# wenbowen123/BundleTrack

Measured on AMD Instinct MI355X. Metric: Gauss-Newton iters/sec (K=15, 2k corr/frame-pair) + achieved HBM GB/s, higher is better.
Workload: dtype f32

## Files before the change

bundletrack_amd/_lib.py:

```python
from __future__ import annotations

import ctypes as C
import os
import subprocess

import numpy as np

_PKG = os.path.dirname(os.path.abspath(__file__))
_ROOT = os.path.dirname(_PKG)
LIB_PATH = os.path.join(_PKG, "libbtba.so")
SRC_DIR = os.path.join(_PKG, "csrc")
HEADER = os.path.join(_ROOT, "include", "btba.h")

BTBA_OK, BTBA_EINVAL, BTBA_EHIP, BTBA_ENUMERIC, BTBA_ENOMEM, BTBA_ESCHED = 0, 1, 2, 3, 4, 5
PAIRS_TARGET_LOWER, PAIRS_TARGET_MORE_VALID, PAIRS_EXPLICIT, PAIRS_TARGET_HIGHER = 0, 1, 2, 3
REDUCE_DETERMINISTIC, REDUCE_ATOMIC = 0, 1
RANSAC_REFERENCE_SVD, RANSAC_HORN = 0, 1
RANSAC_DRAW_HASH = 0x100
FLAG_TRACE, FLAG_TIME_KERNELS = 1, 2
FLAG_OVERLAP, FLAG_NO_FUSE, FLAG_KEYED_CORR, FLAG_FLOAT4_CACHE, FLAG_NO_COMPACTION, FLAG_COMPACTION, FLAG_TIME_SAMPLED = 32, 64, 4096, 256, 512, 1024, 2048
OPT_DENSE_ORDER, OPT_TILE_MAJOR, OPT_BLOCK_WALK, OPT_BLOCK_SKIP, OPT_BIG_ASSEMBLY, OPT_OVERLAP_GROUPS, OPT_OVERLAP_EQUAL_PRIO, OPT_KEYED_CORR_MIN_BYTES, OPT_SPARSE_TAIL = 1, 2, 3, 4, 5, 6, 7, 8, 9
OPT_CHAIN, OPT_CHAIN_SPARSE_PERIOD, OPT_CHAIN_TIMEOUT_MS, OPT_COUNT_LIVE, OPT_RELAYOUT, OPT_CORR_NONTEMPORAL, OPT_SOLVE_SMALL = 10, 11, 12, 13, 14, 15, 16

ENTRYJ_DTYPE = np.dtype(
    [("imgIdx_i", "<u4"), ("imgIdx_j", "<u4"), ("pos_i", "<f4", (3,)), ("pos_j", "<f4", (3,))]
)

EXPORTED_SYMBOLS = [
    "btba_params_default", "btba_strerror", "btba_last_hip_error", "btba_version",
    "btba_workspace_create", "btba_workspace_create_on_stream", "btba_workspace_destroy", "btba_workspace_sync",
    "btba_workspace_wait_stream", "btba_workspace_signal_stream", "btba_workspace_set_option", "btba_workspace_live_blocks",
    "btba_optimize_frames", "btba_optimize_frames_keyed", "btba_frame_cache_clear", "btba_frame_cache_evict", "btba_ransac_pairs", "btba_ransac_pairs_ex", "btba_ransac_reference_uniforms", "btba_build_cache", "btba_solve_batch", "btba_solve_cached", "btba_collect_stats",
    "btba_trace_layout_get", "btba_bucket_correspondences",
    "btba_matrices_to_poses", "btba_poses_to_matrices",
    "btba_process_depth", "btba_depth_to_normals",
    "btba_build_cache_zn", "btba_pack_zn", "btba_solve_batch_zn", "btba_zn_block_ranges", "btba_zn_valid_lists", "btba_solve_batch_zn_aux", "btba_pack_correspondences24",
    "btba_match_params_default", "btba_match_capacity", "btba_match_pairs",
    "btba_mask_params_default", "btba_apply_masks",
    "btba_detector_params_default", "btba_detector_transform", "btba_detector_inputs", "btba_detector_keypoints_to_image",
    "btba_pose_errors",
    "btba_mappoints_create", "btba_mappoints_destroy", "btba_mappoints_register_frame", "btba_mappoints_forget_frame", "btba_mappoints_export",
    "btba_corres_params_default", "btba_corres_chain_capacity", "btba_corres_chain",
    "btba_window_layout", "btba_marshal_windows", "btba_procrustes_pairs",
]

MATCH_DTYPE = np.dtype(
    [("idx_a", "<i4"), ("idx_b", "<i4"), ("dist", "<f4"), ("dir", "<i4"), ("ptA_cam", "<f4", (3,)), ("ptB_cam", "<f4", (3,))]
)


class Params(C.Structure):
    _fields_ = [
        ("n_gn_iters", C.c_int32), ("n_pcg_iters", C.c_int32),
        ("robust_delta", C.c_float), ("dense_dist_thresh", C.c_float), ("dense_normal_thresh", C.c_float),
        ("depth_min", C.c_float), ("depth_max", C.c_float),
        ("weight_sparse", C.c_float), ("weight_dense_depth", C.c_float), ("image_downscale", C.c_float),
        ("pair_policy", C.c_int32), ("dense_tiles", C.c_int32), ("sparse_chunks", C.c_int32), ("flags", C.c_int32), ("reduction_mode", C.c_int32),
        ("weights_sparse_per_iter", C.c_void_p), ("weights_dense_per_iter", C.c_void_p),
        ("n_weights_per_iter", C.c_int32),
    ]


class MatchParams(C.Structure):
    _fields_ = [("k", C.c_int32), ("mutual", C.c_int32), ("max_dist_neighbor", C.c_float), ("cos_max_normal_neighbor", C.c_float),
                ("max_dist_no_neighbor", C.c_float), ("cos_max_normal_no_neighbor", C.c_float), ("min_z", C.c_float)]


class MaskParams(C.Structure):
    _fields_ = [("largest_component_hull", C.c_int32), ("dilate", C.c_int32)]


class DetectorParams(C.Structure):
    _fields_ = [("out_size", C.c_int32)]


class Stats(C.Structure):
    _fields_ = [
        ("n_instances", C.c_int32), ("n_frames", C.c_int32), ("n_pairs", C.c_int32), ("n_dense_pairs", C.c_int32),
        ("n_corr", C.c_int64),
        ("dense_tiles", C.c_int32), ("sparse_chunks", C.c_int32),
        ("ms_total", C.c_float), ("ms_upload", C.c_float), ("ms_cache", C.c_float), ("ms_solve", C.c_float),
        ("ms_dense_sweep", C.c_float), ("ms_sparse_sweep", C.c_float), ("ms_system_solve", C.c_float),
        ("n_dense_launches", C.c_int32), ("n_sparse_launches", C.c_int32), ("n_solve_launches", C.c_int32),
        ("bytes_dense_alg", C.c_int64), ("bytes_sparse_alg", C.c_int64),
        ("fused_sweeps", C.c_int32), ("cache_frames_built", C.c_int32), ("corr_pairs_uploaded", C.c_int32),
        ("chain_iterations", C.c_int32),
    ]

    def as_dict(self):
        return {f[0]: getattr(self, f[0]) for f in self._fields_}


class ZnAux(C.Structure):
    _fields_ = [("block_ranges", C.c_void_p), ("valid_lists", C.c_void_p), ("valid_counts", C.c_void_p), ("corr24", C.c_void_p)]


class TraceLayout(C.Structure):
    _fields_ = [(n, C.c_int64) for n in
                ("record_floats", "off_x", "off_T", "off_rhs", "off_precond", "off_pcg", "off_delta", "off_dense_pair", "off_A", "off_clk")]


class CorresParams(C.Structure):
    _fields_ = [("n_trials", C.c_int32), ("dist_thres", C.c_float), ("hypothesis", C.c_int32), ("pad", C.c_int32), ("seed", C.c_uint64)]


class BtbaError(RuntimeError):
    def __init__(self, status: int, where: str):
        self.status = status
        msg = lib().btba_strerror(status).decode() if _lib is not None else str(status)
        extra = f" (hipError {lib().btba_last_hip_error()})" if status == BTBA_EHIP else ""
        super().__init__(f"{where}: {msg}{extra}")


HIPCC_FLAGS = ["--offload-arch=gfx950", "-O3", "-std=c++17", "-fno-slp-vectorize", "-Wno-pass-failed", "-fPIC", "-shared", "-fvisibility=hidden"]


def build(force: bool = False, verbose: bool = False) -> str:
    srcs = [os.path.join(SRC_DIR, f) for f in os.listdir(SRC_DIR)] + [HEADER]
    newest = max(os.path.getmtime(s) for s in srcs)
    if not force and os.path.exists(LIB_PATH) and os.path.getmtime(LIB_PATH) >= newest:
        return LIB_PATH
    cmd = ["hipcc"] + HIPCC_FLAGS + ["-o", LIB_PATH, os.path.join(SRC_DIR, "btba_api.hip")]
    if verbose:
        print(" ".join(cmd))
    subprocess.check_call(cmd)
    return LIB_PATH


HOST_DRIVER = os.path.join(os.path.dirname(_PKG), "tests", "cpp", "host_driver")


def build_host_cpp(force: bool = False, verbose: bool = False) -> str:
    root = os.path.dirname(_PKG)
    srcs = [os.path.join(root, "tests", "cpp", "host_driver.cpp"), os.path.join(_PKG, "cpp", "btba_host.cpp")]
    deps = srcs + [os.path.join(_PKG, "cpp", "btba_host.hpp"), HEADER, LIB_PATH]
    if not force and os.path.exists(HOST_DRIVER) and os.path.getmtime(HOST_DRIVER) >= max(os.path.getmtime(d) for d in deps):
        return HOST_DRIVER
    rocm = os.environ.get("ROCM_PATH", "/opt/rocm")
    cmd = ["g++", "-O2", "-std=c++17", "-Wall", "-D__HIP_PLATFORM_AMD__", "-I" + os.path.join(rocm, "include"), "-o", HOST_DRIVER] + srcs + [
        "-L" + _PKG, "-lbtba", "-L" + os.path.join(rocm, "lib"), "-lamdhip64",
        "-Wl,-rpath," + _PKG, "-Wl,-rpath,$ORIGIN/../../bundletrack_amd", "-Wl,-rpath," + os.path.join(rocm, "lib")]
    if verbose:
        print(" ".join(cmd))
    subprocess.check_call(cmd)
    return HOST_DRIVER


_lib = None


def lib() -> C.CDLL:
    global _lib
    if _lib is None:
        path = os.environ.get("BTBA_LIB_PATH", LIB_PATH)
        if not os.path.exists(path):
            raise ImportError(
                f"{path} is missing: the HIP extension has not been built. "
                "Run `python -c 'import __graft_entry__ as g; g.build()'` (needs hipcc). There is no CPU fallback.")
        try:
            import torch
        except ImportError:
            pass
        L = C.CDLL(path)
        import re
        header_version = int(re.search(r"#define BTBA_VERSION (\d+)", open(HEADER).read()).group(1))
        if "BTBA_LIB_PATH" not in os.environ and L.btba_version() != header_version:
            raise ImportError(f"{path} is version {L.btba_version()}, include/btba.h is {header_version}: rebuild (python -c 'import __graft_entry__ as g; g.build()')")
        L.btba_strerror.restype = C.c_char_p
        L.btba_strerror.argtypes = [C.c_int]
        for name in EXPORTED_SYMBOLS:
            if "BTBA_LIB_PATH" in os.environ and name in ("btba_workspace_set_option", "btba_pack_correspondences24", "btba_workspace_live_blocks") and not hasattr(L, name):
                continue
            getattr(L, name)
        L.btba_workspace_create.argtypes = [C.POINTER(C.c_void_p), C.c_void_p]
        L.btba_workspace_create_on_stream.argtypes = [C.POINTER(C.c_void_p), C.c_void_p]
        L.btba_workspace_destroy.argtypes = [C.c_void_p]
        L.btba_workspace_destroy.restype = None
        L.btba_workspace_sync.argtypes = [C.c_void_p]
        if hasattr(L, "btba_workspace_set_option"):
            L.btba_workspace_set_option.argtypes = [C.c_void_p, C.c_int, C.c_int64]
        if hasattr(L, "btba_workspace_live_blocks"):
            L.btba_workspace_live_blocks.argtypes = [C.c_void_p, C.POINTER(C.c_uint64)]
        L.btba_workspace_wait_stream.argtypes = [C.c_void_p, C.c_void_p]
        L.btba_workspace_signal_stream.argtypes = [C.c_void_p, C.c_void_p]
        L.btba_collect_stats.argtypes = [C.c_void_p, C.POINTER(Stats)]
        L.btba_optimize_frames.argtypes = [
            C.c_void_p, C.POINTER(Params), C.c_int, C.c_int, C.c_int, C.c_void_p,
            C.c_void_p, C.c_uint32, C.c_void_p, C.c_void_p, C.c_void_p, C.c_void_p, C.c_int, C.c_void_p, C.POINTER(Stats)]
        L.btba_optimize_frames_keyed.argtypes = [
            C.c_void_p, C.POINTER(Params), C.c_int, C.c_int, C.c_int, C.c_void_p,
            C.c_void_p, C.c_uint32, C.c_void_p, C.c_void_p, C.c_void_p, C.c_void_p, C.c_void_p, C.c_int, C.c_void_p, C.POINTER(Stats)]
        L.btba_frame_cache_clear.argtypes = [C.c_void_p]
        L.btba_frame_cache_evict.argtypes = [C.c_void_p, C.c_uint64]
        L.btba_solve_cached.argtypes = [
            C.c_void_p, C.POINTER(Params), C.c_int, C.c_int, C.c_int, C.c_void_p,
            C.c_void_p, C.c_void_p, C.c_void_p, C.c_uint32, C.c_void_p, C.c_uint32, C.c_void_p, C.c_int, C.c_void_p, C.c_void_p]
        L.btba_build_cache.argtypes = [C.c_void_p, C.c_int, C.c_int, C.c_int, C.c_void_p, C.c_float,
                                       C.c_void_p, C.c_void_p, C.c_void_p, C.c_void_p, C.c_void_p, C.c_void_p]
        L.btba_solve_batch.argtypes = [
            C.c_void_p, C.POINTER(Params), C.c_int, C.c_int, C.c_int, C.c_int, C.c_void_p,
            C.c_void_p, C.c_void_p, C.c_void_p, C.c_int64, C.c_void_p, C.c_uint32, C.c_void_p, C.c_int, C.c_void_p, C.c_void_p]
        L.btba_trace_layout_get.argtypes = [C.c_int, C.c_int, C.c_int, C.POINTER(TraceLayout)]
        L.btba_trace_layout_get.restype = None
        L.btba_bucket_correspondences.argtypes = [C.c_void_p, C.c_uint32, C.c_int, C.c_void_p, C.c_void_p]
        L.btba_matrices_to_poses.argtypes = [C.c_void_p, C.c_int, C.c_void_p, C.c_void_p]
        L.btba_poses_to_matrices.argtypes = [C.c_void_p, C.c_int, C.c_void_p, C.c_void_p, C.c_void_p]
        L.btba_build_cache_zn.argtypes = [C.c_void_p, C.c_int, C.c_int, C.c_int, C.c_void_p, C.c_float, C.c_void_p, C.c_void_p, C.c_void_p, C.c_void_p, C.c_void_p]
        L.btba_pack_zn.argtypes = [C.c_void_p, C.c_int64, C.c_void_p, C.c_void_p, C.c_void_p]
        L.btba_solve_batch_zn.argtypes = [C.c_void_p, C.POINTER(Params), C.c_int, C.c_int, C.c_int, C.c_int, C.c_void_p, C.c_void_p,
                                          C.c_void_p, C.c_int64, C.c_void_p, C.c_uint32, C.c_void_p, C.c_int, C.c_void_p, C.c_void_p]
        L.btba_zn_block_ranges.argtypes = [C.c_void_p, C.c_int, C.c_int, C.c_int, C.c_void_p, C.c_void_p]
        if hasattr(L, "btba_pack_correspondences24"):
            L.btba_pack_correspondences24.argtypes = [C.c_void_p, C.c_int, C.c_int, C.c_void_p, C.c_int64, C.c_void_p, C.c_uint32, C.c_void_p, C.c_void_p]
        L.btba_zn_valid_lists.argtypes = [C.c_void_p, C.c_int, C.c_int, C.c_int, C.c_void_p, C.c_void_p, C.c_void_p]
        L.btba_solve_batch_zn_aux.argtypes = [C.c_void_p, C.POINTER(Params), C.c_int, C.c_int, C.c_int, C.c_int, C.c_void_p, C.c_void_p, C.POINTER(ZnAux),
                                              C.c_void_p, C.c_int64, C.c_void_p, C.c_uint32, C.c_void_p, C.c_int, C.c_void_p, C.c_void_p]
        L.btba_process_depth.argtypes = [C.c_void_p, C.c_int, C.c_int, C.c_void_p, C.c_void_p, C.c_int, C.c_float, C.c_float, C.c_int, C.c_float, C.c_float]
        L.btba_depth_to_normals.argtypes = [C.c_void_p, C.c_int, C.c_int, C.c_void_p, C.c_void_p, C.c_void_p, C.c_void_p]
        L.btba_match_params_default.argtypes = [C.POINTER(MatchParams)]
        L.btba_match_params_default.restype = None
        L.btba_match_capacity.argtypes = [C.POINTER(MatchParams), C.c_int, C.c_int, C.c_int, C.c_int, C.c_void_p, C.c_int, C.c_void_p, C.POINTER(C.c_int64)]
        L.btba_match_pairs.argtypes = [C.c_void_p, C.POINTER(MatchParams), C.c_int, C.c_int, C.c_int, C.c_int, C.c_void_p, C.c_void_p, C.c_int, C.c_void_p,
                                       C.c_void_p, C.c_void_p, C.c_void_p, C.c_void_p, C.c_void_p, C.c_int, C.c_void_p,
                                       C.c_void_p, C.c_void_p, C.c_void_p, C.c_void_p]
        L.btba_mask_params_default.argtypes = [C.POINTER(MaskParams)]
        L.btba_mask_params_default.restype = None
        L.btba_apply_masks.argtypes = [C.c_void_p, C.POINTER(MaskParams), C.c_int, C.c_int, C.c_int, C.c_void_p, C.c_void_p, C.c_void_p,
                                       C.c_void_p, C.c_void_p, C.c_void_p]
        L.btba_detector_params_default.argtypes = [C.POINTER(DetectorParams)]
        L.btba_detector_params_default.restype = None
        L.btba_detector_transform.argtypes = [C.POINTER(DetectorParams), C.c_void_p, C.c_void_p, C.c_void_p]
        L.btba_detector_inputs.argtypes = [C.c_void_p, C.POINTER(DetectorParams), C.c_int, C.c_int, C.c_int, C.c_void_p, C.c_void_p,
                                           C.c_void_p, C.c_void_p]
        L.btba_detector_keypoints_to_image.argtypes = [C.c_void_p, C.POINTER(DetectorParams), C.c_int, C.c_void_p, C.c_void_p, C.c_void_p,
                                                       C.c_void_p]
        L.btba_pose_errors.argtypes = [C.c_void_p, C.c_int, C.c_int, C.c_void_p, C.c_void_p, C.c_int, C.c_void_p, C.c_void_p, C.c_void_p,
                                       C.c_void_p, C.c_void_p]
        L.btba_mappoints_create.argtypes = [C.c_void_p, C.POINTER(C.c_void_p)]
        L.btba_mappoints_destroy.argtypes = [C.c_void_p]
        L.btba_mappoints_destroy.restype = None
        L.btba_mappoints_register_frame.argtypes = [C.c_void_p, C.c_int, C.c_void_p, C.POINTER(C.c_int32)]
        L.btba_mappoints_forget_frame.argtypes = [C.c_void_p, C.c_int32]
        L.btba_mappoints_export.argtypes = [C.c_void_p, C.c_void_p, C.c_void_p, C.c_void_p, C.c_void_p, C.c_void_p]
        L.btba_corres_params_default.argtypes = [C.POINTER(CorresParams)]
        L.btba_corres_params_default.restype = None
        L.btba_corres_chain_capacity.argtypes = L.btba_match_capacity.argtypes
        L.btba_corres_chain.argtypes = [C.c_void_p, C.c_void_p, C.POINTER(MatchParams), C.POINTER(CorresParams), C.c_int, C.c_int, C.c_int, C.c_int,
                                        C.c_void_p, C.c_void_p, C.c_int, C.c_void_p, C.c_void_p, C.c_void_p, C.c_void_p, C.c_void_p, C.c_void_p,
                                        C.c_void_p, C.c_void_p, C.c_int, C.c_void_p, C.c_void_p, C.c_void_p, C.c_void_p]
        L.btba_window_layout.argtypes = [C.c_int, C.c_int, C.c_void_p, C.c_void_p, C.c_int32, C.POINTER(C.c_int64), C.POINTER(C.c_uint32),
                                         C.c_void_p, C.c_void_p, C.c_void_p]
        L.btba_marshal_windows.argtypes = [C.c_void_p, C.c_int, C.c_int, C.c_void_p, C.c_int64, C.c_void_p, C.c_uint32, C.c_int64,
                                           C.c_void_p, C.c_void_p, C.c_void_p]
        L.btba_procrustes_pairs.argtypes = [C.c_void_p, C.c_int, C.c_int, C.c_void_p, C.c_int64, C.c_void_p, C.c_void_p, C.c_void_p,
                                            C.c_void_p, C.c_void_p, C.c_void_p]
        _lib = L
    return _lib


def check(status: int, where: str) -> None:
    if status != BTBA_OK:
        raise BtbaError(status, where)


def default_params(**kw) -> Params:
    p = Params()
    lib().btba_params_default(C.byref(p))
    for k, v in kw.items():
        if not hasattr(p, k):
            raise AttributeError(k)
        setattr(p, k, v)
    return p


def match_params(**kw) -> MatchParams:
    p = MatchParams()
    lib().btba_match_params_default(C.byref(p))
    for k, v in kw.items():
        if not hasattr(p, k):
            raise AttributeError(k)
        setattr(p, k, v)
    return p


def corres_params(**kw) -> CorresParams:
    p = CorresParams()
    lib().btba_corres_params_default(C.byref(p))
    for k, v in kw.items():
        if not hasattr(p, k):
            raise AttributeError(k)
        setattr(p, k, v)
    return p


def mask_params(**kw) -> MaskParams:
    p = MaskParams()
    lib().btba_mask_params_default(C.byref(p))
    for k, v in kw.items():
        if not hasattr(p, k):
            raise AttributeError(k)
        setattr(p, k, v)
    return p


def detector_params(**kw) -> DetectorParams:
    p = DetectorParams()
    lib().btba_detector_params_default(C.byref(p))
    for k, v in kw.items():
        if not hasattr(p, k):
            raise AttributeError(k)
        setattr(p, k, v)
    return p


def declared_symbols() -> list[str]:
    import re
    txt = open(HEADER).read()
    return sorted(set(re.findall(r"^BTBA_API[^;]*?\b(btba_[a-z_0-9]+)\s*\(", txt, flags=re.M)))


def bucket_correspondences(corr: np.ndarray, n_frames: int):
    corr = np.ascontiguousarray(corr, ENTRYJ_DTYPE)
    P = n_frames * (n_frames - 1) // 2
    out = np.zeros(max(corr.shape[0], 1), ENTRYJ_DTYPE)
    off = np.zeros(P + 1, np.uint32)
    check(lib().btba_bucket_correspondences(corr.ctypes.data, corr.shape[0], n_frames, out.ctypes.data, off.ctypes.data),
          "btba_bucket_correspondences")
    return out[: int(off[P])], off
```

bundletrack_amd/csrc/btba_api.hip:

```cpp
#include <hip/hip_runtime.h>
#include <chrono>
#include <cmath>
#include <cstdio>
#include <cstring>
#include <cstdlib>
#include <new>
#include <string>
#include <map>
#include <memory>
#include <vector>

#include "../../include/btba.h"
#include "btba_kernels.hpp"
#include "btba_solve_small.hpp"
#include "btba_solve_mid.hpp"
#include "btba_image.hpp"
#include "btba_ransac.hpp"
#include "btba_xorwow.hpp"
#include "btba_match.hpp"
#include "btba_mask.hpp"
#include "btba_detect.hpp"
#include "btba_eval.hpp"
#include "btba_mappoints.hpp"
#include "btba_window.hpp"

using namespace btba;

static thread_local int g_last_hip_error = 0;

#define HIP_TRY(expr)                                   \
    do {                                                \
        hipError_t e_ = (expr);                         \
        if (e_ != hipSuccess) {                         \
            g_last_hip_error = (int)e_;                 \
            return BTBA_EHIP;                           \
        }                                               \
    } while (0)

namespace {

struct DevBuf {
    void *p = nullptr;
    size_t cap = 0;
    int ensure(size_t bytes)
    {
        if (bytes <= cap) return BTBA_OK;
        if (p) { hipError_t e = hipFree(p); p = nullptr; cap = 0; if (e != hipSuccess) { g_last_hip_error = (int)e; return BTBA_EHIP; } }
        size_t want = bytes + bytes / 4 + 256;
        hipError_t e = hipMalloc(&p, want);
        if (e != hipSuccess) { g_last_hip_error = (int)e; p = nullptr; return e == hipErrorOutOfMemory ? BTBA_ENOMEM : BTBA_EHIP; }
        cap = want;
        return BTBA_OK;
    }
    void release() { if (p) (void)hipFree(p); p = nullptr; cap = 0; }
    template <class T> T *as() const { return reinterpret_cast<T *>(p); }
};

struct EventPair { hipEvent_t a, b; int kind; };

}

struct btba_workspace {
    hipStream_t stream = nullptr;
    bool owns_stream = false;
    int device = 0;
    DevBuf x, T, Tinv, sparse_part, dense_part, pairsum, dense_pairs, ptrs, big_A, solve_tab;
    DevBuf corr, offsets, poses, campos, normals, nvalid;
    DevBuf valid_lists, valid_counts;
    DevBuf block_ranges;
    DevBuf chain_sync;
    DevBuf chain_trace;
    DevBuf corr24_tmp;
    DevBuf live_blocks;
    bool count_live = false;
    int *chain_error = nullptr;
    bool chain_failed = false;
    bool chain_reported = false;
    uint64_t chain_launches = 0;
    struct Tuning {
        bool dense_order = true;
        bool tile_major = true;
        bool block_walk = true;
        bool block_skip = true;
        int sparse_tail_256 = -1;
        bool big_assembly = true;
        int overlap_groups = 2;
        bool overlap_equal_prio = false;
        size_t keyed_corr_min_bytes = (size_t)1 << 20;
        int chain = 0;
        int corr_nt = -1;
        int corr_nt_partial = 1;
        long long last_level_cache = 224ll << 20;
        bool relayout = false;
        int chain_group = 1;
        int chain_sparse_period = 0;
        int chain_timeout_ms = 500;
        int chain_solve_prio = 0;
        int chain_debug_skip = 0;
        bool solve_small = true;
        int prepare_keep_T = 0;
        int debug_lds_pad = 0;
        std::string chain_trace_file;
    } tune;
    std::vector<int32_t> dense_pairs_host;
    int dense_pairs_frames = -1;
    size_t dense_work_offset = 0;
    int work_formula = 0;
    int solve_tab_frames = -1;
    std::vector<EventPair> events;
    std::vector<hipEvent_t> event_pool;
    btba_stats stats{};
    bool lds_attr_set = false, small_attr_set = false, mid_attr_set = false;
    int n_cus = 0;
    bool always_time_region = false;
    static constexpr int kMaxGroups = 8;
    uint64_t solves_enqueued = 0;
    hipStream_t aux_streams[kMaxGroups - 1] = {};
    hipEvent_t ev_fork = nullptr, ev_join[kMaxGroups - 1] = {}, ev_order = nullptr;
    hipStream_t copy_stream = nullptr;
    hipEvent_t ev_copy = nullptr, ev_cache = nullptr;
    void *pin = nullptr; size_t pin_cap = 0;
    void *pin_io = nullptr; size_t pin_io_cap = 0;
    int pin_io_ensure(size_t bytes)
    {
        if (bytes <= pin_io_cap) return BTBA_OK;
        if (pin_io) { (void)hipHostFree(pin_io); pin_io = nullptr; pin_io_cap = 0; }
        const size_t want = bytes + bytes / 2 + 4096;
        hipError_t e = hipHostMalloc(&pin_io, want, hipHostMallocDefault);
        if (e != hipSuccess) { g_last_hip_error = (int)e; pin_io = nullptr; return e == hipErrorOutOfMemory ? BTBA_ENOMEM : BTBA_EHIP; }
        pin_io_cap = want;
        return BTBA_OK;
    }
    int pin_ensure(size_t bytes)
    {
        if (bytes <= pin_cap) return BTBA_OK;
        if (pin) { (void)hipHostFree(pin); pin = nullptr; pin_cap = 0; }
        const size_t want = bytes + bytes / 2 + 4096;
        hipError_t e = hipHostMalloc(&pin, want, hipHostMallocDefault);
        if (e != hipSuccess) { g_last_hip_error = (int)e; pin = nullptr; return e == hipErrorOutOfMemory ? BTBA_ENOMEM : BTBA_EHIP; }
        pin_cap = want;
        return BTBA_OK;
    }
    struct PendingSlot { int slot; uint64_t key; const float *depth, *normal; };
    std::vector<PendingSlot> pool_pending;

    struct FrameSlot { uint64_t key = 0; const float *depth = nullptr, *normal = nullptr; uint64_t stamp = 0; bool live = false; int32_t n_valid = 0; };
    DevBuf pool_zn, pool_lists, pool_counts, pool_nvalid, pool_map, pool_ranges;
    size_t pool_map_offset = 0;
    struct CorrSeg { uint32_t off = 0, count = 0; };
    DevBuf corr_pool, corr_desc, corr_stage_dev, corr_lens;
    std::map<std::pair<uint64_t, uint64_t>, CorrSeg> corr_index;
    size_t corr_pool_used = 0;
    void *corr_stage = nullptr; size_t corr_stage_cap = 0;
    DevBuf ransac;
    DevBuf ransac_u;
    std::vector<float> ransac_u_host;
    DevBuf match;
    DevBuf mask;
    DevBuf eval;
    DevBuf corres;
    DevBuf window;
    uint64_t ransac_u_seed = 0;
    std::vector<FrameSlot> pool_slots;
    int pool_H = 0, pool_W = 0, pool_npix = 0;
    float pool_downscale = 0.0f, pool_K[9] = {0};
    uint64_t pool_stamp = 0;
    uint64_t pool_hits = 0, pool_misses = 0;

    hipEvent_t get_event()
    {
        if (!event_pool.empty()) { hipEvent_t e = event_pool.back(); event_pool.pop_back(); return e; }
        hipEvent_t e = nullptr;
        if (hipEventCreate(&e) != hipSuccess) return nullptr;
        return e;
    }
};

struct DeviceGuard {
    int prev = -1;
    explicit DeviceGuard(const btba_workspace *ws)
    {
        int cur = -1;
        if (ws && hipGetDevice(&cur) == hipSuccess && cur != ws->device && hipSetDevice(ws->device) == hipSuccess) prev = cur;
    }
    ~DeviceGuard() { if (prev >= 0) (void)hipSetDevice(prev); }
    DeviceGuard(const DeviceGuard &) = delete;
    DeviceGuard &operator=(const DeviceGuard &) = delete;
};

extern "C" {

void btba_params_default(btba_params *p)
{
    if (!p) return;
    p->n_gn_iters = 7;
    p->n_pcg_iters = 5;
    p->robust_delta = 0.005f;
    p->dense_dist_thresh = 0.02f;
    p->dense_normal_thresh = (float)std::cos(45.0 / 180.0 * M_PI);
    p->depth_min = 0.1f;
    p->depth_max = 9999.0f;
    p->weight_sparse = 1.0f;
    p->weight_dense_depth = 1.0f;
    p->image_downscale = 4.0f;
    p->pair_policy = BTBA_PAIRS_TARGET_LOWER;
    p->dense_tiles = 0;
    p->sparse_chunks = 0;
    p->flags = 0;
    p->reduction_mode = BTBA_REDUCE_DETERMINISTIC;
    p->weights_sparse_per_iter = nullptr;
    p->weights_dense_per_iter = nullptr;
    p->n_weights_per_iter = 0;
}

const char *btba_strerror(int status)
{
    switch (status) {
    case BTBA_OK: return "ok";
    case BTBA_EINVAL: return "invalid argument";
    case BTBA_EHIP: return "HIP runtime error (see btba_last_hip_error)";
    case BTBA_ENUMERIC: return "non-finite value in the output poses";
    case BTBA_ENOMEM: return "out of device memory";
    case BTBA_ESCHED: return "a wait inside the chained launch timed out (workgroups did not start in grid order): the solve's poses are invalid; the workspace now solves unchained";
    default: return "unknown status";
    }
}

int btba_last_hip_error(void) { return g_last_hip_error; }
int btba_version(void) { return BTBA_VERSION; }

static int workspace_create(btba_workspace **out, void *stream, bool use_given);

int btba_workspace_create(btba_workspace **out, void *stream) { return workspace_create(out, stream, stream != nullptr); }
int btba_workspace_create_on_stream(btba_workspace **out, void *stream) { return workspace_create(out, stream, true); }

static int workspace_create(btba_workspace **out, void *stream, bool use_given)
{
    if (!out) return BTBA_EINVAL;
    *out = nullptr;
    int ndev = 0;
    HIP_TRY(hipGetDeviceCount(&ndev));
    if (ndev <= 0) { g_last_hip_error = (int)hipErrorNoDevice; return BTBA_EHIP; }
    btba_workspace *ws = new (std::nothrow) btba_workspace();
    if (!ws) return BTBA_ENOMEM;
    if (hipGetDevice(&ws->device) != hipSuccess) { delete ws; return BTBA_EHIP; }
    if (hipDeviceGetAttribute(&ws->n_cus, hipDeviceAttributeMultiprocessorCount, ws->device) != hipSuccess) ws->n_cus = 0;
    {
        auto on = [](const char *name) { const char *e = std::getenv(name); return e && e[0] && e[0] != '0'; };
        btba_workspace::Tuning &t = ws->tune;
        t.dense_order = !on("BTBA_NO_DENSE_ORDER");
        t.tile_major = !on("BTBA_PAIR_MAJOR");
        t.block_walk = !on("BTBA_NO_BLOCK_WALK");
        t.block_skip = !on("BTBA_NO_BLOCK_SKIP");
        t.big_assembly = !on("BTBA_NO_BIG_ASSEMBLY");
        if (const char *e = std::getenv("BTBA_SPARSE_TAIL")) t.sparse_tail_256 = std::max(0, std::min(256, std::atoi(e)));
        if (const char *e = std::getenv("BTBA_GROUPS")) t.overlap_groups = std::atoi(e);
        if (const char *e = std::getenv("BTBA_GROUP_PRIO")) t.overlap_equal_prio = e[0] == 'e';
        if (const char *e = std::getenv("BTBA_KEYED_CORR_MIN_BYTES")) t.keyed_corr_min_bytes = (size_t)std::strtoull(e, nullptr, 10);
        if (const char *e = std::getenv("BTBA_CHAIN")) t.chain = std::max(-1, std::min(1, std::atoi(e)));
        if (const char *e = std::getenv("BTBA_CHAIN_PERIOD")) t.chain_sparse_period = std::max(0, std::atoi(e));
        t.relayout = on("BTBA_RELAYOUT");
        t.solve_small = !on("BTBA_SOLVE_LEGACY");
        if (const char *e = std::getenv("BTBA_CORR_NT")) t.corr_nt = std::atoi(e);
        if (const char *e = std::getenv("BTBA_LLC_MB")) t.last_level_cache = (long long)std::atoll(e) << 20;
        if (const char *e = std::getenv("BTBA_CORR_NT_PARTIAL")) t.corr_nt_partial = std::atoi(e);
        if (const char *e = std::getenv("BTBA_CHAIN_TIMEOUT_MS")) t.chain_timeout_ms = std::max(1, std::atoi(e));
#if defined(BTBA_DEV_EXPERIMENTS) || defined(BTBA_REFERENCE_ORDER)
        t.prepare_keep_T = on("BTBA_PREPARE_KEEP_T") ? 1 : 0;
#endif
#ifdef BTBA_DEV_EXPERIMENTS
        if (const char *e = std::getenv("BTBA_CHAIN_GROUP")) t.chain_group = std::max(1, std::atoi(e));
        if (const char *e = std::getenv("BTBA_CHAIN_TRACE_FILE")) t.chain_trace_file = e;
        if (const char *e = std::getenv("BTBA_CHAIN_SOLVE_PRIO")) t.chain_solve_prio = std::max(0, std::min(3, std::atoi(e)));
        if (const char *e = std::getenv("BTBA_CHAIN_DEBUG_SKIP")) t.chain_debug_skip = std::atoi(e);
        if (const char *e = std::getenv("BTBA_DEBUG_LDS_PAD")) t.debug_lds_pad = std::max(0, std::min(60000, std::atoi(e)));
#endif
    }
    if (use_given) {
        ws->stream = reinterpret_cast<hipStream_t>(stream);
    } else {
        hipError_t e = hipStreamCreateWithFlags(&ws->stream, hipStreamNonBlocking);
        if (e != hipSuccess) { g_last_hip_error = (int)e; delete ws; return BTBA_EHIP; }
        ws->owns_stream = true;
    }
    *out = ws;
    return BTBA_OK;
}

void btba_workspace_destroy(btba_workspace *ws)
{
    DeviceGuard device_guard(ws);
    if (!ws) return;
    (void)hipStreamSynchronize(ws->stream);
    for (auto &ep : ws->events) { (void)hipEventDestroy(ep.a); (void)hipEventDestroy(ep.b); }
    for (auto e : ws->event_pool) (void)hipEventDestroy(e);
    DevBuf *bufs[] = { &ws->x, &ws->T, &ws->Tinv, &ws->sparse_part, &ws->dense_part, &ws->pairsum, &ws->dense_pairs, &ws->ptrs, &ws->big_A, &ws->solve_tab,
                       &ws->corr, &ws->offsets, &ws->poses, &ws->campos, &ws->normals, &ws->nvalid, &ws->valid_lists, &ws->valid_counts, &ws->block_ranges,
                       &ws->chain_sync, &ws->chain_trace, &ws->live_blocks, &ws->corr24_tmp, &ws->pool_zn, &ws->pool_lists, &ws->pool_counts, &ws->pool_nvalid, &ws->pool_map, &ws->pool_ranges, &ws->ransac, &ws->ransac_u, &ws->match, &ws->mask, &ws->eval, &ws->corr_pool, &ws->corr_desc, &ws->corr_stage_dev, &ws->corr_lens, &ws->window };
    for (auto b : bufs) b->release();
    if (ws->corr_stage) (void)hipHostFree(ws->corr_stage);
    if (ws->chain_error) (void)hipHostFree(ws->chain_error);
    for (auto st : ws->aux_streams) if (st) (void)hipStreamDestroy(st);
    if (ws->copy_stream) (void)hipStreamDestroy(ws->copy_stream);
    if (ws->ev_copy) (void)hipEventDestroy(ws->ev_copy);
    if (ws->ev_cache) (void)hipEventDestroy(ws->ev_cache);
    if (ws->pin) (void)hipHostFree(ws->pin);
    if (ws->pin_io) (void)hipHostFree(ws->pin_io);
    if (ws->ev_fork) (void)hipEventDestroy(ws->ev_fork);
    for (auto e : ws->ev_join) if (e) (void)hipEventDestroy(e);
    if (ws->ev_order) (void)hipEventDestroy(ws->ev_order);
    if (ws->owns_stream) (void)hipStreamDestroy(ws->stream);
    delete ws;
}

int btba_workspace_set_option(btba_workspace *ws, int option, int64_t value)
{
    DeviceGuard device_guard(ws);
    if (!ws) return BTBA_EINVAL;
    btba_workspace::Tuning &t = ws->tune;
    switch (option) {
    case BTBA_OPT_DENSE_ORDER: t.dense_order = value != 0; ws->dense_pairs_frames = -1; break;
    case BTBA_OPT_TILE_MAJOR: t.tile_major = value != 0; break;
    case BTBA_OPT_BLOCK_WALK: t.block_walk = value != 0; break;
    case BTBA_OPT_BLOCK_SKIP: t.block_skip = value != 0; break;
    case BTBA_OPT_BIG_ASSEMBLY: t.big_assembly = value != 0; break;
    case BTBA_OPT_SPARSE_TAIL: if (value < -1 || value > 256) return BTBA_EINVAL; t.sparse_tail_256 = (int)value; break;
    case BTBA_OPT_OVERLAP_GROUPS: if (value < 1 || value > btba_workspace::kMaxGroups) return BTBA_EINVAL; t.overlap_groups = (int)value; break;
    case BTBA_OPT_OVERLAP_EQUAL_PRIO:
        if (t.overlap_equal_prio != (value != 0)) {
            for (auto &st : ws->aux_streams) if (st) { HIP_TRY(hipStreamSynchronize(st)); HIP_TRY(hipStreamDestroy(st)); st = nullptr; }
        }
        t.overlap_equal_prio = value != 0;
        break;
    case BTBA_OPT_KEYED_CORR_MIN_BYTES: if (value < 0) return BTBA_EINVAL; t.keyed_corr_min_bytes = (size_t)value; break;
    case BTBA_OPT_CHAIN: if (value < -1 || value > 1) return BTBA_EINVAL; t.chain = (int)value; break;
    case BTBA_OPT_CHAIN_SPARSE_PERIOD: if (value < 0 || value == 1 || value > 64) return BTBA_EINVAL; t.chain_sparse_period = (int)value; break;
    case BTBA_OPT_CHAIN_TIMEOUT_MS: if (value < 1 || value > 60000) return BTBA_EINVAL; t.chain_timeout_ms = (int)value; break;
    case BTBA_OPT_RELAYOUT: t.relayout = value != 0; break;
    case BTBA_OPT_SOLVE_SMALL: t.solve_small = value != 0; break;
    case BTBA_OPT_CORR_NONTEMPORAL: if (value < -1 || value > 1) return BTBA_EINVAL; t.corr_nt = (int)value; break;
    case BTBA_OPT_COUNT_LIVE:
        ws->count_live = value != 0;
        if (ws->count_live) {
            int rc = ws->live_blocks.ensure(sizeof(unsigned long long));
            if (rc) return rc;
            HIP_TRY(hipMemsetAsync(ws->live_blocks.p, 0, sizeof(unsigned long long), ws->stream));
        }
        break;
    case 1000:
#ifdef BTBA_DEV_EXPERIMENTS
        t.chain_debug_skip = (int)value; break;
#else
        if (value != 0 && value != 64) return BTBA_EINVAL;
        t.chain_debug_skip = (int)value; break;
#endif
    default: return BTBA_EINVAL;
    }
    return BTBA_OK;
}

static int chain_check(btba_workspace *ws)
{
    if (!ws->chain_error || !*ws->chain_error) return BTBA_OK;
    *ws->chain_error = 0;
    ws->chain_failed = true;
    const bool already = ws->chain_reported;
    ws->chain_reported = false;
    return already ? BTBA_OK : BTBA_ESCHED;
}

int btba_workspace_live_blocks(btba_workspace *ws, uint64_t *blocks)
{
    DeviceGuard device_guard(ws);
    if (!ws || !blocks) return BTBA_EINVAL;
    *blocks = 0;
    if (!ws->live_blocks.p) return BTBA_OK;
    HIP_TRY(hipStreamSynchronize(ws->stream));
    unsigned long long v = 0;
    HIP_TRY(hipMemcpy(&v, ws->live_blocks.p, sizeof v, hipMemcpyDeviceToHost));
    *blocks = v;
    return BTBA_OK;
}

int btba_workspace_sync(btba_workspace *ws)
{
    DeviceGuard device_guard(ws);
    if (!ws) return BTBA_EINVAL;
    HIP_TRY(hipStreamSynchronize(ws->stream));
    return chain_check(ws);
}

static int order_streams(btba_workspace *ws, hipStream_t from, hipStream_t to)
{
    if (from == to) return BTBA_OK;
    if (!ws->ev_order) HIP_TRY(hipEventCreateWithFlags(&ws->ev_order, hipEventDisableTiming));
    HIP_TRY(hipEventRecord(ws->ev_order, from));
    HIP_TRY(hipStreamWaitEvent(to, ws->ev_order, 0));
    return BTBA_OK;
}

int btba_workspace_wait_stream(btba_workspace *ws, void *stream)
{
    DeviceGuard device_guard(ws);
    if (!ws) return BTBA_EINVAL;
    return order_streams(ws, static_cast<hipStream_t>(stream), ws->stream);
}

int btba_workspace_signal_stream(btba_workspace *ws, void *stream)
{
    DeviceGuard device_guard(ws);
    if (!ws) return BTBA_EINVAL;
    return order_streams(ws, ws->stream, static_cast<hipStream_t>(stream));
}

void btba_trace_layout_get(int n_frames, int n_dense_pairs, int n_pcg_iters, btba_trace_layout *L)
{
    if (!L) return;
    const int64_t N = n_frames, n = 6 * N;
    int64_t o = 0;
    L->off_x = o; o += N * 6;
    L->off_T = o; o += N * 16;
    L->off_rhs = o; o += N * 6;
    L->off_precond = o; o += N * 6;
    L->off_pcg = o; o += (int64_t)n_pcg_iters * 4;
    L->off_delta = o; o += N * 6;
    L->off_dense_pair = o; o += (int64_t)n_dense_pairs * kDenseVals;
    L->off_A = o; o += n * n;
    L->off_clk = o; o += 8;
    L->record_floats = o;
}

static inline int pair_index(int n_frames, uint32_t i, uint32_t j) { return (int)(i * n_frames - i * (i + 1) / 2 + (j - i - 1)); }

static int count_correspondences(const btba_entryj *in, uint32_t n, int n_frames, uint32_t *out_offsets, bool *already_bucketed)
{
    const int P = n_frames * (n_frames - 1) / 2;
    std::vector<uint32_t> cnt(P + 1, 0);
    bool ordered = true;
    int prev = 0;
    for (uint32_t e = 0; e < n; e++) {
        const btba_entryj &c = in[e];
        if (c.imgIdx_i == 0xFFFFFFFFu) { ordered = false; continue; }
        if (c.imgIdx_i >= (uint32_t)n_frames || c.imgIdx_j >= (uint32_t)n_frames || c.imgIdx_i >= c.imgIdx_j) return BTBA_EINVAL;
        const int p = pair_index(n_frames, c.imgIdx_i, c.imgIdx_j);
        ordered = ordered && (p >= prev);
        prev = p;
        cnt[p + 1]++;
    }
    out_offsets[0] = 0;
    for (int p = 0; p < P; p++) out_offsets[p + 1] = out_offsets[p] + cnt[p + 1];
    if (already_bucketed) *already_bucketed = ordered;
    return BTBA_OK;
}

static void scatter_correspondences(const btba_entryj *in, uint32_t n, int n_frames, const uint32_t *offsets, btba_entryj *out_sorted)
{
    const int P = n_frames * (n_frames - 1) / 2;
    std::vector<uint32_t> cur(offsets, offsets + P);
    for (uint32_t e = 0; e < n; e++) {
        const btba_entryj &c = in[e];
        if (c.imgIdx_i == 0xFFFFFFFFu) continue;
        out_sorted[cur[pair_index(n_frames, c.imgIdx_i, c.imgIdx_j)]++] = c;
    }
}

int btba_bucket_correspondences(const btba_entryj *in, uint32_t n, int n_frames, btba_entryj *out_sorted, uint32_t *out_offsets)
{
    if ((!in && n) || n_frames < 2 || !out_sorted || !out_offsets) return BTBA_EINVAL;
    if (int rc = count_correspondences(in, n, n_frames, out_offsets, nullptr)) return rc;
    scatter_correspondences(in, n, n_frames, out_offsets, out_sorted);
    return BTBA_OK;
}

}

static int time_begin(btba_workspace *ws, bool on, int kind, size_t *slot, hipStream_t st = nullptr)
{
    if (!st) st = ws->stream;
    *slot = (size_t)-1;
    if (!on) return BTBA_OK;
    EventPair ep{ ws->get_event(), ws->get_event(), kind };
    if (!ep.a || !ep.b) return BTBA_EHIP;
    HIP_TRY(hipEventRecord(ep.a, st));
    ws->events.push_back(ep);
    *slot = ws->events.size() - 1;
    return BTBA_OK;
}
static int time_end(btba_workspace *ws, size_t slot, hipStream_t st = nullptr)
{
    if (!st) st = ws->stream;
    if (slot == (size_t)-1) return BTBA_OK;
    HIP_TRY(hipEventRecord(ws->events[slot].b, st));
    return BTBA_OK;
}

static int pick_chunks(const btba_params *prm, int B, int P, uint32_t max_corr_per_pair, bool with_dense)
{
    if (prm->sparse_chunks > 0) return prm->sparse_chunks;
    if (max_corr_per_pair == 0) return 1;
    const long blocks = (long)B * P;
    if (with_dense) {
        const int cap = std::min(16, (int)((max_corr_per_pair + 2 * kBlock - 1) / (2 * kBlock)));
        const int want = (int)((64 + blocks - 1) / blocks);
        if (want <= cap) return std::max(1, want);
    }
    int want = (int)((512 + blocks - 1) / blocks);
    const int cap = (int)((max_corr_per_pair + 2 * kBlock - 1) / (2 * kBlock));
    if (want > cap) want = cap;
    if (want < 1) want = 1;
    if (want > 16) want = 16;
    return want;
}
static int pick_tiles(const btba_params *prm, int B, int Pd, int npix, bool lists, int Wd, int Hd)
{
    if (prm->dense_tiles > 0) return prm->dense_tiles;
    if (Pd == 0) return 1;
    const long blocks = (long)B * Pd;
    if (lists) return blocks >= 64 ? 1 : 3;
    int want = blocks >= 1536 ? 1 : blocks >= 768 ? 2 : blocks >= 192 ? 4 : 8;
    const int cap = (npix + kBlock - 1) / kBlock;
    if (want > cap) want = cap;
    if (want < 1) want = 1;
    if (Wd % 8 == 0 && Hd % 8 == 0) {
        const int bw = Wd / 8, bh = Hd / 8;
        const int min_tiles = (bw * bh + 1023) / 1024;
        if (want < min_tiles && bw <= 1024) want = std::min(min_tiles, bh);
        const int rows_per = (bh + want - 1) / want;
        want = (bh + rows_per - 1) / rows_per;
        while (want < bh && (long)((bh + want - 1) / want) * bw > 1024 && bw <= 1024) want++;
    }
    return want;
}

static void scaled_intrinsics(int H, int W, int Hd, int Wd, const float *K, float intr[4], Mat4 *Kinv);

struct ZnSpec {
    const float *zn = nullptr; int H = 0, W = 0; const float *K = nullptr;
    const int *frame_slot = nullptr;
    const uint32_t *lists = nullptr; const int *counts = nullptr;
    const float *block_ranges = nullptr;
};

static int solve_enqueue(btba_workspace *ws, const btba_params *prm, int B, int N, int Hd, int Wd, const float *intr,
                         const float *campos, const float *normals, const ZnSpec &Z, const btba_entryj *corr, int64_t corr_stride,
                         const uint32_t *pair_offsets, uint32_t max_corr_per_pair,
                         const int32_t *dense_pairs, int Pd_in, float *poses, float *trace, int *order_flag = nullptr,
                         bool corr24 = false, const uint32_t *pair_lens = nullptr)
{
    if (!ws || !prm || B < 1 || N < 2 || Hd < 2 || Wd < 2 || !intr || !poses) return BTBA_EINVAL;
    if (prm->n_gn_iters < 1 || prm->n_pcg_iters < 0) return BTBA_EINVAL;
    if (ws->chain_error && *ws->chain_error && !ws->chain_reported) { ws->chain_reported = true; ws->chain_failed = true; return BTBA_ESCHED; }
    if (prm->reduction_mode != BTBA_REDUCE_DETERMINISTIC && prm->reduction_mode != BTBA_REDUCE_ATOMIC) return BTBA_EINVAL;
    const bool atomic_sums = prm->reduction_mode == BTBA_REDUCE_ATOMIC;
    if (atomic_sums && trace) return BTBA_EINVAL;
    if (N > BTBA_MAX_FRAMES) return BTBA_EINVAL;
    const int P = N * (N - 1) / 2;
    const float *wsi = prm->weights_sparse_per_iter, *wdi = prm->weights_dense_per_iter;
    if ((wsi || wdi) && prm->n_weights_per_iter != prm->n_gn_iters) return BTBA_EINVAL;
    auto ws_at = [&](int it) { return wsi ? wsi[it] : prm->weight_sparse; };
    auto wd_at = [&](int it) { return wdi ? wdi[it] : prm->weight_dense_depth; };
    bool any_dense_weight = false, any_sparse_weight = false;
    for (int it = 0; it < prm->n_gn_iters; it++) {
        if (!(ws_at(it) >= 0.0f) || !(wd_at(it) >= 0.0f)) return BTBA_EINVAL;
        any_dense_weight |= wd_at(it) > 0.0f; any_sparse_weight |= ws_at(it) > 0.0f;
    }
    const bool use_sparse = any_sparse_weight && corr && pair_offsets && max_corr_per_pair > 0;
    std::vector<int32_t> pairs;
    if (any_dense_weight) {
        if (dense_pairs && Pd_in >= 0) pairs.assign(dense_pairs, dense_pairs + 2 * (size_t)Pd_in);
        else for (int i = 0; i < N; i++) for (int j = i + 1; j < N; j++) { pairs.push_back(i); pairs.push_back(j); }
        for (size_t k = 0; k < pairs.size(); k += 2)
            if (pairs[k] < 0 || pairs[k] >= N || pairs[k + 1] < 0 || pairs[k + 1] >= N || pairs[k] == pairs[k + 1]) return BTBA_EINVAL;
        if (dense_pairs && Pd_in >= 0) {
            std::vector<char> seen((size_t)N * N, 0);
            for (size_t k = 0; k < pairs.size(); k += 2) {
                char &c = seen[(size_t)pairs[k] * N + pairs[k + 1]];
                if (c) return BTBA_EINVAL;
                c = 1;
            }
        }
    }
    const int Pd = (int)(pairs.size() / 2);
    const bool use_zn = Z.zn != nullptr;
    const bool use_dense = Pd > 0 && ((campos && normals) || use_zn);
    if (!use_sparse && !use_dense) {
    }
    const int npix = Hd * Wd;
    int B_launch = B;
    if (B >= 8 && (prm->flags & BTBA_FLAG_OVERLAP)) {
        const int groups = std::max(1, std::min({ ws->tune.overlap_groups, (int)btba_workspace::kMaxGroups, B / 2 }));
        B_launch = B / groups;
    }
    const int chunks = use_sparse ? pick_chunks(prm, B_launch, P, max_corr_per_pair, use_dense && !(prm->flags & BTBA_FLAG_NO_FUSE)) : 1;
    const int tiles = use_dense ? pick_tiles(prm, B_launch, Pd, npix, use_zn && (prm->flags & BTBA_FLAG_COMPACTION), Wd, Hd) : 1;
    const bool timing = (prm->flags & BTBA_FLAG_TIME_KERNELS) != 0;
    const int timed_iteration = (prm->flags & BTBA_FLAG_TIME_SAMPLED) ? (int)(ws->solves_enqueued++ % (uint64_t)std::max(1, prm->n_gn_iters)) : -1;

    int rc;
    if ((rc = ws->x.ensure(sizeof(float) * 6 * (size_t)B * N))) return rc;
    if ((rc = ws->T.ensure(sizeof(float) * 16 * (size_t)B * N))) return rc;
    if ((rc = ws->Tinv.ensure(sizeof(float) * 16 * (size_t)B * N))) return rc;
    if ((rc = ws->sparse_part.ensure(sizeof(float) * (size_t)B * P * chunks * kSparseVals))) return rc;
    if ((rc = ws->dense_part.ensure(sizeof(float) * (size_t)B * (Pd > 0 ? Pd : 1) * tiles * kDenseVals))) return rc;
    if (Pd > 0 && (pairs != ws->dense_pairs_host || ws->dense_pairs_frames != N)) {
        std::vector<int32_t> tab(pairs);
        std::vector<int32_t> off(N + 1, 0);
        for (int q = 0; q < Pd; q++) { off[pairs[2 * q] + 1]++; off[pairs[2 * q + 1] + 1]++; }
        for (int k = 0; k < N; k++) off[k + 1] += off[k];
        std::vector<int32_t> adj(2 * (size_t)Pd), cur(off.begin(), off.end() - 1);
        for (int q = 0; q < Pd; q++) { adj[cur[pairs[2 * q]]++] = (q << 1); adj[cur[pairs[2 * q + 1]]++] = (q << 1) | 1; }
        tab.insert(tab.end(), off.begin(), off.end());
        tab.insert(tab.end(), adj.begin(), adj.end());
        std::vector<int32_t> first_listed((size_t)N * N, -1);
        for (int q = Pd - 1; q >= 0; q--) first_listed[(size_t)pairs[2 * q] * N + pairs[2 * q + 1]] = q;
        for (int i = 0; i < N; i++) for (int j = i + 1; j < N; j++) tab.push_back(first_listed[(size_t)i * N + j]);
        std::vector<int32_t> order(Pd);
        for (int q = 0; q < Pd; q++) order[q] = q;
        if (ws->tune.dense_order) std::stable_sort(order.begin(), order.end(), [&](int32_t a, int32_t b2) { return std::abs(pairs[2 * a] - pairs[2 * a + 1]) < std::abs(pairs[2 * b2] - pairs[2 * b2 + 1]); });
        ws->work_formula = 0;
        if (Pd == N * (N - 1) / 2) {
            for (int form = 1; form <= 2 && !ws->work_formula; form++) {
                bool same = true;
                int q = 0;
                for (int d = 1; d < N && same; d++)
                    for (int i = 0; i + d < N && same; i++, q++) {
                        const int pc = pair_index(N, (uint32_t)i, (uint32_t)(i + d));
                        same = order[q] == pc && pairs[2 * pc] == (form == 1 ? i : i + d) && pairs[2 * pc + 1] == (form == 1 ? i + d : i);
                    }
                if (same) ws->work_formula = form;
            }
        }
        while (tab.size() % 4) tab.push_back(0);
        ws->dense_work_offset = tab.size();
        for (int q = 0; q < Pd; q++) { tab.push_back(pairs[2 * order[q]]); tab.push_back(pairs[2 * order[q] + 1]); tab.push_back(order[q]); tab.push_back(0); }
        if ((rc = ws->dense_pairs.ensure(sizeof(int32_t) * tab.size()))) return rc;
        HIP_TRY(hipMemcpyAsync(ws->dense_pairs.p, tab.data(), sizeof(int32_t) * tab.size(), hipMemcpyHostToDevice, ws->stream));
        HIP_TRY(hipStreamSynchronize(ws->stream));
        ws->dense_pairs_host = pairs;
        ws->dense_pairs_frames = N;
    }
    if (ws->solve_tab_frames != N) {
        const size_t lut16 = ((size_t)P + 288 + 3) & ~(size_t)3;
        std::vector<int32_t> tab(lut16 + 288);
        int q = 0;
        for (int i = 0; i < N; i++) for (int j = i + 1; j < N; j++) tab[q++] = (i << 8) | j;
        for (int t = 0; t < 72; t++) { sparse_entry_descriptor(t >= 36, (t % 36) / 6, t % 6, &tab[(size_t)P + 4 * t]); sparse_entry_descriptor(t >= 36, (t % 36) / 6, t % 6, &tab[lut16 + 4 * t]); }
        if ((rc = ws->solve_tab.ensure(sizeof(int32_t) * tab.size()))) return rc;
        HIP_TRY(hipMemcpyAsync(ws->solve_tab.p, tab.data(), sizeof(int32_t) * tab.size(), hipMemcpyHostToDevice, ws->stream));
        HIP_TRY(hipStreamSynchronize(ws->stream));
        ws->solve_tab_frames = N;
    }
    const int32_t *d_adj_off = ws->dense_pairs.as<int32_t>() + 2 * (size_t)Pd;
    const int32_t *d_adj = d_adj_off + (N + 1);

    SolveDims D{};
    D.n_frames = N; D.n_pairs = P; D.n_dense_pairs = use_dense ? Pd : 0;
    D.npix = npix; D.width = Wd; D.height = Hd;
    D.sparse_chunks = chunks; D.dense_tiles = tiles; D.n_pcg = prm->n_pcg_iters;
    D.use_sparse = use_sparse; D.use_dense = use_dense;
    D.fx = intr[0]; D.fy = intr[1]; D.cx = intr[2]; D.cy = intr[3];
    D.robust_delta = prm->robust_delta; D.dist_thresh = prm->dense_dist_thresh; D.normal_thresh = prm->dense_normal_thresh;
    D.dist2_thresh = prm->dense_dist_thresh * prm->dense_dist_thresh;
    D.wm1 = (float)(Wd - 1); D.hm1 = (float)(Hd - 1); D.wm2 = (float)(Wd - 2); D.hm2 = (float)(Hd - 2);
    D.depth_min = prm->depth_min; D.depth_max = prm->depth_max;
    D.w_sparse = prm->weight_sparse; D.w_dense = prm->weight_dense_depth;
    D.corr_stride = corr_stride;
    D.corr_nt_from = B;
    D.order_flag = order_flag;
    D.live_blocks = (ws->count_live && ws->live_blocks.p) ? ws->live_blocks.as<unsigned long long>() : nullptr;
    D.pose_stride = 16 * N; D.x_stride = 6 * N;
    D.sp_stride = (unsigned)((size_t)P * (atomic_sums ? 1 : chunks) * kSparseVals);
    D.dp_stride = (unsigned)((size_t)(Pd > 0 ? Pd : 1) * (atomic_sums ? 1 : tiles) * kDenseVals);
    if ((size_t)B * std::max(D.sp_stride, D.dp_stride) >= ((size_t)1 << 32) || (size_t)B * 16 * N >= ((size_t)1 << 31)) return BTBA_EINVAL;
    D.atomic_sums = atomic_sums ? 1 : 0;
    D.corr24 = corr24 ? 1 : 0;
    D.pair_lens = pair_lens;
    if (Pd > 0) { D.dense_work = reinterpret_cast<const int4 *>(ws->dense_pairs.as<int32_t>() + ws->dense_work_offset); D.work_formula = ws->work_formula; }
    D.tile_major = ws->tune.tile_major ? 1 : 0;
    D.sparse_tail_256 = 0;
    D.walk_blocks = (Wd % 8 == 0 && Hd % 8 == 0 && Wd + Hd <= 1024 && ws->tune.block_walk) ? 1 : 0;
    D.n_gn = prm->n_gn_iters;
    int zn_layout = 0;
    if (use_zn) {
        if (!Z.K || Z.H < 2 || Z.W < 2) return BTBA_EINVAL;
        float intr_chk[4];
        Mat4 Kinv;
        scaled_intrinsics(Z.H, Z.W, Hd, Wd, Z.K, intr_chk, &Kinv);
        for (int k = 0; k < 16; k++) D.zn_ki[k] = Kinv.m[k];
        D.zn_scale_w = (float)(Z.W - 1) / (float)(Wd - 1);
        D.zn_scale_h = (float)(Z.H - 1) / (float)(Hd - 1);
        const float *ki = D.zn_ki;
        D.zn_simple = (ki[1] == 0.f && ki[3] == 0.f && ki[4] == 0.f && ki[7] == 0.f && ki[12] == 0.f && ki[13] == 0.f && ki[14] == 0.f && ki[15] == 1.0f) ? 1 : 0;
        zn_layout = D.zn_simple ? 1 : 2;
    }
    D.trace_on = (trace != nullptr) && (prm->flags & BTBA_FLAG_TRACE);
    btba_trace_layout L;
    btba_trace_layout_get(N, D.n_dense_pairs, prm->n_pcg_iters, &L);
    D.trace_record = L.record_floats; D.tr_x = L.off_x; D.tr_T = L.off_T; D.tr_rhs = L.off_rhs; D.tr_prec = L.off_precond;
    D.tr_pcg = L.off_pcg; D.tr_delta = L.off_delta; D.tr_dpair = L.off_dense_pair; D.tr_A = L.off_A; D.tr_clk = L.off_clk;

    const size_t n = 6 * (size_t)N, ld = 4 * (((n + 3) / 4) | 1);
    const size_t lds_rest = (6 * ld + 16 + 16 * (size_t)N + 4 * (size_t)D.n_dense_pairs + (size_t)N + 1 + (size_t)P + 288 + (((size_t)P + 3) & ~(size_t)3) + ((6 * (size_t)N + 3) & ~(size_t)3)) * sizeof(float);
    const size_t lds_limit = 160 * 1024;
    const bool a_global = n * ld * sizeof(float) + lds_rest > lds_limit;
    const size_t lds_core = (a_global ? 0 : n * ld * sizeof(float)) + lds_rest;
    const size_t lds_pairs = ((size_t)P * kSparseVals + (size_t)D.n_dense_pairs * kDenseVals) * sizeof(float);
    D.pairsum_in_lds = (lds_core + lds_pairs <= 64 * 1024) ? 1 : 0;
    if (!D.pairsum_in_lds && lds_core + lds_pairs <= lds_limit && B <= 256) D.pairsum_in_lds = 1;
    const size_t lds_bytes = lds_core + (D.pairsum_in_lds ? lds_pairs : 0);
    if (lds_bytes > lds_limit) return BTBA_EINVAL;
    if (!D.pairsum_in_lds) { if ((rc = ws->pairsum.ensure((size_t)B * lds_pairs + 16))) return rc; }
    const size_t mid_lds = sizeof(float) * mid_solve_lds_floats(N, D.n_dense_pairs);
    const bool mid_solve = ws->tune.solve_small && N > kSmallMaxFrames && N <= kMidMaxFrames && !atomic_sums && !a_global && D.n_dense_pairs <= P && mid_lds <= lds_limit;
    D.pre_assembled = ((a_global || N >= 24) && !trace && ws->tune.big_assembly && !mid_solve) ? 1 : 0;
    if (a_global || D.pre_assembled) { if ((rc = ws->big_A.ensure((size_t)B * (n + 2) * ld * sizeof(float)))) return rc; }
    if (D.pre_assembled && D.pairsum_in_lds) { D.pairsum_in_lds = 0; if ((rc = ws->pairsum.ensure((size_t)B * lds_pairs + 16))) return rc; }
    if (lds_bytes > 64 * 1024 || !ws->lds_attr_set) {
        HIP_TRY(hipFuncSetAttribute(reinterpret_cast<const void *>(&k_system_solve<true, false>), hipFuncAttributeMaxDynamicSharedMemorySize, (int)lds_limit));
        HIP_TRY(hipFuncSetAttribute(reinterpret_cast<const void *>(&k_system_solve<false, false>), hipFuncAttributeMaxDynamicSharedMemorySize, (int)lds_limit));
        HIP_TRY(hipFuncSetAttribute(reinterpret_cast<const void *>(&k_system_solve<true, true>), hipFuncAttributeMaxDynamicSharedMemorySize, (int)lds_limit));
        HIP_TRY(hipFuncSetAttribute(reinterpret_cast<const void *>(&k_system_solve<false, true>), hipFuncAttributeMaxDynamicSharedMemorySize, (int)lds_limit));
        ws->lds_attr_set = true;
    }

    const int small_cpl_v = small_cpl(N);
    const size_t small_lds = sizeof(float) * small_solve_lds_floats(N, D.n_dense_pairs, small_cpl_v);
    const bool small_solve = ws->tune.solve_small && N <= kSmallMaxFrames && !atomic_sums && !a_global && !D.pre_assembled && 2 * D.n_dense_pairs <= kSmallBlock && small_lds <= lds_limit;
    if (small_solve && !ws->small_attr_set) {
        HIP_TRY(hipFuncSetAttribute(reinterpret_cast<const void *>(&k_solve_small<4>), hipFuncAttributeMaxDynamicSharedMemorySize, (int)lds_limit));
        HIP_TRY(hipFuncSetAttribute(reinterpret_cast<const void *>(&k_solve_small<8>), hipFuncAttributeMaxDynamicSharedMemorySize, (int)lds_limit));
        HIP_TRY(hipFuncSetAttribute(reinterpret_cast<const void *>(&k_solve_small<12>), hipFuncAttributeMaxDynamicSharedMemorySize, (int)lds_limit));
        HIP_TRY(hipFuncSetAttribute(reinterpret_cast<const void *>(&k_solve_small<16>), hipFuncAttributeMaxDynamicSharedMemorySize, (int)lds_limit));
        ws->small_attr_set = true;
    }
    if (mid_solve && !ws->mid_attr_set) {
        HIP_TRY(hipFuncSetAttribute(reinterpret_cast<const void *>(&k_solve_mid), hipFuncAttributeMaxDynamicSharedMemorySize, (int)lds_limit));
        ws->mid_attr_set = true;
    }

    btba_stats &S = ws->stats;
    if (ws->events.empty() || !timing) std::memset(&S, 0, sizeof S);
    S.n_instances = B; S.n_frames = N; S.n_pairs = P; S.n_dense_pairs = D.n_dense_pairs;
    S.dense_tiles = tiles; S.sparse_chunks = chunks;
    S.bytes_dense_alg = use_dense ? (int64_t)64 * D.n_dense_pairs * npix * B : 0;
    S.bytes_sparse_alg = 0;

    {
        const int nb0 = (B >= 8 && (prm->flags & BTBA_FLAG_OVERLAP)) ? B / 2 : B;
        S.fused_sweeps = (use_sparse && use_dense && (unsigned)chunks * P * nb0 >= 64u && (unsigned)tiles * D.n_dense_pairs * nb0 >= 64u && !(prm->flags & BTBA_FLAG_NO_FUSE)) ? 1 : 0;
    }
    size_t reg;
    if ((rc = time_begin(ws, timing || ws->always_time_region, 3, &reg))) return rc;
    if (atomic_sums) {
        HIP_TRY(hipMemsetAsync(ws->sparse_part.p, 0, sizeof(float) * (size_t)B * P * kSparseVals, ws->stream));
        HIP_TRY(hipMemsetAsync(ws->dense_part.p, 0, sizeof(float) * (size_t)B * (Pd > 0 ? Pd : 1) * kDenseVals, ws->stream));
    }
    const bool compaction = use_zn && use_dense && (prm->flags & BTBA_FLAG_COMPACTION);
    const int chain_lay = zn_layout == 1 ? (compaction ? 3 : 1) : 0;
    const bool chain = chain_lay != 0 && !ws->chain_failed && ws->n_cus == 256 && ws->tune.chain > 0 && use_sparse && use_dense && !wsi && !wdi
                       && !trace && !atomic_sums && !a_global && !D.pre_assembled && N <= kChainMaxFrames && chunks <= kChainMaxParts && tiles <= kChainMaxParts
                       && !(prm->flags & (BTBA_FLAG_NO_FUSE | BTBA_FLAG_OVERLAP)) && !Z.frame_slot
                       && lds_rest + 16 + sizeof(float) * chain_region_floats(N) <= kChainLdsBytes;
    const bool relayout = ws->tune.relayout && use_sparse && !corr24 && !pair_lens && !chain && prm->n_gn_iters >= 3 && !atomic_sums && !compaction
                          && (size_t)B * (size_t)corr_stride * sizeof(btba_entryj) >= ((size_t)4 << 20);
    if (relayout) { if ((rc = ws->corr24_tmp.ensure(sizeof(float2) * 192 * (((size_t)B * (size_t)corr_stride + 63) / 64)))) return rc; }
    const long long frames_bytes = use_dense ? (long long)B * N * npix * (use_zn ? 16 : 32) : 0;
    const long long corr_bytes = use_sparse ? (long long)B * (long long)corr_stride * (corr24 ? 24 : 32) : 0;
    const long long corr_per_instance = corr_bytes / B;
    int corr_nt_auto = B;
    if (use_dense && use_sparse && !compaction && frames_bytes + corr_bytes > ws->tune.last_level_cache)
        corr_nt_auto = (frames_bytes >= ws->tune.last_level_cache || corr_per_instance <= 0) ? 0 : (int)std::min<long long>(B, (ws->tune.last_level_cache - frames_bytes) / corr_per_instance);
    if (ws->tune.corr_nt_partial == 0 && corr_nt_auto < B) corr_nt_auto = 0;
    const int corr_nt_from = ws->tune.corr_nt >= 0 ? (ws->tune.corr_nt ? 0 : B) : corr_nt_auto;
    ChainDims Cn{};
    int plain_pairsum_in_lds = 0;
    auto pad32 = [](size_t floats) { return (floats + 31) & ~(size_t)31; };
    if (chain) {
        const int n_it = prm->n_gn_iters;
        D.pose_stride = (int)pad32(16 * (size_t)N); D.x_stride = (int)pad32(6 * (size_t)N);
        D.sp_stride = (unsigned)pad32((size_t)P * chunks * kSparseVals); D.dp_stride = (unsigned)pad32((size_t)Pd * tiles * kDenseVals);
        D.publish = 1;
        D.corr_nt_from = corr_nt_from;
        plain_pairsum_in_lds = D.pairsum_in_lds;
        D.pairsum_in_lds = 0;
        Cn.last_solve_external = 1;
        Cn.n_iter = n_it; Cn.n_inst = B; Cn.inst_per_xcd = (unsigned)((B + 7) / 8);
        Cn.items_d = (unsigned)tiles * (unsigned)D.n_dense_pairs; Cn.items_s = (unsigned)chunks * (unsigned)P;
        Cn.sparse_period = (unsigned)ws->tune.chain_sparse_period;
        if (Cn.sparse_period >= 2u && Cn.sparse_period * Cn.items_s > Cn.items_d + Cn.items_s) Cn.sparse_period = (Cn.items_d + Cn.items_s) / Cn.items_s;
        if (Cn.sparse_period < 2u) Cn.sparse_period = 0u;
        Cn.group = (Cn.sparse_period == 0u && ws->tune.chain_group > 1 && Cn.inst_per_xcd % (unsigned)ws->tune.chain_group == 0u && B % 8 == 0) ? (unsigned)ws->tune.chain_group : 1u;
        Cn.timeout_ticks = (long long)ws->tune.chain_timeout_ms * 100000ll;
        Cn.solve_prio = ws->tune.chain_solve_prio;
        Cn.debug_skip = ws->tune.chain_debug_skip;
        if (Cn.debug_skip & 16) D.publish = 0;
        Cn.pose_ring = (size_t)B * D.pose_stride; Cn.x_ring = (size_t)B * D.x_stride;
        Cn.sp_ring = (size_t)B * (size_t)D.sp_stride; Cn.dp_ring = (size_t)B * (size_t)D.dp_stride;
        Cn.ps_size = pad32((size_t)D.n_dense_pairs * kDenseVals); Cn.A_size = pad32((n + 2) * ld);
        if ((rc = ws->x.ensure(sizeof(float) * (n_it + 1) * Cn.x_ring))) return rc;
        if ((rc = ws->T.ensure(sizeof(float) * (n_it + 1) * Cn.pose_ring))) return rc;
        if ((rc = ws->Tinv.ensure(sizeof(float) * (n_it + 1) * Cn.pose_ring))) return rc;
        if ((rc = ws->sparse_part.ensure(sizeof(float) * n_it * Cn.sp_ring))) return rc;
        if ((rc = ws->dense_part.ensure(sizeof(float) * n_it * Cn.dp_ring))) return rc;
        if ((rc = ws->pairsum.ensure(sizeof(float) * (size_t)n_it * B * Cn.ps_size))) return rc;
        if ((rc = ws->big_A.ensure(sizeof(float) * (size_t)n_it * B * Cn.A_size))) return rc;
        const size_t sync_head = ((size_t)B * (n_it + 1) + 15) & ~(size_t)15;
        const size_t sync_ints = sync_head + (size_t)16 * B * (n_it + 1);
        if ((rc = ws->chain_sync.ensure(sizeof(int) * sync_ints))) return rc;
        if (!ws->chain_error) {
            HIP_TRY(hipHostMalloc(reinterpret_cast<void **>(&ws->chain_error), 64, hipHostMallocDefault));
            *ws->chain_error = 0;
        }
        HIP_TRY(hipMemsetAsync(ws->chain_sync.p, 0, sizeof(int) * sync_ints, ws->stream));
        Cn.flags = ws->chain_sync.as<int>(); Cn.arrivals = Cn.flags + B; Cn.published = Cn.flags + sync_head; Cn.error = ws->chain_error;
    }
    {
        const int total = B * N;
        if (chain) k_prepare_strided<<<(total + 63) / 64, 64, 0, ws->stream>>>(total, N, D.pose_stride, D.x_stride, poses, ws->x.as<float>(), ws->T.as<float>(), ws->Tinv.as<float>());
        else k_prepare<<<(total + 63) / 64, 64, 0, ws->stream>>>(total, poses, ws->x.as<float>(), ws->T.as<float>(), ws->Tinv.as<float>(), ws->tune.prepare_keep_T);
    }
    const uint32_t *lists_base = Z.lists;
    const int *counts_base = Z.counts;
    if (compaction && !lists_base) {
        if ((rc = ws->valid_lists.ensure(sizeof(uint32_t) * (size_t)B * N * npix))) return rc;
        if ((rc = ws->valid_counts.ensure(sizeof(int) * (size_t)B * N))) return rc;
        k_valid_lists<<<B * N, 1024, 0, ws->stream>>>(npix, reinterpret_cast<const float4 *>(Z.zn), ws->valid_lists.as<uint32_t>(), ws->valid_counts.as<int>(), nullptr);
        lists_base = ws->valid_lists.as<uint32_t>();
        counts_base = ws->valid_counts.as<int>();
    }
    if (Z.frame_slot && B != 1) return BTBA_EINVAL;
    D.frame_slot = Z.frame_slot;
    size_t blist_bytes = 0;
    if (!(zn_layout == 1 && use_dense && !compaction)) D.walk_blocks = 0;
    D.sparse_tail_256 = ws->tune.sparse_tail_256 >= 0 ? ws->tune.sparse_tail_256 : ((use_dense && !compaction) ? 256 : 0);
    if (D.walk_blocks) {
        const int bw = Wd / 8, bh = Hd / 8;
        const size_t band_blocks = (size_t)((bh + tiles - 1) / tiles) * bw;
        if (band_blocks > 1024) D.walk_blocks = 0;
        else {
            blist_bytes = 32 + sizeof(uint32_t) * band_blocks;
            if (ws->tune.block_skip) {
                if (Z.block_ranges) D.block_ranges = reinterpret_cast<const float2 *>(Z.block_ranges);
                else if (!Z.frame_slot) {
                    if ((rc = ws->block_ranges.ensure(sizeof(float2) * (size_t)B * N * bw * bh))) return rc;
                    k_block_ranges<<<dim3((unsigned)((bw * bh + kBlock / 64 - 1) / (kBlock / 64)), (unsigned)(B * N)), kBlock, 0, ws->stream>>>(Wd, Hd, reinterpret_cast<const float4 *>(Z.zn), nullptr, ws->block_ranges.as<float2>());
                    D.block_ranges = ws->block_ranges.as<float2>();
                }
            }
        }
    }
    int n_halves = (B >= 8 && (prm->flags & BTBA_FLAG_OVERLAP)) ? 2 : 1;
    if (n_halves == 2) n_halves = std::max(1, std::min({ ws->tune.overlap_groups, (int)btba_workspace::kMaxGroups, B / 2 }));
    for (int g = 1; g < n_halves; g++) {
        if (ws->aux_streams[g - 1]) continue;
        int prio_least = 0, prio_greatest = 0;
        HIP_TRY(hipDeviceGetStreamPriorityRange(&prio_least, &prio_greatest));
        HIP_TRY(hipStreamCreateWithPriority(&ws->aux_streams[g - 1], hipStreamNonBlocking, ws->tune.overlap_equal_prio ? 0 : prio_least));
        HIP_TRY(hipEventCreateWithFlags(&ws->ev_join[g - 1], hipEventDisableTiming));
        if (!ws->ev_fork) HIP_TRY(hipEventCreateWithFlags(&ws->ev_fork, hipEventDisableTiming));
    }
    struct Half { int b0, nb; hipStream_t st; } halves[btba_workspace::kMaxGroups];
    for (int g = 0; g < n_halves; g++) {
        const int lo = (int)((long long)B * g / n_halves), hi = (int)((long long)B * (g + 1) / n_halves);
        halves[g] = { lo, hi - lo, g == 0 ? ws->stream : ws->aux_streams[g - 1] };
    }
    if (n_halves > 1) {
        HIP_TRY(hipEventRecord(ws->ev_fork, ws->stream));
        for (int g = 1; g < n_halves; g++) HIP_TRY(hipStreamWaitEvent(ws->aux_streams[g - 1], ws->ev_fork, 0));
    }
    const size_t pairsum_floats = lds_pairs / sizeof(float);
    S.chain_iterations = 0;
    const size_t lut_bytes = sizeof(float) * (size_t)((Wd + Hd + 3) & ~3) + (zn_layout == 1 ? sizeof(float4) * (size_t)(Wd + Hd) : 0) + blist_bytes + (size_t)ws->tune.debug_lds_pad;
    if (chain) {
        const size_t chain_lds = std::max(lut_bytes, lds_rest + 16 + sizeof(float) * chain_region_floats(N));
        const unsigned per_inst = Cn.items_d + Cn.items_s + 1u;
        const unsigned grid = 8u * (unsigned)prm->n_gn_iters * Cn.inst_per_xcd * per_inst;
        if (!ws->tune.chain_trace_file.empty()) {
            const size_t trace_bytes = 32 * (size_t)grid + 64 * (size_t)prm->n_gn_iters * B;
            if ((rc = ws->chain_trace.ensure(trace_bytes))) return rc;
            HIP_TRY(hipMemsetAsync(ws->chain_trace.p, 0, trace_bytes, ws->stream));
            Cn.trace = ws->chain_trace.as<unsigned long long>();
            Cn.stamps = Cn.trace + 4 * (size_t)grid;
        }
        const float4 *corr_c = reinterpret_cast<const float4 *>(corr);
        size_t slot;
        if (Cn.debug_skip & 32) {
            ChainDims C1 = Cn;
            C1.n_iter = 1; C1.debug_skip |= 8; C1.trace = nullptr; C1.stamps = nullptr;
            const unsigned grid1 = 8u * Cn.inst_per_xcd * per_inst;
            if ((rc = ws->pairsum.ensure(sizeof(float) * (size_t)B * ((size_t)P * kSparseVals + (size_t)D.n_dense_pairs * kDenseVals + 64)))) return rc;
            for (int it = 0; it < prm->n_gn_iters; it++) {
                if ((rc = time_begin(ws, timing, 0, &slot))) return rc;
#define BTBA_CHAIN_ARGS1 D, C1, reinterpret_cast<const float4 *>(Z.zn), ws->T.as<float>(), ws->Tinv.as<float>(), ws->x.as<float>(), ws->dense_part.as<float>(), corr_c, pair_offsets, \
                        ws->sparse_part.as<float>(), compaction ? lists_base : nullptr, compaction ? counts_base : nullptr, ws->dense_pairs.as<int2>(), d_adj_off, d_adj, ws->solve_tab.as<int>(), \
                        ws->pairsum.as<float>(), ws->big_A.as<float>(), poses
                if (chain_lay == 1) k_chain<1><<<dim3(grid1), kBlock, chain_lds, ws->stream>>>(BTBA_CHAIN_ARGS1);
                else k_chain<3><<<dim3(grid1), kBlock, chain_lds, ws->stream>>>(BTBA_CHAIN_ARGS1);
#undef BTBA_CHAIN_ARGS1
                if ((rc = time_end(ws, slot))) return rc;
                if ((rc = time_begin(ws, timing, 2, &slot))) return rc;
                k_system_solve<false, false><<<B, kSolveBlock, lds_core, ws->stream>>>(D, it, ws->sparse_part.as<float>(), ws->dense_part.as<float>(), ws->dense_pairs.as<int2>(), d_adj_off, d_adj,
                    ws->x.as<float>(), ws->T.as<float>(), ws->Tinv.as<float>(), ws->pairsum.as<float>(), nullptr, nullptr, it == prm->n_gn_iters - 1 ? poses : nullptr, ws->solve_tab.as<int>());
                if ((rc = time_end(ws, slot))) return rc;
            }
            S.fused_sweeps = 1;
        } else {
        if ((rc = time_begin(ws, timing, 0, &slot))) return rc;
#define BTBA_CHAIN_ARGS D, Cn, reinterpret_cast<const float4 *>(Z.zn), ws->T.as<float>(), ws->Tinv.as<float>(), ws->x.as<float>(), ws->dense_part.as<float>(), corr_c, pair_offsets, \
                        ws->sparse_part.as<float>(), compaction ? lists_base : nullptr, compaction ? counts_base : nullptr, ws->dense_pairs.as<int2>(), d_adj_off, d_adj, ws->solve_tab.as<int>(), \
                        ws->pairsum.as<float>(), ws->big_A.as<float>(), poses
        if (chain_lay == 1) k_chain<1><<<dim3(grid), kBlock, chain_lds, ws->stream>>>(BTBA_CHAIN_ARGS);
        else k_chain<3><<<dim3(grid), kBlock, chain_lds, ws->stream>>>(BTBA_CHAIN_ARGS);
#undef BTBA_CHAIN_ARGS
        if ((rc = time_end(ws, slot))) return rc;
        if (Cn.last_solve_external) {
            const int il = prm->n_gn_iters - 1;
            SolveDims Dl = D;
            Dl.pairsum_in_lds = plain_pairsum_in_lds; Dl.publish = 0;
            if (!Dl.pairsum_in_lds) { if ((rc = ws->pairsum.ensure(std::max(sizeof(float) * (size_t)prm->n_gn_iters * B * Cn.ps_size, (size_t)B * lds_pairs + 16)))) return rc; }
            if ((rc = time_begin(ws, timing, 2, &slot))) return rc;
#define BTBA_LAST_SOLVE(LP) k_system_solve<LP, false><<<B, kSolveBlock, lds_bytes, ws->stream>>>(Dl, il, ws->sparse_part.as<float>() + il * Cn.sp_ring, ws->dense_part.as<float>() + il * Cn.dp_ring, \
                ws->dense_pairs.as<int2>(), d_adj_off, d_adj, ws->x.as<float>() + il * Cn.x_ring, ws->T.as<float>() + il * Cn.pose_ring, ws->Tinv.as<float>() + il * Cn.pose_ring, \
                ws->pairsum.as<float>(), nullptr, nullptr, poses, ws->solve_tab.as<int>())
            if (Dl.pairsum_in_lds) BTBA_LAST_SOLVE(true); else BTBA_LAST_SOLVE(false);
#undef BTBA_LAST_SOLVE
            if ((rc = time_end(ws, slot))) return rc;
        }
        k_chain_poison<<<(16 * B * N + 255) / 256, 256, 0, ws->stream>>>(Cn.error, poses, 16 * B * N);
        S.chain_iterations = prm->n_gn_iters;
        S.fused_sweeps = 1;
        ws->chain_launches++;
        if (Cn.trace) {
            HIP_TRY(hipStreamSynchronize(ws->stream));
            std::vector<unsigned long long> host(4 * (size_t)grid + 8 * (size_t)prm->n_gn_iters * B);
            HIP_TRY(hipMemcpy(host.data(), ws->chain_trace.p, 8 * host.size(), hipMemcpyDeviceToHost));
            if (FILE *f = std::fopen(ws->tune.chain_trace_file.c_str(), "wb")) {
                const unsigned long long nrec = grid;
                std::fwrite(&nrec, 8, 1, f); std::fwrite(host.data(), 8, host.size(), f); std::fclose(f);
            }
        }
        }
    } else
    for (int it = 0; it < prm->n_gn_iters; it++) {
        const bool timing_it = timing && (timed_iteration < 0 || timed_iteration == it);
        SolveDims Di = D;
        Di.w_sparse = ws_at(it); Di.w_dense = wd_at(it);
        const bool use_dense_it = use_dense && Di.w_dense > 0.0f;
        Di.use_dense = use_dense_it ? 1 : 0;
        for (int h = 0; h < n_halves; h++) {
            const Half &H = halves[h];
            const size_t b0 = (size_t)H.b0;
            const float *campos_h = campos ? campos + 4 * b0 * N * npix : nullptr, *normals_h = normals ? normals + 4 * b0 * N * npix : nullptr;
            const float4 *zn_h = use_zn ? reinterpret_cast<const float4 *>(Z.zn) + b0 * N * npix : nullptr;
            const uint32_t *vl_h = compaction ? lists_base + b0 * N * npix : nullptr;
            const int *vc_h = compaction ? counts_base + b0 * N : nullptr;
            const bool c24_it = corr24 || (relayout && it > 0);
            const float4 *corr_h = corr ? (corr24 ? reinterpret_cast<const float4 *>(corr) : (relayout && it > 0) ? ws->corr24_tmp.as<float4>()
                                                  : reinterpret_cast<const float4 *>(corr) + 2 * b0 * (size_t)corr_stride) : nullptr;
            const uint32_t *off_h = pair_offsets ? pair_offsets + b0 * (P + 1) : nullptr;
            float *x_h = ws->x.as<float>() + 6 * b0 * N, *T_h = ws->T.as<float>() + 16 * b0 * N, *Ti_h = ws->Tinv.as<float>() + 16 * b0 * N;
            float *sp_h = ws->sparse_part.as<float>() + b0 * P * (atomic_sums ? 1 : chunks) * kSparseVals;
            float *dp_h = ws->dense_part.as<float>() + b0 * (size_t)(Pd > 0 ? Pd : 1) * (atomic_sums ? 1 : tiles) * kDenseVals;
            float *ps_h = ws->pairsum.p ? ws->pairsum.as<float>() + b0 * pairsum_floats : nullptr;
            float *tr_h = trace ? trace + b0 * (size_t)D.n_gn * D.trace_record : nullptr;
            size_t slot;
            SolveDims Dh = Di;
            if (Dh.pair_lens) Dh.pair_lens += b0 * P;
            Dh.corr24 = c24_it ? 1 : 0;
            Dh.corr_entry0 = (c24_it || relayout) ? (int64_t)b0 * corr_stride : 0;
            Dh.corr24_out = (relayout && it == 0) ? ws->corr24_tmp.as<float2>() : nullptr;
            if (Dh.block_ranges) Dh.block_ranges += b0 * N * (size_t)((Wd / 8) * (Hd / 8));
            const unsigned n_d = (unsigned)tiles * D.n_dense_pairs * H.nb, n_s = (unsigned)chunks * P * H.nb;
            const bool fuse = use_sparse && use_dense_it && n_s >= 64 && n_d >= 64 && !(prm->flags & BTBA_FLAG_NO_FUSE);
            Dh.corr_nt_from = ((fuse && use_dense_it) || ws->tune.corr_nt >= 0) ? corr_nt_from - (int)b0 : B;
            if (fuse) {
                if ((rc = time_begin(ws, timing_it, 0, &slot, H.st))) return rc;
#define BTBA_FUSED_ARGS(CACHE) Dh, n_d, n_s, CACHE, reinterpret_cast<const float4 *>(normals_h), ws->dense_pairs.as<int2>(), T_h, Ti_h, dp_h, corr_h, off_h, sp_h, vl_h, vc_h
                const int lay = zn_layout ? zn_layout + (compaction ? 2 : 0) : 0;
                if (lay == 0) k_fused_sweeps<0><<<dim3(n_d + n_s), kBlock, 0, H.st>>>(BTBA_FUSED_ARGS(reinterpret_cast<const float4 *>(campos_h)));
                else if (lay == 1) k_fused_sweeps<1><<<dim3(n_d + n_s), kBlock, lut_bytes, H.st>>>(BTBA_FUSED_ARGS(zn_h));
                else if (lay == 2) k_fused_sweeps<2><<<dim3(n_d + n_s), kBlock, lut_bytes, H.st>>>(BTBA_FUSED_ARGS(zn_h));
                else if (lay == 3) k_fused_sweeps<3><<<dim3(n_d + n_s), kBlock, lut_bytes, H.st>>>(BTBA_FUSED_ARGS(zn_h));
                else k_fused_sweeps<4><<<dim3(n_d + n_s), kBlock, lut_bytes, H.st>>>(BTBA_FUSED_ARGS(zn_h));
#undef BTBA_FUSED_ARGS
                if ((rc = time_end(ws, slot, H.st))) return rc;
            } else {
                if (use_sparse) {
                    if ((rc = time_begin(ws, timing_it, 1, &slot, H.st))) return rc;
                    k_sparse_sweep<<<dim3(chunks, P, H.nb), kBlock, 0, H.st>>>(Dh, corr_h, off_h, T_h, sp_h);
                    if ((rc = time_end(ws, slot, H.st))) return rc;
                }
                if (use_dense_it) {
                    if ((rc = time_begin(ws, timing_it, 0, &slot, H.st))) return rc;
                    const dim3 dgrid(n_d);
#define BTBA_DENSE_ARGS Di, reinterpret_cast<const float4 *>(campos_h), reinterpret_cast<const float4 *>(normals_h), ws->dense_pairs.as<int2>(), T_h, Ti_h, dp_h
                    if (zn_layout == 1 && !compaction) k_dense_sweep_zn<true, false><<<dgrid, kBlock, lut_bytes, H.st>>>(Dh, zn_h, ws->dense_pairs.as<int2>(), T_h, Ti_h, dp_h, vl_h, vc_h);
                    else if (zn_layout == 2 && !compaction) k_dense_sweep_zn<false, false><<<dgrid, kBlock, lut_bytes, H.st>>>(Dh, zn_h, ws->dense_pairs.as<int2>(), T_h, Ti_h, dp_h, vl_h, vc_h);
                    else if (zn_layout == 1) k_dense_sweep_zn<true, true><<<dgrid, kBlock, lut_bytes, H.st>>>(Dh, zn_h, ws->dense_pairs.as<int2>(), T_h, Ti_h, dp_h, vl_h, vc_h);
                    else if (zn_layout == 2) k_dense_sweep_zn<false, true><<<dgrid, kBlock, lut_bytes, H.st>>>(Dh, zn_h, ws->dense_pairs.as<int2>(), T_h, Ti_h, dp_h, vl_h, vc_h);
                    else k_dense_sweep<<<dgrid, kBlock, 0, H.st>>>(BTBA_DENSE_ARGS);
#undef BTBA_DENSE_ARGS
                    if ((rc = time_end(ws, slot, H.st))) return rc;
                }
            }
            if ((rc = time_begin(ws, timing_it, 2, &slot, H.st))) return rc;
            float *A_h = (a_global || D.pre_assembled) ? ws->big_A.as<float>() + b0 * (n + 2) * ld : nullptr;
            float *out_h = (it == prm->n_gn_iters - 1) ? poses + 16 * b0 * N : nullptr;
            SolveDims Ds = Di;
            if (atomic_sums) { Ds.sparse_chunks = 1; Ds.dense_tiles = 1; }
            if (D.pre_assembled) {
                const size_t n_sums = (size_t)P * kSparseVals + (size_t)D.n_dense_pairs * kDenseVals;
                k_big_reduce<<<dim3((unsigned)((n_sums + 255) / 256), (unsigned)H.nb), 256, 0, H.st>>>(Ds, sp_h, dp_h, ps_h);
                const BigTasks bt = big_tasks(N, P, (int)ld);
                k_big_assemble<<<dim3((bt.total + 255u) / 256u, (unsigned)H.nb), 256, 0, H.st>>>(Di, ps_h, ws->dense_pairs.as<int2>(), d_adj_off, d_adj, ws->solve_tab.as<int>(), A_h);
            }
#define BTBA_SOLVE(LP, AG) k_system_solve<LP, AG><<<H.nb, kSolveBlock, lds_bytes, H.st>>>(Ds, it, sp_h, dp_h, ws->dense_pairs.as<int2>(), d_adj_off, d_adj, x_h, T_h, Ti_h, ps_h, tr_h, A_h, out_h, ws->solve_tab.as<int>())
            if (small_solve || mid_solve) {
                SmallSolveArgs Sa{};
                Sa.n_frames = N; Sa.n_pairs = P; Sa.n_dense_pairs = use_dense_it ? D.n_dense_pairs : 0;
                Sa.sparse_chunks = Ds.sparse_chunks; Sa.dense_tiles = Ds.dense_tiles; Sa.n_pcg = D.n_pcg; Sa.use_sparse = use_sparse ? 1 : 0;
                Sa.w_sparse = Di.w_sparse;
                Sa.sp_stride = D.sp_stride; Sa.dp_stride = D.dp_stride; Sa.pose_stride = D.pose_stride; Sa.x_stride = D.x_stride;
                Sa.iter = it;
                Sa.trace_record = D.trace_record; Sa.tr_x = D.tr_x; Sa.tr_T = D.tr_T; Sa.tr_rhs = D.tr_rhs; Sa.tr_prec = D.tr_prec; Sa.tr_pcg = D.tr_pcg;
                Sa.tr_delta = D.tr_delta; Sa.tr_dpair = D.tr_dpair; Sa.tr_A = D.tr_A; Sa.tr_clk = D.tr_clk; Sa.trace_instance = (int64_t)D.n_gn * D.trace_record;
                Sa.sparse_partials = sp_h; Sa.dense_partials = dp_h;
                Sa.adj_off = d_adj_off; Sa.adj = d_adj; Sa.cross = d_adj + 2 * (size_t)Pd; Sa.pair_ij = ws->solve_tab.as<int>(); Sa.entry_lut = ws->solve_tab.as<int>() + (((size_t)P + 288 + 3) & ~(size_t)3);
                Sa.x = x_h; Sa.T = T_h; Sa.Tinv = Ti_h; Sa.poses_out = out_h; Sa.trace = D.trace_on ? tr_h : nullptr;
                if (mid_solve) k_solve_mid<<<H.nb, kSmallBlock, mid_lds, H.st>>>(Sa);
                else if (small_cpl_v == 4) k_solve_small<4><<<H.nb, kSmallBlock, small_lds, H.st>>>(Sa);
                else if (small_cpl_v == 8) k_solve_small<8><<<H.nb, kSmallBlock, small_lds, H.st>>>(Sa);
                else if (small_cpl_v == 12) k_solve_small<12><<<H.nb, kSmallBlock, small_lds, H.st>>>(Sa);
                else k_solve_small<16><<<H.nb, kSmallBlock, small_lds, H.st>>>(Sa);
            } else
            if (a_global) { if (D.pairsum_in_lds) BTBA_SOLVE(true, true); else BTBA_SOLVE(false, true); }
            else { if (D.pairsum_in_lds) BTBA_SOLVE(true, false); else BTBA_SOLVE(false, false); }
#undef BTBA_SOLVE
            if ((rc = time_end(ws, slot, H.st))) return rc;
        }
    }
    for (int g = 1; g < n_halves; g++) {
        HIP_TRY(hipEventRecord(ws->ev_join[g - 1], ws->aux_streams[g - 1]));
        HIP_TRY(hipStreamWaitEvent(ws->stream, ws->ev_join[g - 1], 0));
    }
    if ((rc = time_end(ws, reg))) return rc;
    HIP_TRY(hipGetLastError());
    return BTBA_OK;
}

extern "C" {

int btba_collect_stats(btba_workspace *ws, btba_stats *stats)
{
    DeviceGuard device_guard(ws);
    if (!ws) return BTBA_EINVAL;
    HIP_TRY(hipStreamSynchronize(ws->stream));
    btba_stats &S = ws->stats;
    for (auto &ep : ws->events) {
        float ms = 0.0f;
        hipError_t e = hipEventElapsedTime(&ms, ep.a, ep.b);
        if (e == hipSuccess) {
            switch (ep.kind) {
            case 0: S.ms_dense_sweep += ms; S.n_dense_launches++; break;
            case 1: S.ms_sparse_sweep += ms; S.n_sparse_launches++; break;
            case 2: S.ms_system_solve += ms; S.n_solve_launches++; break;
            case 3: S.ms_solve += ms; break;
            case 4: S.ms_cache += ms; break;
            default: break;
            }
        }
        ws->event_pool.push_back(ep.a);
        ws->event_pool.push_back(ep.b);
    }
    ws->events.clear();
    if (stats) *stats = S;
    S.ms_dense_sweep = S.ms_sparse_sweep = S.ms_system_solve = S.ms_solve = S.ms_cache = 0.0f;
    S.n_dense_launches = S.n_sparse_launches = S.n_solve_launches = 0;
    return chain_check(ws);
}

int btba_solve_batch(btba_workspace *ws, const btba_params *params, int n_instances, int n_frames, int Hd, int Wd, const float *intr,
                     const float *campos_dev, const float *normals_dev, const btba_entryj *corr_dev, int64_t corr_stride,
                     const uint32_t *pair_offsets_dev, uint32_t max_corr_per_pair, const int32_t *dense_pairs, int n_dense_pairs,
                     float *poses_dev, float *trace_dev)
{
    DeviceGuard device_guard(ws);
    if (!ws) return BTBA_EINVAL;
    if (ws->events.size() > 65536) {
        for (auto &ep : ws->events) { ws->event_pool.push_back(ep.a); ws->event_pool.push_back(ep.b); }
        ws->events.clear();
    }
    return solve_enqueue(ws, params, n_instances, n_frames, Hd, Wd, intr, campos_dev, normals_dev, ZnSpec{}, corr_dev, corr_stride,
                         pair_offsets_dev, max_corr_per_pair, dense_pairs, dense_pairs ? n_dense_pairs : -1, poses_dev, trace_dev);
}

int btba_solve_cached(btba_workspace *ws, const btba_params *params, int n_frames, int Hd, int Wd, const float *intr,
                      const float *campos_dev, const float *normals_dev, const btba_entryj *corr_dev, uint32_t n_corr,
                      const uint32_t *pair_offsets_dev, uint32_t max_corr_per_pair, const int32_t *dense_pairs, int n_dense_pairs,
                      float *poses_dev, float *trace_dev)
{
    DeviceGuard device_guard(ws);
    return btba_solve_batch(ws, params, 1, n_frames, Hd, Wd, intr, campos_dev, normals_dev, corr_dev, (int64_t)(n_corr ? n_corr : 1), pair_offsets_dev,
                            max_corr_per_pair, dense_pairs, n_dense_pairs, poses_dev, trace_dev);
}

static void scaled_intrinsics(int H, int W, int Hd, int Wd, const float *K, float intr[4], Mat4 *Kinv)
{
    intr[0] = K[0] * ((float)Wd / (float)W);
    intr[1] = K[4] * ((float)Hd / (float)H);
    intr[2] = K[2] * ((float)(Wd - 1) / (float)(W - 1));
    intr[3] = K[5] * ((float)(Hd - 1) / (float)(H - 1));
    const float m[16] = { K[0], K[1], K[2], 0, K[3], K[4], K[5], 0, K[6], K[7], K[8], 0, 0, 0, 0, 1 };
    auto minor = [&](int r0, int r1, int r2, int c0, int c1, int c2) {
        return m[4 * r0 + c0] * (m[4 * r1 + c1] * m[4 * r2 + c2] - m[4 * r1 + c2] * m[4 * r2 + c1])
             - m[4 * r0 + c1] * (m[4 * r1 + c0] * m[4 * r2 + c2] - m[4 * r1 + c2] * m[4 * r2 + c0])
             + m[4 * r0 + c2] * (m[4 * r1 + c0] * m[4 * r2 + c1] - m[4 * r1 + c1] * m[4 * r2 + c0]);
    };
    float adj[16];
    for (int r = 0; r < 4; r++)
        for (int c = 0; c < 4; c++) {
            int rr[3], cc[3], a = 0, b = 0;
            for (int k = 0; k < 4; k++) { if (k != r) rr[a++] = k; if (k != c) cc[b++] = k; }
            float mn = minor(rr[0], rr[1], rr[2], cc[0], cc[1], cc[2]);
// ... 1666 lines not shown
```

bundletrack_amd/csrc/btba_kernels.hpp:

```cpp
#pragma once
#ifndef BTBA_FUSED_WAVES
#define BTBA_FUSED_WAVES 6
#endif
#if defined(BTBA_REFERENCE_ORDER) && !defined(BTBA_EXACT_DIV)
#define BTBA_EXACT_DIV 1
#endif
#include <type_traits>
#include <hip/hip_runtime.h>
#include <stdint.h>
#include "btba_device.hpp"

namespace btba {

constexpr int kBlock = 256;
constexpr int kSolveBlock = 1024;
constexpr int kSparseVals = 44;
constexpr int kDenseVals = 28;
constexpr float kEps = 0.000001f;
constexpr int kRedFloats = 4 * kSparseVals + 8;


struct SolveDims {
    int n_frames;
    int n_pairs;
    int n_dense_pairs;
    int npix, width, height;
    int sparse_chunks;
    int dense_tiles;
    int n_pcg;
    int use_sparse, use_dense;
    float fx, fy, cx, cy;
    float robust_delta, dist_thresh, normal_thresh, depth_min, depth_max;
    float dist2_thresh;
    float wm1, hm1, wm2, hm2;
    float w_sparse, w_dense;
    int64_t corr_stride;
    int trace_on;
    int64_t trace_record;
    int64_t tr_x, tr_T, tr_rhs, tr_prec, tr_pcg, tr_delta, tr_dpair, tr_A, tr_clk;
    int n_gn;
    int pairsum_in_lds;
    int pre_assembled;
    int walk_blocks;
    const int4 *dense_work;
    int work_formula;
    const float2 *block_ranges;
    int sparse_tail_256;
    int tile_major;
    int *order_flag;
    int atomic_sums;
    int corr24;
    int64_t corr_entry0;
    const uint32_t *pair_lens;
    float zn_ki[16];
    float zn_scale_w, zn_scale_h;
    int zn_simple;
    const int *frame_slot;
    int pose_stride, x_stride;
    unsigned sp_stride, dp_stride;
    float2 *corr24_out;
    unsigned long long *live_blocks;
    int publish;
    int corr_nt_from;
};

__device__ __forceinline__ size_t frame_slot_of(const SolveDims &D, size_t f) { return D.frame_slot ? (size_t)D.frame_slot[f] : f; }

__device__ __forceinline__ void pair_from_index(int p, int n, int &i, int &j)
{
    int ii = 0, rem = p;
    while (rem >= n - 1 - ii) { rem -= n - 1 - ii; ii++; }
    i = ii; j = ii + 1 + rem;
}
__device__ __forceinline__ int pair_index(int i, int j, int n) { return i * n - i * (i + 1) / 2 + (j - i - 1); }

__device__ __forceinline__ Mat4 load_mat4(const float *p)
{
    Mat4 m;
    const float4 *q = reinterpret_cast<const float4 *>(p);
    float4 a = q[0], b = q[1], c = q[2], d = q[3];
    m.m[0] = a.x; m.m[1] = a.y; m.m[2] = a.z; m.m[3] = a.w;
    m.m[4] = b.x; m.m[5] = b.y; m.m[6] = b.z; m.m[7] = b.w;
    m.m[8] = c.x; m.m[9] = c.y; m.m[10] = c.z; m.m[11] = c.w;
    m.m[12] = d.x; m.m[13] = d.y; m.m[14] = d.z; m.m[15] = d.w;
    return m;
}
__device__ __forceinline__ Mat4 load_mat4_uniform(const float *p)
{
    Mat4 m;
    const float4 a = ld_const_f4(p), b = ld_const_f4(p + 4), c = ld_const_f4(p + 8), d = ld_const_f4(p + 12);
    m.m[0] = a.x; m.m[1] = a.y; m.m[2] = a.z; m.m[3] = a.w;
    m.m[4] = b.x; m.m[5] = b.y; m.m[6] = b.z; m.m[7] = b.w;
    m.m[8] = c.x; m.m[9] = c.y; m.m[10] = c.z; m.m[11] = c.w;
    m.m[12] = d.x; m.m[13] = d.y; m.m[14] = d.z; m.m[15] = d.w;
    return m;
}
__device__ __forceinline__ void store_mat4(float *p, const Mat4 &m)
{
    float4 *q = reinterpret_cast<float4 *>(p);
    q[0] = make_float4(m.m[0], m.m[1], m.m[2], m.m[3]);
    q[1] = make_float4(m.m[4], m.m[5], m.m[6], m.m[7]);
    q[2] = make_float4(m.m[8], m.m[9], m.m[10], m.m[11]);
    q[3] = make_float4(m.m[12], m.m[13], m.m[14], m.m[15]);
}

__global__ void __launch_bounds__(64) k_prepare(int total, const float *__restrict__ poses, float *__restrict__ x, float *__restrict__ T, float *__restrict__ Tinv, int keep_T = 0)
{
    const int idx = blockIdx.x * blockDim.x + threadIdx.x;
    if (idx >= total) return;
    const Mat4 M = load_mat4(poses + 16 * (size_t)idx);
    float rot[3], trans[3];
    matrix_to_pose(M, rot, trans);
    if (x) { float *o = x + 6 * (size_t)idx; o[0] = rot[0]; o[1] = rot[1]; o[2] = rot[2]; o[3] = trans[0]; o[4] = trans[1]; o[5] = trans[2]; }
    if (T || Tinv) {
        Mat4 E = pose_to_matrix(rot, trans);
#if defined(BTBA_DEV_EXPERIMENTS) || defined(BTBA_REFERENCE_ORDER)
        if (keep_T) E = M;
#endif
        if (T) store_mat4(T + 16 * (size_t)idx, E);
        if (Tinv) store_mat4(Tinv + 16 * (size_t)idx, mat_inverse(E));
    }
}

__global__ void __launch_bounds__(64) k_poses_to_matrices(int total, const float *__restrict__ x, float *__restrict__ T, float *__restrict__ Tinv)
{
    const int idx = blockIdx.x * blockDim.x + threadIdx.x;
    if (idx >= total) return;
    const float *o = x + 6 * (size_t)idx;
    const float rot[3] = { o[0], o[1], o[2] }, trans[3] = { o[3], o[4], o[5] };
    const Mat4 E = pose_to_matrix(rot, trans);
    if (T) store_mat4(T + 16 * (size_t)idx, E);
    if (Tinv) store_mat4(Tinv + 16 * (size_t)idx, mat_inverse(E));
}

__global__ void __launch_bounds__(kBlock) k_build_cache(int W, int H, int Wd, int Hd, Mat4 Kinv,
                                                       const float *const *__restrict__ depth, const float *const *__restrict__ normals,
                                                       float4 *__restrict__ campos_out, float4 *__restrict__ normals_out, int *__restrict__ n_valid)
{
#pragma clang fp contract(off)
    const int f = blockIdx.y;
    const int o = blockIdx.x * blockDim.x + threadIdx.x;
    const int npix = Wd * Hd;
    int valid = 0;
    if (o < npix) {
        const int x = o % Wd, y = o / Wd;
        const float scaleW = (float)(W - 1) / (float)(Wd - 1);
        const float scaleH = (float)(H - 1) / (float)(Hd - 1);
        const unsigned xi = (unsigned)(x * scaleW + 0.5f);
        const unsigned yi = (unsigned)(y * scaleH + 0.5f);
        if (xi < (unsigned)W && yi < (unsigned)H) {
            const size_t s = (size_t)yi * W + xi;
            const float d = depth[f][s];
            float4 cp = make_float4(0.f, 0.f, 0.f, 0.f);
            if ((double)d >= 0.1) {
                const float vx = (float)xi * d, vy = (float)yi * d;
                cp.x = Kinv.m[0] * vx + Kinv.m[1] * vy + Kinv.m[2] * d + Kinv.m[3] * d;
                cp.y = Kinv.m[4] * vx + Kinv.m[5] * vy + Kinv.m[6] * d + Kinv.m[7] * d;
                cp.z = Kinv.m[12] * vx + Kinv.m[13] * vy + Kinv.m[14] * d + Kinv.m[15] * d;
                cp.w = 1.0f;
                valid = 1;
            }
            campos_out[(size_t)f * npix + o] = cp;
            normals_out[(size_t)f * npix + o] = reinterpret_cast<const float4 *>(normals[f])[s];
        }
    }
    if (n_valid) {
        const unsigned long long b = __ballot(valid);
        if ((threadIdx.x & 63) == 0 && b) atomicAdd(&n_valid[f], __popcll(b));
    }
}

template <bool SIMPLE>
__device__ __forceinline__ float3 zn_backproject(const float *ki, float cx, float cy, float d)
{
#pragma clang fp contract(off)
    d = (d >= 0.1f) ? d : 0.0f;
    if (SIMPLE) return make_float3(cx * d, cy * d, ki[15] * d);
    const float vx = cx * d, vy = cy * d;
    return make_float3(ki[0] * vx + ki[1] * vy + ki[2] * d + ki[3] * d, ki[4] * vx + ki[5] * vy + ki[6] * d + ki[7] * d,
                       ki[12] * vx + ki[13] * vy + ki[14] * d + ki[15] * d);
}
__device__ __forceinline__ unsigned zn_src_coord(int c, float scale)
{
#pragma clang fp contract(off)
    return (unsigned)(c * scale + 0.5f);
}

__global__ void __launch_bounds__(kBlock) k_build_cache_zn(int W, int H, int Wd, int Hd, const float *const *__restrict__ depth, const float *const *__restrict__ normals,
                                                          float4 *__restrict__ zn_out, int *__restrict__ n_valid, const int *__restrict__ out_slot)
{
#pragma clang fp contract(off)
    const int f = blockIdx.y;
    const int fo = out_slot ? out_slot[f] : f;
    const int o = blockIdx.x * blockDim.x + threadIdx.x;
    const int npix = Wd * Hd;
    int valid = 0;
    if (o < npix) {
        const int x = o % Wd, y = o / Wd;
        const float scaleW = (float)(W - 1) / (float)(Wd - 1);
        const float scaleH = (float)(H - 1) / (float)(Hd - 1);
        const unsigned xi = (unsigned)(x * scaleW + 0.5f);
        const unsigned yi = (unsigned)(y * scaleH + 0.5f);
        if (xi < (unsigned)W && yi < (unsigned)H) {
            const size_t s = (size_t)yi * W + xi;
            const float d = depth[f][s];
            const float4 nr = reinterpret_cast<const float4 *>(normals[f])[s];
            valid = ((double)d >= 0.1) ? 1 : 0;
            zn_out[(size_t)fo * npix + o] = make_float4(valid ? d : 0.0f, nr.x, nr.y, nr.z);
        }
    }
    if (n_valid) {
        const unsigned long long b = __ballot(valid);
        if ((threadIdx.x & 63) == 0 && b) atomicAdd(&n_valid[fo], __popcll(b));
    }
}

__global__ void __launch_bounds__(kBlock) k_pack_zn(size_t total, const float4 *__restrict__ campos, const float4 *__restrict__ normals, float4 *__restrict__ zn)
{
    const size_t o = (size_t)blockIdx.x * blockDim.x + threadIdx.x;
    if (o >= total) return;
    const float4 c = campos[o], nr = normals[o];
    zn[o] = make_float4(c.z, nr.x, nr.y, nr.z);
}

__device__ __forceinline__ size_t corr24_index(size_t E) { return (E >> 6) * 192 + (E & 63); }
template <bool C24, bool NT>
__device__ __forceinline__ void sparse_block_impl(const SolveDims &D, const float4 *__restrict__ corr, const uint32_t *__restrict__ pair_offsets,
                                                  const float *__restrict__ T, float *__restrict__ partials, int chunk, int p, int b, float *red)
{
    const unsigned tid = item_tid();
    int fi, fj;
    pair_from_index(p, D.n_frames, fi, fj);
    const auto off = as_const(pair_offsets + (size_t)b * (D.n_pairs + 1));
    const uint32_t seg0 = off[p];
    const uint32_t len = D.pair_lens ? as_const(D.pair_lens)[(size_t)b * D.n_pairs + p] : off[p + 1] - seg0;
    const uint32_t per = (len + D.sparse_chunks - 1) / D.sparse_chunks;
    const uint32_t lo = seg0 + min(len, per * chunk), hi = seg0 + min(len, per * (chunk + 1));
    const float *Tb = T + (unsigned)b * (unsigned)D.pose_stride;
    const Mat4 Ti = load_mat4_uniform(Tb + 16 * fi);
    const Mat4 Tj = load_mat4_uniform(Tb + 16 * fj);
    float acc[kSparseVals];
#pragma unroll
    for (int k = 0; k < kSparseVals; k++) acc[k] = 0.0f;

    const float delta2 = D.robust_delta * D.robust_delta;
    auto accumulate = [&](bool valid, float pix, float piy, float piz, float pjx, float pjy, float pjz) {
        const float m = valid ? 1.0f : 0.0f;
        float wix, wiy, wiz, wjx, wjy, wjz;
        xform_point(Ti, pix, piy, piz, wix, wiy, wiz);
        xform_point(Tj, pjx, pjy, pjz, wjx, wjy, wjz);
        wix = m != 0.0f ? wix : 0.0f; wiy = m != 0.0f ? wiy : 0.0f; wiz = m != 0.0f ? wiz : 0.0f;
        wjx = m != 0.0f ? wjx : 0.0f; wjy = m != 0.0f ? wjy : 0.0f; wjz = m != 0.0f ? wjz : 0.0f;
        const float rx = wix - wjx, ry = wiy - wjy, rz = wiz - wjz;
        const float e2 = rx * rx + ry * ry + rz * rz;
#ifdef BTBA_EXACT_DIV
        const float rho = m * ((e2 <= delta2) ? 1.0f : D.robust_delta / sqrtf(e2));
#else
        const float rho = m * ((e2 <= delta2) ? 1.0f : D.robust_delta * __builtin_amdgcn_rsqf(e2));
#endif
        acc[0] += m;
        acc[1] += wix; acc[2] += wiy; acc[3] += wiz;
        acc[4] += wjx; acc[5] += wjy; acc[6] += wjz;
        acc[7] += wix * wix; acc[8] += wix * wiy; acc[9] += wix * wiz; acc[10] += wiy * wiy; acc[11] += wiy * wiz; acc[12] += wiz * wiz;
        acc[13] += wjx * wjx; acc[14] += wjx * wjy; acc[15] += wjx * wjz; acc[16] += wjy * wjy; acc[17] += wjy * wjz; acc[18] += wjz * wjz;
        acc[19] += wix * wjx; acc[20] += wix * wjy; acc[21] += wix * wjz;
        acc[22] += wiy * wjx; acc[23] += wiy * wjy; acc[24] += wiy * wjz;
        acc[25] += wiz * wjx; acc[26] += wiz * wjy; acc[27] += wiz * wjz;
        acc[28] += rho * rx; acc[29] += rho * ry; acc[30] += rho * rz;
        acc[31] += rho * (wiy * rz - wiz * ry); acc[32] += rho * (wiz * rx - wix * rz); acc[33] += rho * (wix * ry - wiy * rx);
        acc[34] += rho * (wjy * rz - wjz * ry); acc[35] += rho * (wjz * rx - wjx * rz); acc[36] += rho * (wjx * ry - wjy * rx);
        acc[37] += rho;
        acc[38] += rho * (wiy * wiy + wiz * wiz); acc[39] += rho * (wix * wix + wiz * wiz); acc[40] += rho * (wix * wix + wiy * wiy);
        acc[41] += rho * (wjy * wjy + wjz * wjz); acc[42] += rho * (wjx * wjx + wjz * wjz); acc[43] += rho * (wjx * wjx + wjy * wjy);
    };
    if (C24) {
        const float2 *cb = reinterpret_cast<const float2 *>(corr);
        const size_t e_base = (size_t)D.corr_entry0 + (size_t)b * (size_t)D.corr_stride;
        for (uint32_t e = lo + tid; e < hi; e += 2 * kBlock) {
            const uint32_t e2 = e + kBlock;
            const bool live2 = e2 < hi;
            const float2 *qa = cb + corr24_index(e_base + e), *qb = cb + corr24_index(e_base + (live2 ? e2 : e));
            const float2 a0 = ld_stream_f2<NT>(qa), a1 = ld_stream_f2<NT>(qa + 64), a2 = ld_stream_f2<NT>(qa + 128), b0 = ld_stream_f2<NT>(qb), b1 = ld_stream_f2<NT>(qb + 64), b2 = ld_stream_f2<NT>(qb + 128);
            accumulate(__float_as_uint(a0.x) != 0xFFFFFFFFu, a0.x, a0.y, a1.x, a1.y, a2.x, a2.y);
            accumulate(live2 && __float_as_uint(b0.x) != 0xFFFFFFFFu, b0.x, b0.y, b1.x, b1.y, b2.x, b2.y);
        }
    } else {
        const float4 *cb = corr + 2 * (size_t)b * D.corr_stride;
        bool misplaced = false;
        float2 *const c24 = D.corr24_out;
        const size_t e_out = (size_t)D.corr_entry0 + (size_t)b * (size_t)D.corr_stride;
        auto entry = [&](const float4 &q0, const float4 &q1, bool live, uint32_t e) {
            const bool valid = live && __float_as_uint(q0.x) != 0xFFFFFFFFu;
            misplaced |= valid & ((__float_as_uint(q0.x) != (uint32_t)fi) | (__float_as_uint(q0.y) != (uint32_t)fj));
            if (c24 && live) {
                float2 *o = c24 + corr24_index(e_out + e);
                o[0] = make_float2(valid ? q0.z : __uint_as_float(0xFFFFFFFFu), q0.w);
                o[64] = make_float2(q1.x, q1.y);
                o[128] = make_float2(q1.z, q1.w);
            }
            accumulate(valid, q0.z, q0.w, q1.x, q1.y, q1.z, q1.w);
        };
        for (uint32_t e = lo + tid; e < hi; e += 2 * kBlock) {
            const uint32_t e2 = e + kBlock;
            const bool live2 = e2 < hi;
            const uint32_t e2c = live2 ? e2 : e;
            const float4 a0 = ld_stream_f4<NT>(cb + 2 * (size_t)e), a1 = ld_stream_f4<NT>(cb + 2 * (size_t)e + 1), b0 = ld_stream_f4<NT>(cb + 2 * (size_t)e2c), b1 = ld_stream_f4<NT>(cb + 2 * (size_t)e2c + 1);
            entry(a0, a1, true, e);
            entry(b0, b1, live2, e2c);
        }
        if (D.order_flag && misplaced) atomicOr(D.order_flag, 1);
    }
    float *out = partials + ((unsigned)b * D.sp_stride + (unsigned)(D.atomic_sums ? p : p * D.sparse_chunks + chunk) * (unsigned)kSparseVals);
    block_reduce_store<kSparseVals, 4>(acc, red, out, D.atomic_sums ? 1 : D.publish ? 2 : 0);
}
__device__ __forceinline__ void sparse_block(const SolveDims &D, const float4 *__restrict__ corr, const uint32_t *__restrict__ pair_offsets,
                                             const float *__restrict__ T, float *__restrict__ partials, int chunk, int p, int b, float *red)
{
    if (D.corr24) { if (b >= D.corr_nt_from) sparse_block_impl<true, true>(D, corr, pair_offsets, T, partials, chunk, p, b, red); else sparse_block_impl<true, false>(D, corr, pair_offsets, T, partials, chunk, p, b, red); }
    else { if (b >= D.corr_nt_from) sparse_block_impl<false, true>(D, corr, pair_offsets, T, partials, chunk, p, b, red); else sparse_block_impl<false, false>(D, corr, pair_offsets, T, partials, chunk, p, b, red); }
}

__global__ void __launch_bounds__(256) k_pack_corr24(const uint4 *__restrict__ seg, const uint4 *__restrict__ src, float2 *__restrict__ dst, int *__restrict__ order_flag)
{
    const uint4 d = seg[blockIdx.y];
    const uint32_t e = blockIdx.x * 256u + threadIdx.x;
    if (e >= d.z) return;
    const uint4 a = src[2 * (size_t)(d.x + e)], b = src[2 * (size_t)(d.x + e) + 1];
    const bool valid = a.x != 0xFFFFFFFFu;
    if (valid && ((a.x != (d.w >> 16)) | (a.y != (d.w & 0xFFFFu)))) atomicOr(order_flag, 1);
    float2 *o = dst + corr24_index((size_t)(d.y + e));
    o[0] = make_float2(valid ? __uint_as_float(a.z) : __uint_as_float(0xFFFFFFFFu), __uint_as_float(a.w));
    o[64] = make_float2(__uint_as_float(b.x), __uint_as_float(b.y));
    o[128] = make_float2(__uint_as_float(b.z), __uint_as_float(b.w));
}
__global__ void __launch_bounds__(256) k_pack_corr24_batch(int n_frames, int n_pairs, int64_t corr_stride, const uint32_t *__restrict__ pair_offsets,
                                                          const uint4 *__restrict__ src, float2 *__restrict__ dst, int *__restrict__ order_flag)
{
    const int p = blockIdx.y, b = blockIdx.z;
    const uint32_t *off = pair_offsets + (size_t)b * (n_pairs + 1);
    const uint32_t seg0 = off[p], len = off[p + 1] - seg0, e = blockIdx.x * 256u + threadIdx.x;
    if (e >= len) return;
    int fi, fj;
    pair_from_index(p, n_frames, fi, fj);
    const size_t at = (size_t)b * (size_t)corr_stride + seg0 + e;
    const uint4 a = src[2 * at], q = src[2 * at + 1];
    const bool valid = a.x != 0xFFFFFFFFu;
    if (order_flag && valid && ((a.x != (uint32_t)fi) | (a.y != (uint32_t)fj))) atomicOr(order_flag, 1);
    float2 *o = dst + corr24_index(at);
    o[0] = make_float2(valid ? __uint_as_float(a.z) : __uint_as_float(0xFFFFFFFFu), __uint_as_float(a.w));
    o[64] = make_float2(__uint_as_float(q.x), __uint_as_float(q.y));
    o[128] = make_float2(__uint_as_float(q.z), __uint_as_float(q.w));
}

__global__ void __launch_bounds__(kBlock) k_sparse_sweep(SolveDims D, const float4 *__restrict__ corr, const uint32_t *__restrict__ pair_offsets,
                                                        const float *__restrict__ T, float *__restrict__ partials)
{
    __shared__ float red[kRedFloats];
    sparse_block(D, corr, pair_offsets, T, partials, blockIdx.x, blockIdx.y, blockIdx.z, red);
}

#ifdef BTBA_EXACT_DIV
__device__ __forceinline__ float fast_rcp(float x) { return 1.0f / x; }
__device__ __forceinline__ float fast_rsq(float x) { return 1.0f / sqrtf(x); }
#else
__device__ __forceinline__ float fast_rcp(float x) { return __builtin_amdgcn_rcpf(x); }
__device__ __forceinline__ float fast_rsq(float x) { return __builtin_amdgcn_rsqf(x); }
#endif

__device__ __forceinline__ unsigned xcd_remap(unsigned L, unsigned n)
{
    const unsigned q = n >> 3, r = n & 7u, xcd = L & 7u, slot = L >> 3;
    return xcd < r ? xcd * (q + 1) + slot : r * (q + 1) + (xcd - r) * q + slot;
}

struct DenseCtx {
    Mat4 Tij;
    const float4 *cam_t, *nrm_t;
    float fx, fy, cx, cy, depth_min, depth_max, normal_thresh, dist2_thresh, delta, delta2, w_dense;
    int W, H;
};

struct PixelGeom {
    float qx, qy, qz, nqx, nqy, nqz;
    float c00, c10, c01, c11;
    int i00, i10, i01, i11;
    int xa, xb, ya, yb;
    bool valid;
};

__device__ __forceinline__ PixelGeom pixel_geom(const DenseCtx &C, const float4 &cs, const float4 &ns)
{
    PixelGeom g;
    g.valid = (cs.z > C.depth_min && cs.z < C.depth_max);
    const Mat4 &M = C.Tij;
    g.nqx = M.m[0] * ns.x + M.m[1] * ns.y + M.m[2] * ns.z;
    g.nqy = M.m[4] * ns.x + M.m[5] * ns.y + M.m[6] * ns.z;
    g.nqz = M.m[8] * ns.x + M.m[9] * ns.y + M.m[10] * ns.z;
    xform_point(M, cs.x, cs.y, cs.z, g.qx, g.qy, g.qz);
    const float rqz = fast_rcp(g.qz);
    float u = g.qx * C.fx * rqz + C.cx, v = g.qy * C.fy * rqz + C.cy;
    g.valid = g.valid && (u > -0.5f) && (u < (float)C.W - 0.5f) && (v > -0.5f) && (v < (float)C.H - 0.5f);
    u = g.valid ? u : 0.0f; v = g.valid ? v : 0.0f;
    const float fx0 = floorf(u), fy0 = floorf(v);
    const int x0 = (int)fx0, y0 = (int)fy0;
    const float alpha = u - fx0, beta = v - fy0;
    const bool okx0 = (unsigned)x0 < (unsigned)C.W, okx1 = (unsigned)(x0 + 1) < (unsigned)C.W;
    const bool oky0 = (unsigned)y0 < (unsigned)C.H, oky1 = (unsigned)(y0 + 1) < (unsigned)C.H;
    const int xa = min(max(x0, 0), C.W - 1), xb = min(max(x0 + 1, 0), C.W - 1);
    const int ya = min(max(y0, 0), C.H - 1), yb = min(max(y0 + 1, 0), C.H - 1);
    g.i00 = ya * C.W + xa; g.i10 = ya * C.W + xb; g.i01 = yb * C.W + xa; g.i11 = yb * C.W + xb;
    g.xa = xa; g.xb = xb; g.ya = ya; g.yb = yb;
    const float a0 = okx0 ? 1.0f - alpha : 0.0f, a1 = okx1 ? alpha : 0.0f;
    const float wr = a0 + a1;
    const float b0 = (oky0 && wr > 0.0f) ? 1.0f - beta : 0.0f, b1 = (oky1 && wr > 0.0f) ? beta : 0.0f;
    const float ww = b0 + b1;
    const float k = (ww > 0.0f) ? fast_rcp(wr) * fast_rcp(ww) : 0.0f;
    const float k0 = k * b0, k1 = k * b1;
    g.c00 = k0 * a0; g.c10 = k0 * a1; g.c01 = k1 * a0; g.c11 = k1 * a1;
    return g;
}

__device__ __forceinline__ void pixel_accumulate(const DenseCtx &C, const PixelGeom &g,
                                                 const float4 &c00, const float4 &c10, const float4 &c01, const float4 &c11,
                                                 const float4 &n00, const float4 &n10, const float4 &n01, const float4 &n11,
                                                 float (&acc)[kDenseVals])
{
    const float cix = g.c00 * c00.x + g.c10 * c10.x + g.c01 * c01.x + g.c11 * c11.x;
    const float ciy = g.c00 * c00.y + g.c10 * c10.y + g.c01 * c01.y + g.c11 * c11.y;
    const float ciz = g.c00 * c00.z + g.c10 * c10.z + g.c01 * c01.z + g.c11 * c11.z;
    const float nix = g.c00 * n00.x + g.c10 * n10.x + g.c01 * n01.x + g.c11 * n11.x;
    const float niy = g.c00 * n00.y + g.c10 * n10.y + g.c01 * n01.y + g.c11 * n11.y;
    const float niz = g.c00 * n00.z + g.c10 * n10.z + g.c01 * n01.z + g.c11 * n11.z;
    const float dx = g.qx - cix, dy = g.qy - ciy, dz = g.qz - ciz;
    const float dist2 = dx * dx + dy * dy + dz * dz;
    const float dn = g.nqx * nix + g.nqy * niy + g.nqz * niz;
    const bool ok = g.valid & (ciz > C.depth_min) & (ciz < C.depth_max) & (dn >= C.normal_thresh) & (dist2 <= C.dist2_thresh);
    const unsigned keep = ok ? 0xFFFFFFFFu : 0u;
    auto masked = [keep](float x) { return __uint_as_float(__float_as_uint(x) & keep); };
    const float res = masked(-(dx * nix + dy * niy + dz * niz));
    const float e = res * res;
    const float wgt = masked(C.w_dense * ((e <= C.delta2) ? 1.0f : C.delta * fast_rsq(e)));
    const float mx = masked(nix), my = masked(niy), mz = masked(niz);
    const float a[6] = { -mx, -my, -mz, my * g.qz - mz * g.qy, mz * g.qx - mx * g.qz, mx * g.qy - my * g.qx };
    int k = 0;
#pragma unroll
    for (int r = 0; r < 6; r++) {
        const float wa = wgt * a[r];
#pragma unroll
        for (int c = r; c < 6; c++) acc[k++] += wa * a[c];
        acc[21 + r] += wa * res;
    }
    acc[27] += masked(1.0f);
}

#ifdef BTBA_REFERENCE_ORDER
__device__ __attribute__((noinline)) bool bilinear4_reference(float x, float y, const float4 *__restrict__ img, int W, int H, float out[4])
{
#pragma clang fp contract(off)
    const int p00x = (int)floorf(x), p00y = (int)floorf(y);
    const int p01x = p00x, p01y = p00y + 1, p10x = p00x + 1, p10y = p00y, p11x = p00x + 1, p11y = p00y + 1;
    const float alpha = x - (float)p00x, beta = y - (float)p00y;
    const float MINF = -INFINITY;
    float s0[4] = { 0.f, 0.f, 0.f, 0.f }, w0 = 0.0f;
    if ((unsigned)p00x < (unsigned)W && (unsigned)p00y < (unsigned)H) { const float4 q = img[(size_t)p00y * W + p00x]; const float v[4] = { q.x, q.y, q.z, q.w }; if (v[0] != MINF) { for (int k = 0; k < 4; k++) s0[k] += (1.0f - alpha) * v[k]; w0 += (1.0f - alpha); } }
    if ((unsigned)p10x < (unsigned)W && (unsigned)p10y < (unsigned)H) { const float4 q = img[(size_t)p10y * W + p10x]; const float v[4] = { q.x, q.y, q.z, q.w }; if (v[0] != MINF) { for (int k = 0; k < 4; k++) s0[k] += alpha * v[k]; w0 += alpha; } }
    float s1[4] = { 0.f, 0.f, 0.f, 0.f }, w1 = 0.0f;
    if ((unsigned)p01x < (unsigned)W && (unsigned)p01y < (unsigned)H) { const float4 q = img[(size_t)p01y * W + p01x]; const float v[4] = { q.x, q.y, q.z, q.w }; if (v[0] != MINF) { for (int k = 0; k < 4; k++) s1[k] += (1.0f - alpha) * v[k]; w1 += (1.0f - alpha); } }
    if ((unsigned)p11x < (unsigned)W && (unsigned)p11y < (unsigned)H) { const float4 q = img[(size_t)p11y * W + p11x]; const float v[4] = { q.x, q.y, q.z, q.w }; if (v[0] != MINF) { for (int k = 0; k < 4; k++) s1[k] += alpha * v[k]; w1 += alpha; } }
    float ss[4] = { 0.f, 0.f, 0.f, 0.f }, ww = 0.0f;
    if (w0 > 0.0f) { for (int k = 0; k < 4; k++) ss[k] += (1.0f - beta) * (s0[k] / w0); ww += (1.0f - beta); }
    if (w1 > 0.0f) { for (int k = 0; k < 4; k++) ss[k] += beta * (s1[k] / w1); ww += beta; }
    if (ww > 0.0f) { for (int k = 0; k < 4; k++) out[k] = ss[k] / ww; return true; }
    out[0] = out[1] = out[2] = out[3] = MINF;
    return false;
}

__device__ __attribute__((noinline)) void pixel_reference_order(const DenseCtx &C, float dist_thresh, const float4 &cs, const float4 &ns, float (&acc)[kDenseVals])
{
#pragma clang fp contract(off)
    const float *T = C.Tij.m;
    bool ok = (cs.z > C.depth_min && cs.z < C.depth_max) && (ns.x != -INFINITY);
    float q[3] = { 0.f, 0.f, 0.f }, ci[4] = { 0.f, 0.f, 0.f, 0.f }, ni[4] = { 0.f, 0.f, 0.f, 0.f };
    if (ok) {
        const float nt[4] = { T[0] * ns.x + T[1] * ns.y + T[2] * ns.z + T[3] * ns.w, T[4] * ns.x + T[5] * ns.y + T[6] * ns.z + T[7] * ns.w,
                              T[8] * ns.x + T[9] * ns.y + T[10] * ns.z + T[11] * ns.w, T[12] * ns.x + T[13] * ns.y + T[14] * ns.z + T[15] * ns.w };
        q[0] = T[0] * cs.x + T[1] * cs.y + T[2] * cs.z + T[3] * 1.0f;
        q[1] = T[4] * cs.x + T[5] * cs.y + T[6] * cs.z + T[7] * 1.0f;
        q[2] = T[8] * cs.x + T[9] * cs.y + T[10] * cs.z + T[11] * 1.0f;
        const float u = q[0] * C.fx / q[2] + C.cx, v = q[1] * C.fy / q[2] + C.cy;
        const int sx = (int)roundf(u), sy = (int)roundf(v);
        ok = sx >= 0 && sy >= 0 && sx < C.W && sy < C.H;
        if (ok) {
            bilinear4_reference(u, v, C.cam_t, C.W, C.H, ci);
            ok = ci[2] > C.depth_min && ci[2] < C.depth_max;
        }
        if (ok) {
            bilinear4_reference(u, v, C.nrm_t, C.W, C.H, ni);
            ok = ni[0] != -INFINITY;
        }
        if (ok) {
            const float d[3] = { q[0] - ci[0], q[1] - ci[1], q[2] - ci[2] };
            const float dist = sqrtf(d[0] * d[0] + d[1] * d[1] + d[2] * d[2]);
            const float dNormal = nt[0] * ni[0] + nt[1] * ni[1] + nt[2] * ni[2] + nt[3] * ni[3];
            ok = dNormal >= C.normal_thresh && dist <= dist_thresh;
        }
    }
    if (!ok) return;
    const float dx = q[0] - ci[0], dy = q[1] - ci[1], dz = q[2] - ci[2];
    const float res = -(dx * ni[0] + dy * ni[1] + dz * ni[2]);
    const float e = res * res;
    const float wgt = C.w_dense * ((e <= C.delta2) ? 1.0f : C.delta / sqrtf(e));
// ... 499 lines not shown
        const float nix = fma_nd(c11, z11.y, fma_nd(c01, z01.y, fma_nd(c00, z00.y, c10 * z10.y)));
        const float niy = fma_nd(c11, z11.z, fma_nd(c01, z01.z, fma_nd(c00, z00.z, c10 * z10.z)));
        const float niz = fma_nd(c11, z11.w, fma_nd(c01, z01.w, fma_nd(c00, z00.w, c10 * z10.w)));
        const float dx = qx - cix, dy = qy - ciy, dz = qz - ciz;
        const float dist2 = fma_nd(dz, dz, fma_nd(dx, dx, dy * dy));
        const float dn = fma_nd(nqz, niz, fma_nd(nqx, nix, nqy * niy));
        const bool ok = valid & ((__float_as_uint(ciz) - C.zmin_bits) < C.zrange_bits) & (dn >= C.normal_thresh) & (dist2 <= C.dist2_thresh);
        const unsigned keep = opaque_vgpr(ok ? 0xFFFFFFFFu : 0u);
        auto masked = [keep](float x) { return __uint_as_float(__float_as_uint(x) & keep); };
        const float res = masked(fma_nd(dz, niz, fma_nd(dx, nix, dy * niy)));
        const float wgt = min_raw_s(C.wdelta * fast_rsq(res * res), C.w_dense);
        const float mx = masked(nix), my = masked(niy), mz = masked(niz);
        const float a[6] = { mx, my, mz, my * qz - mz * qy, mz * qx - mx * qz, mx * qy - my * qx };
        int k = 0;
        typedef float f2v __attribute__((ext_vector_type(2)));
        f2v pr[6];
#pragma unroll
        for (int r = 0; r < 6; r++) { pr[r] = (f2v){ wgt * a[r], a[r] }; asm volatile("" : "+v"(pr[r])); }
        f2v rr = (f2v){ wgt, res };
        asm volatile("" : "+v"(rr));
#pragma unroll
        for (int r = 0; r < 6; r++) {
#pragma unroll
            for (int c = r; c < 6; c++) acc[k++] += pr[r].x * pr[c].y;
            acc[21 + r] += pr[r].x * rr.y;
        }
        acc[27] += masked(1.0f);
    };

    if (WALK == 2) {
        const int lane = (int)tid & 63, wave = __builtin_amdgcn_readfirstlane((int)tid >> 6);
        n_live = __builtin_amdgcn_readfirstlane(n_live);
        if (D.live_blocks && tid == 0) atomicAdd(D.live_blocks, (unsigned long long)n_live);
        const unsigned lx = (unsigned)lane & 7u, ly = (unsigned)lane >> 3;
        const unsigned lane_px = ly * (unsigned)D.width + lx;
        const unsigned ox_l = 16u * lx, oy_l = 16u * ly + 16u * (unsigned)D.width;
        unsigned lane_off16 = 16u * lane_px;
        constexpr unsigned kBlockStep = 128u;
        const int nt = (n_live > wave) ? (n_live - wave + kBlock / 64 - 1) / (kBlock / 64) : 0;
        int list_chunk = 0;
        unsigned list_reg = nt > 0 ? blist[wave + (kBlock / 64) * min(lane, nt - 1)] : 0u;
        auto fetch = [&](int i, unsigned &code, float4 &zs) {
            const int idx = min(i, nt - 1);
            if ((idx >> 6) != list_chunk) { list_chunk = idx >> 6; list_reg = blist[wave + (kBlock / 64) * min(64 * list_chunk + lane, nt - 1)]; }
            code = (unsigned)__builtin_amdgcn_readlane((int)list_reg, idx & 63);
            asm volatile("" : "+v"(lane_off16));
            zs = gather16_imm<0>(reinterpret_cast<const char *>(zn_s) + (size_t)(16u * ((code >> 16) * 8u * (unsigned)D.width + (code & 0xFFFFu) * 8u)), lane_off16);
        };
        auto work = [&](const float4 &zs, unsigned code) { pixel(zs, ox_l + kBlockStep * (code & 0xFFFFu), oy_l + kBlockStep * (code >> 16)); };
        if (nt > 0) {
            unsigned code_a, code_b = 0u;
            float4 zs_a, zs_b = make_float4(0.f, 0.f, 0.f, 0.f);
            fetch(0, code_a, zs_a);
            for (int i = 0;;) {
                fetch(i + 1, code_b, zs_b);
                work(zs_a, code_a);
                if (++i >= nt) break;
                fetch(i + 1, code_a, zs_a);
                work(zs_b, code_b);
                if (++i >= nt) break;
            }
        }
    } else {
        const int n_src = LISTS ? valid_counts[slot_s] : D.npix;
        const uint32_t *list = LISTS ? valid_lists + slot_s * (size_t)D.npix : nullptr;
        const int per = (n_src + D.dense_tiles - 1) / D.dense_tiles;
        const int lo = min(n_src, per * tile), hi = min(n_src, per * (tile + 1));
        const float inv_w = 1.0f / (float)D.width;
        int t = lo + (int)tid;
        int s_n = (t < hi) ? (LISTS ? (int)list[t] : t) : 0;
        const unsigned w4 = 4u * (unsigned)D.width;
        unsigned px4 = 4u * (unsigned)(s_n % D.width), py4 = 4u * (unsigned)(s_n / D.width) + w4;
        const unsigned step_x4 = 4u * (unsigned)(kBlock % D.width), step_y4 = 4u * (unsigned)(kBlock / D.width);
        float4 zs_n = make_float4(0.f, 0.f, 0.f, 0.f);
        if (t < hi) zs_n = zn_s[s_n];
        for (; t < hi; t += kBlock) {
            const float4 zs = zs_n;
            const int s = s_n;
            const int tn = min(t + (int)kBlock, hi - 1);
            s_n = LISTS ? (int)list[tn] : tn; zs_n = zn_s[s_n];
            unsigned ox, oy;
            if (!LISTS) {
                ox = px4; oy = py4;
                px4 += step_x4; py4 += step_y4;
                if (px4 >= w4) { px4 -= w4; py4 += 4u; }
            } else {
                const float sf = (float)s;
                const float pyf = floorf((sf + 0.5f) * inv_w);
                ox = (unsigned)(4.0f * (sf - pyf * (float)D.width)); oy = (unsigned)(4.0f * pyf + C.ybase4);
            }
            pixel(zs, 4u * ox, 4u * oy);
        }
    }
    float *out = partials + ((unsigned)b * D.dp_stride + (unsigned)(D.atomic_sums ? p : p * D.dense_tiles + tile) * (unsigned)kDenseVals);
    dense_epilogue<true>(acc, red, out, D.atomic_sums ? 1 : D.publish ? 2 : 0);
}

template <bool SIMPLE, bool LISTS>
__global__ void __launch_bounds__(kBlock, 5) k_dense_sweep_zn(SolveDims D, const float4 *__restrict__ zn, const int2 *__restrict__ dense_pairs,
                                                             const float *__restrict__ T, const float *__restrict__ Tinv, float *__restrict__ partials,
                                                             const uint32_t *__restrict__ valid_lists, const int *__restrict__ valid_counts)
{
    __shared__ float red[kRedFloats];
    extern __shared__ __attribute__((aligned(16))) float zn_lut[];
    const unsigned L = xcd_remap(blockIdx.x, gridDim.x);
    const int tile = (int)(L % (unsigned)D.dense_tiles);
    const int p = (int)((L / (unsigned)D.dense_tiles) % (unsigned)D.n_dense_pairs);
    const int b = (int)(L / ((unsigned)D.dense_tiles * (unsigned)D.n_dense_pairs));
    if (SIMPLE && LISTS) dense_block_pinhole<1>(D, zn, p, T, Tinv, partials, tile, b, red, valid_lists, valid_counts, zn_lut);
    else if (SIMPLE && D.walk_blocks) dense_block_pinhole<2>(D, zn, p, T, Tinv, partials, tile, b, red, valid_lists, valid_counts, zn_lut);
    else if (SIMPLE) dense_block_pinhole<0>(D, zn, p, T, Tinv, partials, tile, b, red, valid_lists, valid_counts, zn_lut);
    else dense_block_zn<false, LISTS>(D, zn, dense_pairs[p], T, Tinv, partials, tile, p, b, red, valid_lists, valid_counts, zn_lut);
}

__global__ void __launch_bounds__(kBlock, 3) k_dense_sweep(SolveDims D, const float4 *__restrict__ campos, const float4 *__restrict__ normals,
                                                              const int2 *__restrict__ dense_pairs, const float *__restrict__ T, const float *__restrict__ Tinv,
                                                              float *__restrict__ partials)
{
    __shared__ float red[kRedFloats];
    const unsigned L = xcd_remap(blockIdx.x, gridDim.x);
    const int tile = (int)(L % (unsigned)D.dense_tiles);
    const int p = (int)((L / (unsigned)D.dense_tiles) % (unsigned)D.n_dense_pairs);
    const int b = (int)(L / ((unsigned)D.dense_tiles * (unsigned)D.n_dense_pairs));
    dense_block(D, campos, normals, dense_pairs[p], T, Tinv, partials, tile, p, b, red);
}

#ifndef BTBA_FUSED_WAVES
#define BTBA_FUSED_WAVES 3
#endif
template <int LAYOUT>
__device__ __forceinline__ void fused_item(const SolveDims &D, unsigned n_d, unsigned n_s, unsigned g,
                                           const float4 *__restrict__ campos, const float4 *__restrict__ normals,
                                           const int2 *__restrict__ dense_pairs, const float *__restrict__ T, const float *__restrict__ Tinv,
                                           float *__restrict__ dense_partials,
                                           const float4 *__restrict__ corr, const uint32_t *__restrict__ pair_offsets, float *__restrict__ sparse_partials,
                                           const uint32_t *__restrict__ valid_lists, const int *__restrict__ valid_counts, float *red, float *zn_lut)
{
    const unsigned G = n_d + n_s, xcd = g & 7u, slot = g >> 3;
    const unsigned qd = n_d >> 3, rd = n_d & 7u;
    const unsigned Gx = (G - xcd + 7u) >> 3, ndx = qd + (xcd < rd ? 1u : 0u), nsx = Gx - ndx;
    unsigned sparse_base = 0;
    for (unsigned y = 0; y < xcd; y++) sparse_base += ((G - y + 7u) >> 3) - (qd + (y < rd ? 1u : 0u));
    const unsigned nst = (nsx * (unsigned)D.sparse_tail_256) >> 8, nsi = nsx - nst, Gi = ndx + nsi;
    const unsigned Rx0 = nsi ? Gi / nsi : 0xFFFFFFFFu;
    const unsigned Rx = (nsi && Rx0 >= 4u && !(Rx0 & 1u)) ? Rx0 - 1u : Rx0;
    const bool in_tail = slot >= Gi;
    const bool is_sparse = in_tail || (nsi && (slot % Rx == 0u) && (slot / Rx < nsi));
    const unsigned sparse_local = in_tail ? nsi + (slot - Gi) : slot / Rx;
    if (is_sparse) {
        const unsigned i = sparse_base + sparse_local;
        const int chunk = (int)(i % (unsigned)D.sparse_chunks);
        const int p = (int)((i / (unsigned)D.sparse_chunks) % (unsigned)D.n_pairs);
        const int b = (int)(i / ((unsigned)D.sparse_chunks * (unsigned)D.n_pairs));
        sparse_block(D, corr, pair_offsets, T, sparse_partials, chunk, p, b, red);
    } else {
        const unsigned before = nsi ? min(nsi, (slot + Rx - 1u) / Rx) : 0u;
        const unsigned dl = slot - before;
        const unsigned L = (xcd < rd ? xcd * (qd + 1u) : rd * (qd + 1u) + (xcd - rd) * qd) + dl;
        const int b = (int)(L / ((unsigned)D.dense_tiles * (unsigned)D.n_dense_pairs));
        const unsigned Lb = L - (unsigned)b * (unsigned)D.dense_tiles * (unsigned)D.n_dense_pairs;
        const int tile = D.tile_major ? (int)(Lb / (unsigned)D.n_dense_pairs) : (int)(Lb % (unsigned)D.dense_tiles);
        int p = D.tile_major ? (int)(Lb % (unsigned)D.n_dense_pairs) : (int)(Lb / (unsigned)D.dense_tiles);
        if (LAYOUT == 1 && D.walk_blocks) dense_block_pinhole<2>(D, campos, p, T, Tinv, dense_partials, tile, b, red, valid_lists, valid_counts, zn_lut);
        else if (LAYOUT == 1) dense_block_pinhole<0>(D, campos, p, T, Tinv, dense_partials, tile, b, red, valid_lists, valid_counts, zn_lut);
        else if (LAYOUT == 3) dense_block_pinhole<1>(D, campos, p, T, Tinv, dense_partials, tile, b, red, valid_lists, valid_counts, zn_lut);
        else {
            const int4 w = D.dense_work[p];
            const int2 ij = make_int2(w.x, w.y);
            p = w.z;
            if (LAYOUT == 0) dense_block(D, campos, normals, ij, T, Tinv, dense_partials, tile, p, b, red);
            else if (LAYOUT == 2) dense_block_zn<false, false>(D, campos, ij, T, Tinv, dense_partials, tile, p, b, red, valid_lists, valid_counts, zn_lut);
            else dense_block_zn<false, true>(D, campos, ij, T, Tinv, dense_partials, tile, p, b, red, valid_lists, valid_counts, zn_lut);
        }
    }
}

#define BTBA_FUSED_ITEM_ARGS D, n_d, n_s, g, campos, normals, dense_pairs, T, Tinv, dense_partials, corr, pair_offsets, sparse_partials, valid_lists, valid_counts, red, zn_lut
template <int LAYOUT>
__global__ void __launch_bounds__(kBlock, BTBA_FUSED_WAVES) k_fused_sweeps(SolveDims D, unsigned n_d, unsigned n_s,
                                                           const float4 *__restrict__ campos, const float4 *__restrict__ normals,
                                                           const int2 *__restrict__ dense_pairs, const float *__restrict__ T, const float *__restrict__ Tinv,
                                                           float *__restrict__ dense_partials,
                                                           const float4 *__restrict__ corr, const uint32_t *__restrict__ pair_offsets, float *__restrict__ sparse_partials,
                                                           const uint32_t *__restrict__ valid_lists, const int *__restrict__ valid_counts)
{
    __shared__ float red[kRedFloats];
    extern __shared__ __attribute__((aligned(16))) float zn_lut[];
    const unsigned g = blockIdx.x;
    fused_item<LAYOUT>(BTBA_FUSED_ITEM_ARGS);
}

#undef BTBA_FUSED_ITEM_ARGS

__device__ __forceinline__ float sym3(const float *m, int r, int c) { if (r > c) { const int t = r; r = c; c = t; } return m[r * 3 - r * (r - 1) / 2 + (c - r)]; }
__device__ __forceinline__ float skew(const float *v, int r, int c)
{
    if (r == c) return 0.0f;
    const int k = 3 - r - c;
    const float s = ((c - r + 3) % 3 == 1) ? -1.0f : 1.0f;
    return s * v[k];
}

__device__ __forceinline__ float sparse_diag_entry(const float *rec, int e, int r, int c)
{
    const float *s = rec + 1 + 3 * e, *M = rec + 7 + 6 * e;
    const int br = r / 3, bc = c / 3, rr = r % 3, cc = c % 3;
    if (br == 0 && bc == 0) return rr == cc ? rec[0] : 0.0f;
    if (br == 0 && bc == 1) return -skew(s, rr, cc);
    if (br == 1 && bc == 0) return skew(s, rr, cc);
    const float tr = M[0] + M[3] + M[5];
    return (rr == cc ? tr : 0.0f) - sym3(M, rr, cc);
}
__device__ __forceinline__ float sparse_cross_entry(const float *rec, int r, int c)
{
    const float *si = rec + 1, *sj = rec + 4, *Mij = rec + 19;
    const int br = r / 3, bc = c / 3, rr = r % 3, cc = c % 3;
    if (br == 0 && bc == 0) return rr == cc ? rec[0] : 0.0f;
    if (br == 0 && bc == 1) return -skew(sj, rr, cc);
    if (br == 1 && bc == 0) return skew(si, rr, cc);
    const float tr = Mij[0] + Mij[4] + Mij[8];
    return (rr == cc ? tr : 0.0f) - Mij[cc * 3 + rr];
}

__host__ __device__ inline void sparse_entry_descriptor(bool cross, int r, int c, int out[4])
{
    const int br = r / 3, bc = c / 3, rr = r % 3, cc = c % 3;
    int i1 = 0, i2 = 0, es = 0;
    int c1 = 0, c2 = 0;
    const int k = 3 - rr - cc;
    const int sgn = ((cc - rr + 3) % 3 == 1) ? -1 : 1;
    if (br == 0 && bc == 0) { if (rr == cc) { i1 = 0; c1 = 1; } }
    else if (br == 0 && bc == 1) { if (rr != cc) { i1 = (cross ? 4 : 1) + k; c1 = -sgn; es = cross ? 0 : 3; } }
    else if (br == 1 && bc == 0) { if (rr != cc) { i1 = 1 + k; c1 = sgn; es = cross ? 0 : 3; } }
    else if (rr == cc) {
        const int a = (rr + 1) % 3, b = (rr + 2) % 3;
        const int dg[3] = { 0, 3, 5 };
        i1 = cross ? 19 + 4 * a : 7 + dg[a]; i2 = cross ? 19 + 4 * b : 7 + dg[b]; c1 = 1; c2 = 1; es = cross ? 0 : 6;
    } else {
        const int lo = rr < cc ? rr : cc, hi = rr < cc ? cc : rr;
        i1 = cross ? 19 + cc * 3 + rr : 7 + lo * 3 - lo * (lo - 1) / 2 + (hi - lo); c1 = -1; es = cross ? 0 : 6;
    }
    const int one = 0x3F800000, minus_one = (int)0xBF800000u;
    out[0] = i1 | (es << 8); out[1] = i2;
    out[2] = c1 > 0 ? one : c1 < 0 ? minus_one : 0; out[3] = c2 > 0 ? one : c2 < 0 ? minus_one : 0;
}

__device__ __forceinline__ float block_sum(float v, float *scratch)
{
    const float s = wave_sum_to_lane63(v);
    const int nw = blockDim.x >> 6;
    __syncthreads();
    if ((threadIdx.x & 63) == 63) scratch[threadIdx.x >> 6] = s;
    __syncthreads();
    float t = scratch[0];
    for (int w = 1; w < nw; w++) t += scratch[w];
    return t;
}

__device__ __forceinline__ float strided_sum(const float *__restrict__ q, int count, int stride)
{
    float s = 0.0f;
    int c = 0;
    for (; c + 4 <= count; c += 4) {
        const float a0 = q[(size_t)c * stride], a1 = q[(size_t)(c + 1) * stride], a2 = q[(size_t)(c + 2) * stride], a3 = q[(size_t)(c + 3) * stride];
        s += a0; s += a1; s += a2; s += a3;
    }
    for (; c < count; c++) s += q[(size_t)c * stride];
    return s;
}

__global__ void __launch_bounds__(256) k_big_reduce(SolveDims D, float *sparse_partials, float *dense_partials,
                                                    float *__restrict__ pairsum_global)
{
    const int b = blockIdx.y;
    const size_t ns = (size_t)D.n_pairs * kSparseVals, nd = (size_t)D.n_dense_pairs * kDenseVals;
    const size_t e = (size_t)blockIdx.x * 256 + threadIdx.x;
    if (e >= ns + nd) return;
    float *out = pairsum_global + (size_t)b * (ns + nd);
    float s = 0.0f;
    if (e < ns) {
        if (D.use_sparse) {
            const size_t p = e / kSparseVals, v = e - p * kSparseVals;
            float *q = sparse_partials + (size_t)b * D.sp_stride + (p * D.sparse_chunks) * kSparseVals + v;
            for (int c = 0; c < D.sparse_chunks; c++) s += q[(size_t)c * kSparseVals];
            if (D.atomic_sums) q[0] = 0.0f;
        }
    } else if (D.use_dense) {
        const size_t ed = e - ns, p = ed / kDenseVals, v = ed - p * kDenseVals;
        float *q = dense_partials + (size_t)b * D.dp_stride + (p * D.dense_tiles) * kDenseVals + v;
        for (int c = 0; c < D.dense_tiles; c++) s += q[(size_t)c * kDenseVals];
        if (D.atomic_sums) q[0] = 0.0f;
    }
    out[e] = s;
}

struct BigTasks { unsigned off_diag, diag, rhs, zero, total; };
__host__ __device__ inline BigTasks big_tasks(int N, int P, int ld)
{
    const unsigned n = 6u * (unsigned)N;
    auto pad = [](unsigned x) { return (x + 63u) & ~63u; };
    BigTasks t;
    t.off_diag = pad((unsigned)P * 36u);
    t.diag = pad((unsigned)(N - 1) * 36u * 8u);
    t.rhs = pad(n * 8u);
    t.zero = pad(6u * (unsigned)ld + (n - 6u) * (6u + (unsigned)ld - n));
    t.total = t.off_diag + t.diag + t.rhs + t.zero;
    return t;
// ... 598 lines not shown
#pragma unroll
            for (int j = 0; j < kMaxRows; j++) if (lane + 64 * j < n) vd[lane + 64 * j] = d_[j];
        }
        };
        if (n <= 128) pcg(std::integral_constant<int, 2>{}); else pcg(std::integral_constant<int, 4>{});
    }
    __syncthreads();

    BTBA_STAMP(3);
    for (int k = tid; k < N; k += nthr) {
        float *xk = (CHAIN ? io.x_out : const_cast<float *>(io.x_in)) + 6 * k;
        const float *xl = x_l + 6 * k;
        float rot[3] = { xl[0], xl[1], xl[2] }, trans[3] = { xl[3], xl[4], xl[5] };
        if (k > 0) {
            const float dW[3] = { vd[6 * k + 3], vd[6 * k + 4], vd[6 * k + 5] }, dT[3] = { vd[6 * k], vd[6 * k + 1], vd[6 * k + 2] };
            const Mat4 U = pose_to_matrix(dW, dT);
            const Mat4 C = load_mat4(vT + 16 * k);
            matrix_to_pose(mat_mul(U, C), rot, trans);
        }
        if (k > 0 || CHAIN) { xk[0] = rot[0]; xk[1] = rot[1]; xk[2] = rot[2]; xk[3] = trans[0]; xk[4] = trans[1]; xk[5] = trans[2]; }
        const Mat4 E = pose_to_matrix(rot, trans);
        store_mat4((CHAIN ? io.T_out : const_cast<float *>(io.T_in)) + 16 * k, E);
        if (io.poses_out) store_mat4(io.poses_out + 16 * k, E);
        store_mat4(io.Tinv_out + 16 * k, mat_inverse(E));
        if (tr) {
            for (int q = 0; q < 3; q++) { tr[D.tr_x + 6 * k + q] = rot[q]; tr[D.tr_x + 6 * k + 3 + q] = trans[q]; }
            for (int q = 0; q < 16; q++) tr[D.tr_T + 16 * k + q] = E.m[q];
            for (int q = 0; q < 3; q++) { tr[D.tr_delta + 6 * k + q] = vd[6 * k + 3 + q]; tr[D.tr_delta + 6 * k + 3 + q] = vd[6 * k + q]; }
        }
    }
    BTBA_STAMP(4);
#undef BTBA_STAMP
}

template <bool LDS_PAIRS, bool A_GLOBAL = false>
__global__ void __launch_bounds__(kSolveBlock) k_system_solve(SolveDims D, int iter,
                                                        float *sparse_partials, float *dense_partials,
                                                        const int2 *__restrict__ dense_pairs, const int *__restrict__ adj_off, const int *__restrict__ adj,
                                                        float *__restrict__ x, float *__restrict__ T, float *__restrict__ Tinv,
                                                        float *__restrict__ pairsum_global, float *__restrict__ trace, float *__restrict__ A_scratch = nullptr,
                                                        float *__restrict__ poses_out = nullptr, const int *__restrict__ solve_tab = nullptr)
{
    extern __shared__ __attribute__((aligned(16))) float lds[];
    const size_t b = blockIdx.x;
    const int N = D.n_frames, n = 6 * N, ld = 4 * (((n + 3) / 4) | 1);
    SolveIO io;
    io.sparse_partials = sparse_partials + b * D.sp_stride; io.dense_partials = dense_partials + b * D.dp_stride;
    io.x_in = io.x_out = x + b * D.x_stride;
    io.T_in = io.T_out = T + b * D.pose_stride; io.Tinv_out = Tinv + b * D.pose_stride;
    io.poses_out = poses_out ? poses_out + 16 * b * N : nullptr;
    io.pairsum_global = pairsum_global ? pairsum_global + b * ((size_t)D.n_pairs * kSparseVals + (size_t)D.n_dense_pairs * kDenseVals) : nullptr;
    io.A_scratch = A_scratch ? A_scratch + b * (size_t)(n + 2) * ld : nullptr;
    io.trace = trace ? trace + b * (size_t)D.n_gn * D.trace_record : nullptr;
    io.stamps = nullptr;
    system_solve_body<LDS_PAIRS, A_GLOBAL, false, kSolveBlock>(D, iter, (int)threadIdx.x, lds, io, dense_pairs, adj_off, adj, solve_tab);
}


constexpr int kChainMaxParts = 2;
constexpr size_t kChainLdsBytes = 26560;
constexpr int kChainMaxFrames = 21;
__host__ __device__ inline size_t chain_region_floats(int n_frames) { const size_t P = (size_t)n_frames * (n_frames - 1) / 2, na = 6 * (size_t)n_frames - 6; return P * kSparseVals > na * (na + 1) / 2 ? P * kSparseVals : na * (na + 1) / 2; }
struct ChainDims {
    int n_iter;
    int n_inst;
    unsigned inst_per_xcd;
    unsigned items_d, items_s;
    unsigned sparse_period;
    unsigned group;
    int *flags;
    const int *published;
    int *arrivals;
    int *error;
    long long timeout_ticks;
    size_t pose_ring, x_ring;
    size_t sp_ring, dp_ring;
    size_t ps_size, A_size;
    unsigned long long *trace;
    unsigned long long *stamps;
    int solve_prio;
    int last_solve_external;
    int debug_skip;
};

__device__ __forceinline__ void chain_wait_ge(const int *word, int want, const ChainDims &Cn)
{
    const bool lane0 = (item_tid() & 63u) == 0u;
    auto poll = [&]() {
        int v = 0;
        if (lane0) v = __hip_atomic_load(word, __ATOMIC_RELAXED, __HIP_MEMORY_SCOPE_AGENT);
        return __builtin_amdgcn_readfirstlane(v);
    };
    if (poll() >= want) return;
    const long long t0 = wall_clock64();
    for (;;) {
        __builtin_amdgcn_s_sleep(16);
        if (poll() >= want) return;
        if (wall_clock64() - t0 > Cn.timeout_ticks) {
            if (lane0) __hip_atomic_store(Cn.error, 1, __ATOMIC_RELAXED, __HIP_MEMORY_SCOPE_SYSTEM);
            return;
        }
    }
}

template <int LAYOUT>
__global__ void __launch_bounds__(kBlock, BTBA_FUSED_WAVES) k_chain(SolveDims D, ChainDims Cn, const float4 *__restrict__ zn,
                                                    float *T, float *Tinv, float *x, float *dense_partials,
                                                    const float4 *__restrict__ corr, const uint32_t *__restrict__ pair_offsets, float *sparse_partials,
                                                    const uint32_t *__restrict__ valid_lists, const int *__restrict__ valid_counts,
                                                    const int2 *__restrict__ dense_pairs, const int *__restrict__ adj_off, const int *__restrict__ adj,
                                                    const int *__restrict__ solve_tab, float *pairsum_global, float *A_scratch, float *poses_out)
{
    __shared__ float red[kRedFloats];
    extern __shared__ __attribute__((aligned(16))) float dyn_lds[];
    const unsigned g = blockIdx.x, xcd = g & 7u, sg = g >> 3;
    const unsigned n_sweep = Cn.items_d + Cn.items_s, slots_per_inst = n_sweep + 1u, per_iter = Cn.inst_per_xcd * slots_per_inst;
    const unsigned it = sg / per_iter, s = sg - it * per_iter;
    unsigned k = s / slots_per_inst, r = s - k * slots_per_inst;
    if (Cn.group > 1u) {
        const unsigned per_group = Cn.group * slots_per_inst, gi = s / per_group, rg = s - gi * per_group;
        unsigned kg, rr;
        if (rg < Cn.group * Cn.items_d) { kg = rg / Cn.items_d; rr = rg - kg * Cn.items_d; }
        else if (rg < Cn.group * n_sweep) { const unsigned q = rg - Cn.group * Cn.items_d; kg = q / Cn.items_s; rr = Cn.items_d + (q - kg * Cn.items_s); }
        else { kg = rg - Cn.group * n_sweep; rr = n_sweep; }
        k = gi * Cn.group + kg; r = rr;
    }
    const int b = (int)(xcd * Cn.inst_per_xcd + k);
    if (b >= Cn.n_inst) return;
    const unsigned tid = item_tid();
    const unsigned long long t_start = Cn.trace ? (unsigned long long)wall_clock64() : 0ull;
    unsigned long long t_wait = t_start;
    int kind;
    if (r < n_sweep) {
        bool is_sparse;
        unsigned idx;
        if (Cn.sparse_period >= 2u) {
            const unsigned q = r / Cn.sparse_period, m = r - q * Cn.sparse_period;
            is_sparse = (m == Cn.sparse_period - 1u) && (q < Cn.items_s);
            idx = is_sparse ? q : r - min(q, Cn.items_s);
        } else {
            is_sparse = r >= Cn.items_d;
            idx = is_sparse ? r - Cn.items_d : r;
        }
        const float *T_it = T + (size_t)it * Cn.pose_ring, *Tinv_it = Tinv + (size_t)it * Cn.pose_ring;
        if (it > 0u) {
            const int seen = (Cn.debug_skip & 1) ? 1 : *as_const(Cn.published + ((size_t)it * Cn.n_inst + b) * 16);
            if (seen == 0) chain_wait_ge(Cn.flags + b, (int)it, Cn);
        }
        asm volatile("" : "+s"(T_it), "+s"(Tinv_it) :: "memory");
        if (Cn.trace) t_wait = (unsigned long long)wall_clock64();
        kind = is_sparse ? 1 : 0;
        if (is_sparse) {
            const int chunk = (int)(idx % (unsigned)D.sparse_chunks), p = (int)(idx / (unsigned)D.sparse_chunks);
            sparse_block(D, corr, pair_offsets, T_it, sparse_partials + (size_t)it * Cn.sp_ring, chunk, p, b, red);
        } else {
            const int tile = D.tile_major ? (int)(idx / (unsigned)D.n_dense_pairs) : (int)(idx % (unsigned)D.dense_tiles);
            const int p = D.tile_major ? (int)(idx % (unsigned)D.n_dense_pairs) : (int)(idx / (unsigned)D.dense_tiles);
            float *dp_it = dense_partials + (size_t)it * Cn.dp_ring;
            if (LAYOUT == 1 && D.walk_blocks) dense_block_pinhole<2>(D, zn, p, T_it, Tinv_it, dp_it, tile, b, red, valid_lists, valid_counts, dyn_lds);
            else if (LAYOUT == 1) dense_block_pinhole<0>(D, zn, p, T_it, Tinv_it, dp_it, tile, b, red, valid_lists, valid_counts, dyn_lds);
            else dense_block_pinhole<1>(D, zn, p, T_it, Tinv_it, dp_it, tile, b, red, valid_lists, valid_counts, dyn_lds);
        }
        if (tid < 64u && !(Cn.debug_skip & 2)) {
            asm volatile("s_waitcnt vmcnt(0)" ::: "memory");
            if (tid == 0u) __hip_atomic_fetch_add(Cn.arrivals + (size_t)it * Cn.n_inst + b, 1, __ATOMIC_RELAXED, __HIP_MEMORY_SCOPE_AGENT);
        }
    } else {
        kind = 2;
        if ((Cn.debug_skip & 8) || (Cn.last_solve_external && (int)it == Cn.n_iter - 1)) return;
        if (tid < 64u && !(Cn.debug_skip & 4)) {
            chain_wait_ge(Cn.arrivals + (size_t)it * Cn.n_inst + b, (int)n_sweep, Cn);
            if (tid == 0u) __builtin_amdgcn_fence(__ATOMIC_ACQUIRE, "agent");
        }
        __syncthreads();
        if (Cn.trace) t_wait = (unsigned long long)wall_clock64();
        const int N = D.n_frames;
        const size_t ib = (size_t)it * Cn.n_inst + b;
        SolveIO io;
        io.sparse_partials = sparse_partials + (size_t)it * Cn.sp_ring + (size_t)b * D.sp_stride;
        io.dense_partials = dense_partials + (size_t)it * Cn.dp_ring + (size_t)b * D.dp_stride;
        io.x_in = x + (size_t)it * Cn.x_ring + (size_t)b * D.x_stride; io.x_out = x + (size_t)(it + 1u) * Cn.x_ring + (size_t)b * D.x_stride;
        io.T_in = T + (size_t)it * Cn.pose_ring + (size_t)b * D.pose_stride;
        io.T_out = T + (size_t)(it + 1u) * Cn.pose_ring + (size_t)b * D.pose_stride;
        io.Tinv_out = Tinv + (size_t)(it + 1u) * Cn.pose_ring + (size_t)b * D.pose_stride;
        io.poses_out = ((int)it == Cn.n_iter - 1) ? poses_out + 16 * (size_t)b * N : nullptr;
        io.pairsum_global = pairsum_global + ib * Cn.ps_size;
        io.A_scratch = A_scratch + ib * Cn.A_size;
        io.trace = nullptr;
        io.stamps = Cn.stamps ? Cn.stamps + 8 * ib : nullptr;
        if (Cn.solve_prio == 1) __builtin_amdgcn_s_setprio(1);
        else if (Cn.solve_prio == 2) __builtin_amdgcn_s_setprio(2);
        else if (Cn.solve_prio == 3) __builtin_amdgcn_s_setprio(3);
        system_solve_body<false, false, true, kBlock>(D, (int)it, (int)tid, dyn_lds, io, dense_pairs, adj_off, adj, solve_tab);
        __syncthreads();
        if (tid == 0u && !(Cn.debug_skip & 64)) {
            __builtin_amdgcn_fence(__ATOMIC_RELEASE, "agent");
            asm volatile("s_waitcnt vmcnt(0)" ::: "memory");
            __hip_atomic_store(Cn.flags + b, (int)it + 1, __ATOMIC_RELAXED, __HIP_MEMORY_SCOPE_AGENT);
            __hip_atomic_store(const_cast<int *>(Cn.published) + ((size_t)(it + 1u) * Cn.n_inst + b) * 16, 1, __ATOMIC_RELAXED, __HIP_MEMORY_SCOPE_AGENT);
        }
    }
    if (Cn.trace && tid == 0u) {
        unsigned hw, xcc;
        asm volatile("s_getreg_b32 %0, hwreg(HW_REG_HW_ID)\n s_getreg_b32 %1, hwreg(HW_REG_XCC_ID)" : "=s"(hw), "=s"(xcc));
        unsigned long long *q = Cn.trace + 4 * (size_t)g;
        q[0] = t_start; q[1] = t_wait; q[2] = (unsigned long long)wall_clock64();
        q[3] = (unsigned long long)kind | ((unsigned long long)it << 8) | ((unsigned long long)b << 16) | ((unsigned long long)(hw & 0xFFFFu) << 32) | ((unsigned long long)(xcc & 0xFu) << 48);
    }
}

__global__ void __launch_bounds__(256) k_chain_poison(const int *__restrict__ error, float *__restrict__ poses, int n)
{
    const int e = blockIdx.x * 256 + threadIdx.x;
    if (e < n && __hip_atomic_load(error, __ATOMIC_RELAXED, __HIP_MEMORY_SCOPE_SYSTEM) != 0) poses[e] = __int_as_float(0x7FC00000);
}

__global__ void __launch_bounds__(64) k_prepare_strided(int total, int n_frames, int pose_stride, int x_stride, const float *__restrict__ poses,
                                                        float *__restrict__ x, float *__restrict__ T, float *__restrict__ Tinv)
{
    const int idx = blockIdx.x * blockDim.x + threadIdx.x;
    if (idx >= total) return;
    const int b = idx / n_frames, f = idx - b * n_frames;
    const Mat4 M = load_mat4(poses + 16 * (size_t)idx);
    float rot[3], trans[3];
    matrix_to_pose(M, rot, trans);
    float *o = x + (size_t)b * x_stride + 6 * f;
    o[0] = rot[0]; o[1] = rot[1]; o[2] = rot[2]; o[3] = trans[0]; o[4] = trans[1]; o[5] = trans[2];
    const Mat4 E = pose_to_matrix(rot, trans);
    store_mat4(T + (size_t)b * pose_stride + 16 * f, E);
    store_mat4(Tinv + (size_t)b * pose_stride + 16 * f, mat_inverse(E));
}

}
```

bundletrack_amd/optimizer.py:

```python
from __future__ import annotations

import ctypes as C
from dataclasses import dataclass

import numpy as np

from . import _lib
from ._lib import ENTRYJ_DTYPE, Params, Stats, TraceLayout, check, default_params, lib


def _torch():
    import torch
    return torch


class Workspace:

    def __init__(self, stream: int | None = None, use_torch_stream: bool = True):
        h = C.c_void_p()
        if stream is None and use_torch_stream:
            torch = _torch()
            if not torch.cuda.is_available():
                raise RuntimeError("bundletrack_amd needs a GPU: torch.cuda.is_available() is False (no CPU fallback)")
            check(lib().btba_workspace_create_on_stream(C.byref(h), C.c_void_p(torch.cuda.current_stream().cuda_stream)), "btba_workspace_create_on_stream")
        else:
            check(lib().btba_workspace_create(C.byref(h), C.c_void_p(stream) if stream else None), "btba_workspace_create")
        self._h = h

    @property
    def handle(self):
        return self._h

    def sync(self):
        check(lib().btba_workspace_sync(self._h), "btba_workspace_sync")

    def set_option(self, option: int, value: int):
        check(lib().btba_workspace_set_option(self._h, int(option), int(value)), "btba_workspace_set_option")

    def wait_stream(self, stream: int | None):
        check(lib().btba_workspace_wait_stream(self._h, C.c_void_p(stream) if stream else None), "btba_workspace_wait_stream")

    def signal_stream(self, stream: int | None):
        check(lib().btba_workspace_signal_stream(self._h, C.c_void_p(stream) if stream else None), "btba_workspace_signal_stream")

    def live_blocks(self) -> int:
        v = C.c_uint64(0)
        check(lib().btba_workspace_live_blocks(self._h, C.byref(v)), "btba_workspace_live_blocks")
        return int(v.value)

    def collect_stats(self) -> dict:
        s = Stats()
        check(lib().btba_collect_stats(self._h, C.byref(s)), "btba_collect_stats")
        return s.as_dict()

    def close(self):
        if self._h:
            lib().btba_workspace_destroy(self._h)
            self._h = C.c_void_p()

    def __del__(self):
        try:
            self.close()
        except Exception:
            pass


def _dev_ptr(t, what: str = "tensor"):
    if t is None:
        return None
    if not t.is_cuda:
        raise ValueError(f"{what}: expected a CUDA tensor, got device {t.device}")
    if not t.is_contiguous():
        raise ValueError(f"{what}: expected a contiguous (row-major) tensor, got shape {tuple(t.shape)} with strides {tuple(t.stride())}; call .contiguous()")
    if t.element_size() not in (1, 4):
        raise ValueError(f"{what}: expected float32 / int32 / uint8 data, got {t.dtype}")
    return t.data_ptr()


def _ptr_array(tensors, what: str = "frame map"):
    arr = (C.c_void_p * len(tensors))()
    for k, t in enumerate(tensors):
        arr[k] = _dev_ptr(t, f"{what} {k}")
    return arr


class OptimizerGpu:

    def __init__(self, yml: dict | None = None, workspace: Workspace | None = None, keyed_correspondences: bool = False, **overrides):
        self.params = default_params()
        self.keyed_correspondences = bool(keyed_correspondences)
        if yml:
            b, p = yml.get("bundle", {}), yml.get("p2p", {})
            if "num_iter_outter" in b: self.params.n_gn_iters = int(b["num_iter_outter"])
            if "num_iter_inner" in b: self.params.n_pcg_iters = int(b["num_iter_inner"])
            if "robust_delta" in b: self.params.robust_delta = float(b["robust_delta"])
            if "image_downscale" in b: self.params.image_downscale = float(b["image_downscale"])
            if "max_dist" in p: self.params.dense_dist_thresh = float(p["max_dist"])
            if "max_normal_angle" in p:
                self.params.dense_normal_thresh = float(np.cos(float(p["max_normal_angle"]) / 180.0 * np.pi))
        for k, v in overrides.items():
            setattr(self.params, k, v)
        self.workspace = workspace
        self.last_stats: dict | None = None

    def optimizeFrames(self, global_corres, n_match_per_pair, n_frames, H, W, depths_gpu, colors_gpu, normals_gpu, poses, K,
                       dense_pairs=None, frame_keys=None):
        del colors_gpu
        corr = np.ascontiguousarray(global_corres, ENTRYJ_DTYPE)
        if len(depths_gpu) != n_frames or len(normals_gpu) != n_frames:
            raise ValueError("need one depth and one normal buffer per frame")
        for d, n in zip(depths_gpu, normals_gpu):
            if not (d.is_cuda and n.is_cuda and d.dtype == _torch().float32 and n.dtype == _torch().float32 and d.is_contiguous() and n.is_contiguous()):
                raise ValueError("depth/normal buffers must be contiguous float32 CUDA tensors")
            if d.numel() != H * W or n.numel() != 4 * H * W:
                raise ValueError("depth must hold H*W floats and normals H*W float4")
        Kf = np.ascontiguousarray(K, np.float32).reshape(9)
        nm = None if n_match_per_pair is None else np.ascontiguousarray(n_match_per_pair, np.int32).reshape(-1)
        if nm is not None and nm.shape[0] != n_frames * (n_frames - 1) // 2:
            nm = None
        P = np.ascontiguousarray(poses, np.float32).reshape(n_frames, 16).copy()
        dp = None
        if dense_pairs is not None:
            dp = np.ascontiguousarray(dense_pairs, np.int32).reshape(-1, 2)
        st = Stats()
        dptr, nptr = _ptr_array(depths_gpu), _ptr_array(normals_gpu)
        head = (self.workspace.handle if self.workspace else None, C.byref(self.params), n_frames, H, W, Kf.ctypes.data,
                corr.ctypes.data if corr.shape[0] else None, corr.shape[0], nm.ctypes.data if nm is not None else None,
                C.cast(dptr, C.c_void_p), C.cast(nptr, C.c_void_p))
        tail = (dp.ctypes.data if dp is not None else None, dp.shape[0] if dp is not None else 0, P.ctypes.data, C.byref(st))
        if frame_keys is None:
            rc = lib().btba_optimize_frames(*head, *tail)
        else:
            keys = np.ascontiguousarray(frame_keys, np.uint64)
            if keys.shape != (n_frames,):
                raise ValueError("need one key per frame")
            if self.workspace is None:
                raise ValueError("the persistent frame cache lives in a Workspace: construct OptimizerGpu(workspace=...)")
            flags0 = self.params.flags
            if self.keyed_correspondences:
                self.params.flags |= _lib.FLAG_KEYED_CORR
            try:
                rc = lib().btba_optimize_frames_keyed(*head, keys.ctypes.data, *tail)
            finally:
                self.params.flags = flags0
        check(rc, "btba_optimize_frames")
        self.last_stats = st.as_dict()
        out = P.reshape(n_frames, 4, 4)
        if isinstance(poses, np.ndarray):
            poses[...] = out.reshape(poses.shape)
        else:
            for k in range(n_frames):
                if isinstance(poses[k], np.ndarray):
                    poses[k][...] = out[k]
                else:
                    poses[k] = out[k].copy()
        return poses


def frame_cache_evict(ws: Workspace, key: int) -> None:
    check(lib().btba_frame_cache_evict(ws.handle, C.c_uint64(int(key))), "btba_frame_cache_evict")


def frame_cache_clear(ws: Workspace) -> None:
    check(lib().btba_frame_cache_clear(ws.handle), "btba_frame_cache_clear")


def build_cache(ws: Workspace, depths_gpu, normals_gpu, H, W, K, image_downscale=4.0):
    torch = _torch()
    N = len(depths_gpu)
    Wd, Hd = int(W / image_downscale), int(H / image_downscale)
    dev = depths_gpu[0].device
    campos = torch.empty((N, Hd, Wd, 4), dtype=torch.float32, device=dev)
    normals = torch.empty((N, Hd, Wd, 4), dtype=torch.float32, device=dev)
    nvalid = torch.zeros((N,), dtype=torch.int32, device=dev)
    intr = np.zeros(4, np.float32)
    Kf = np.ascontiguousarray(K, np.float32).reshape(9)
    dptr, nptr = _ptr_array(depths_gpu), _ptr_array(normals_gpu)
    check(lib().btba_build_cache(ws.handle, N, H, W, Kf.ctypes.data, float(image_downscale), C.cast(dptr, C.c_void_p), C.cast(nptr, C.c_void_p),
                                 _dev_ptr(campos, "campos"), _dev_ptr(normals, "normals"), _dev_ptr(nvalid, "nvalid"), intr.ctypes.data), "btba_build_cache")
    return campos, normals, nvalid, intr


def build_cache_zn(ws: Workspace, depths_gpu, normals_gpu, H, W, K, image_downscale=4.0):
    torch = _torch()
    N = len(depths_gpu)
    Wd, Hd = int(W / image_downscale), int(H / image_downscale)
    dev = depths_gpu[0].device
    zn = torch.empty((N, Hd, Wd, 4), dtype=torch.float32, device=dev)
    nvalid = torch.zeros((N,), dtype=torch.int32, device=dev)
    intr = np.zeros(4, np.float32)
    Kf = np.ascontiguousarray(K, np.float32).reshape(9)
    dptr, nptr = _ptr_array(depths_gpu), _ptr_array(normals_gpu)
    check(lib().btba_build_cache_zn(ws.handle, N, H, W, Kf.ctypes.data, float(image_downscale), C.cast(dptr, C.c_void_p), C.cast(nptr, C.c_void_p),
                                    _dev_ptr(zn, "zn"), _dev_ptr(nvalid, "nvalid"), intr.ctypes.data), "btba_build_cache_zn")
    return zn, nvalid, intr


def pack_zn(ws: Workspace, campos, normals):
    torch = _torch()
    zn = torch.empty_like(campos)
    check(lib().btba_pack_zn(ws.handle, campos.numel() // 4, _dev_ptr(campos, "campos"), _dev_ptr(normals, "normals"), _dev_ptr(zn, "zn")), "btba_pack_zn")
# ... 200 lines not shown
```

include/btba.h:

```cpp
#ifndef BTBA_H_
#define BTBA_H_

#include <stdint.h>

#ifdef __cplusplus
extern "C" {
#endif

#define BTBA_VERSION 105

#if defined(__GNUC__)
#define BTBA_API __attribute__((visibility("default")))
#else
#define BTBA_API
#endif

enum {
    BTBA_OK       = 0,
    BTBA_EINVAL   = 1,
    BTBA_EHIP     = 2,
    BTBA_ENUMERIC = 3,
    BTBA_ENOMEM   = 4,
    BTBA_ESCHED   = 5
};

typedef struct btba_entryj {
    uint32_t imgIdx_i;
    uint32_t imgIdx_j;
    float pos_i[3];
    float pos_j[3];
} btba_entryj;

enum {
    BTBA_PAIRS_TARGET_LOWER      = 0,
    BTBA_PAIRS_TARGET_MORE_VALID = 1,
    BTBA_PAIRS_EXPLICIT          = 2,
    BTBA_PAIRS_TARGET_HIGHER     = 3
};

enum {
    BTBA_REDUCE_DETERMINISTIC = 0,
    BTBA_REDUCE_ATOMIC        = 1
};

enum {
    BTBA_FLAG_TRACE         = 1,
    BTBA_FLAG_TIME_KERNELS  = 2,
    BTBA_FLAG_TIME_SAMPLED  = 2048,
    BTBA_FLAG_OVERLAP       = 32,
    BTBA_FLAG_NO_FUSE       = 64,
    BTBA_FLAG_FLOAT4_CACHE  = 256,
    BTBA_FLAG_KEYED_CORR    = 4096,
    BTBA_FLAG_NO_COMPACTION = 512,
    BTBA_FLAG_COMPACTION    = 1024
};

typedef struct btba_params {
    int32_t n_gn_iters;
    int32_t n_pcg_iters;
    float   robust_delta;
    float   dense_dist_thresh;
    float   dense_normal_thresh;
    float   depth_min;
    float   depth_max;
    float   weight_sparse;
    float   weight_dense_depth;
    float   image_downscale;
    int32_t pair_policy;
    int32_t dense_tiles;
    int32_t sparse_chunks;
    int32_t flags;
    int32_t reduction_mode;
    const float *weights_sparse_per_iter;
    const float *weights_dense_per_iter;
    int32_t n_weights_per_iter;
} btba_params;

#define BTBA_MAX_FRAMES 85
#define BTBA_MAX_FRAMES_LDS 31

typedef struct btba_stats {
    int32_t n_instances, n_frames, n_pairs, n_dense_pairs;
    int64_t n_corr;
    int32_t dense_tiles, sparse_chunks;
    float ms_total;
    float ms_upload;
    float ms_cache;
    float ms_solve;
    float ms_dense_sweep;
    float ms_sparse_sweep;
    float ms_system_solve;
    int32_t n_dense_launches, n_sparse_launches, n_solve_launches;
    int64_t bytes_dense_alg;
    int64_t bytes_sparse_alg;
    int32_t fused_sweeps;
    int32_t cache_frames_built;
    int32_t corr_pairs_uploaded;
    int32_t chain_iterations;
} btba_stats;

typedef struct btba_trace_layout {
    int64_t record_floats;
    int64_t off_x, off_T, off_rhs, off_precond, off_pcg, off_delta, off_dense_pair, off_A, off_clk;
} btba_trace_layout;

typedef struct btba_workspace btba_workspace;

BTBA_API void btba_params_default(btba_params *p);
BTBA_API const char *btba_strerror(int status);
BTBA_API int btba_last_hip_error(void);
BTBA_API int btba_version(void);

BTBA_API int btba_workspace_create(btba_workspace **out, void *stream);
BTBA_API int btba_workspace_create_on_stream(btba_workspace **out, void *stream);
BTBA_API void btba_workspace_destroy(btba_workspace *ws);
BTBA_API int btba_workspace_sync(btba_workspace *ws);

enum {
    BTBA_OPT_DENSE_ORDER          = 1,
    BTBA_OPT_TILE_MAJOR           = 2,
    BTBA_OPT_BLOCK_WALK           = 3,
    BTBA_OPT_BLOCK_SKIP           = 4,
    BTBA_OPT_BIG_ASSEMBLY         = 5,
    BTBA_OPT_OVERLAP_GROUPS       = 6,
    BTBA_OPT_OVERLAP_EQUAL_PRIO   = 7,
    BTBA_OPT_SPARSE_TAIL          = 9,
    BTBA_OPT_KEYED_CORR_MIN_BYTES = 8,
    BTBA_OPT_CHAIN                = 10,
    BTBA_OPT_CHAIN_SPARSE_PERIOD  = 11,
    BTBA_OPT_CHAIN_TIMEOUT_MS     = 12,
    BTBA_OPT_RELAYOUT             = 14,
    BTBA_OPT_CORR_NONTEMPORAL     = 15,
    BTBA_OPT_COUNT_LIVE           = 13,
    BTBA_OPT_SOLVE_SMALL          = 16
};
BTBA_API int btba_workspace_set_option(btba_workspace *ws, int option, int64_t value);
BTBA_API int btba_workspace_live_blocks(btba_workspace *ws, uint64_t *blocks);
BTBA_API int btba_workspace_wait_stream(btba_workspace *ws, void *stream);
BTBA_API int btba_workspace_signal_stream(btba_workspace *ws, void *stream);

BTBA_API int btba_optimize_frames(btba_workspace *ws, const btba_params *params,
                         int n_frames, int H, int W, const float *K_rowmajor,
                         const btba_entryj *corres_host, uint32_t n_corres, const int *n_match_per_pair,
                         const float *const *depth_dev, const float *const *normal_dev,
                         const int32_t *dense_pairs, int n_dense_pairs,
                         float *poses_rowmajor, btba_stats *stats);

BTBA_API int btba_optimize_frames_keyed(btba_workspace *ws, const btba_params *params,
                         int n_frames, int H, int W, const float *K_rowmajor,
                         const btba_entryj *corres_host, uint32_t n_corres, const int *n_match_per_pair,
                         const float *const *depth_dev, const float *const *normal_dev, const uint64_t *frame_keys,
                         const int32_t *dense_pairs, int n_dense_pairs,
                         float *poses_rowmajor, btba_stats *stats);
BTBA_API int btba_frame_cache_clear(btba_workspace *ws);
BTBA_API int btba_frame_cache_evict(btba_workspace *ws, uint64_t frame_key);

BTBA_API int btba_build_cache(btba_workspace *ws, int n_frames, int H, int W, const float *K_rowmajor,
                     float image_downscale, const float *const *depth_dev, const float *const *normal_dev,
                     float *campos_dev, float *normals_dev, int32_t *n_valid_dev, float *intr_out);

BTBA_API int btba_solve_batch(btba_workspace *ws, const btba_params *params,
                     int n_instances, int n_frames, int Hd, int Wd, const float *intr,
                     const float *campos_dev, const float *normals_dev,
                     const btba_entryj *corr_dev, int64_t corr_stride,
                     const uint32_t *pair_offsets_dev, uint32_t max_corr_per_pair,
                     const int32_t *dense_pairs, int n_dense_pairs,
                     float *poses_dev, float *trace_dev);
BTBA_API int btba_solve_cached(btba_workspace *ws, const btba_params *params, int n_frames, int Hd, int Wd, const float *intr,
                     const float *campos_dev, const float *normals_dev,
                     const btba_entryj *corr_dev, uint32_t n_corr,
                     const uint32_t *pair_offsets_dev, uint32_t max_corr_per_pair,
                     const int32_t *dense_pairs, int n_dense_pairs,
                     float *poses_dev, float *trace_dev);
BTBA_API int btba_collect_stats(btba_workspace *ws, btba_stats *stats);

BTBA_API void btba_trace_layout_get(int n_frames, int n_dense_pairs, int n_pcg_iters, btba_trace_layout *out);

BTBA_API int btba_bucket_correspondences(const btba_entryj *in, uint32_t n, int n_frames,
                                btba_entryj *out_sorted, uint32_t *out_offsets);

BTBA_API int btba_matrices_to_poses(btba_workspace *ws, int n, const float *T_dev, float *x_dev);
BTBA_API int btba_poses_to_matrices(btba_workspace *ws, int n, const float *x_dev, float *T_dev, float *Tinv_dev);

BTBA_API int btba_process_depth(btba_workspace *ws, int H, int W, const float *depth_in_dev, float *depth_out_dev,
                                int erode_radius, float erode_diff, float erode_ratio,
                                int bf_radius, float sigma_d, float sigma_r);

BTBA_API int btba_depth_to_normals(btba_workspace *ws, int H, int W, const float *K_rowmajor,
                                   const float *depth_dev, float *normals_dev, float *xyz_dev);

BTBA_API int btba_build_cache_zn(btba_workspace *ws, int n_frames, int H, int W, const float *K_rowmajor,
                                 float image_downscale, const float *const *depth_dev, const float *const *normal_dev,
                                 float *zn_dev , int32_t *n_valid_dev, float *intr_out);
BTBA_API int btba_pack_zn(btba_workspace *ws, int64_t n_pixels_total, const float *campos_dev, const float *normals_dev, float *zn_dev);
BTBA_API int btba_solve_batch_zn(btba_workspace *ws, const btba_params *params, int n_instances, int n_frames,
                                 int H, int W, const float *K_rowmajor, const float *zn_dev,
                                 const btba_entryj *corr_dev, int64_t corr_stride,
                                 const uint32_t *pair_offsets_dev, uint32_t max_corr_per_pair,
                                 const int32_t *dense_pairs, int n_dense_pairs, float *poses_dev, float *trace_dev);

typedef struct btba_zn_aux {
    const float *block_ranges;
    const uint32_t *valid_lists;
    const int32_t *valid_counts;
    const float *corr24;
} btba_zn_aux;
BTBA_API int btba_zn_block_ranges(btba_workspace *ws, int n_frames_total, int Hd, int Wd, const float *zn_dev, float *ranges_dev);
BTBA_API int btba_zn_valid_lists(btba_workspace *ws, int n_frames_total, int Hd, int Wd, const float *zn_dev, uint32_t *lists_dev, int32_t *counts_dev);
BTBA_API int btba_pack_correspondences24(btba_workspace *ws, int n_instances, int n_frames, const btba_entryj *corr_dev, int64_t corr_stride,
                                         const uint32_t *pair_offsets_dev, uint32_t max_corr_per_pair, float *corr24_dev, int32_t *order_flag_dev);
BTBA_API int btba_solve_batch_zn_aux(btba_workspace *ws, const btba_params *params, int n_instances, int n_frames,
                                     int H, int W, const float *K_rowmajor, const float *zn_dev, const btba_zn_aux *aux,
                                     const btba_entryj *corr_dev, int64_t corr_stride,
                                     const uint32_t *pair_offsets_dev, uint32_t max_corr_per_pair,
                                     const int32_t *dense_pairs, int n_dense_pairs, float *poses_dev, float *trace_dev);

enum { BTBA_RANSAC_REFERENCE_SVD = 0, BTBA_RANSAC_HORN = 1,
       BTBA_RANSAC_DRAW_HASH = 0x100  };
BTBA_API int btba_ransac_pairs_ex(btba_workspace *ws, int hypothesis, int device_resident, int n_pairs, const float *ptsA, const float *ptsB,
                                  const int32_t *n_pts, int n_trials, float dist_thres, const int32_t *samples, uint64_t seed,
                                  int32_t *inlier_ids_out, int32_t *n_inliers_out, int32_t *best_trial_out, float *best_pose_out,
                                  int32_t *trial_counts_out, float *trial_poses_out);
BTBA_API int btba_ransac_pairs(btba_workspace *ws, int n_pairs, const float *ptsA_host, const float *ptsB_host, const int32_t *n_pts,
                               int n_trials, float dist_thres, const int32_t *samples_host, uint64_t seed,
                               int32_t *inlier_ids_out, int32_t *n_inliers_out, int32_t *best_trial_out, float *best_pose_out,
                               int32_t *trial_counts_out, float *trial_poses_out);

BTBA_API int btba_ransac_reference_uniforms(uint64_t seed, int n_trials, float *u_out);

typedef struct btba_match_params {
    int32_t k;
    int32_t mutual;
    float max_dist_neighbor;
    float cos_max_normal_neighbor;
    float max_dist_no_neighbor;
    float cos_max_normal_no_neighbor;
    float min_z;
} btba_match_params;

typedef struct btba_match {
    int32_t idx_a, idx_b;
    float dist;
    int32_t dir;
    float ptA_cam[3], ptB_cam[3];
} btba_match;

BTBA_API void btba_match_params_default(btba_match_params *p);
BTBA_API int btba_match_capacity(const btba_match_params *params, int n_frames, int H, int W, int D, const int32_t *n_kpts,
                                 int n_pairs, const int32_t *pairs, int64_t *capacity_out);
BTBA_API int btba_match_pairs(btba_workspace *ws, const btba_match_params *params, int device_resident, int n_frames, int H, int W,
                              const float *K_rowmajor, const float *const *desc_dev, int D, const float *const *kpts_dev,
                              const int32_t *n_kpts, const float *const *depth_dev, const float *const *normal_dev, const float *poses,
                              const int32_t *frame_ids, int n_pairs, const int32_t *pairs,
                              btba_match *matches_out, float *ptsA_model_out, float *ptsB_model_out, int32_t *n_out);

typedef struct btba_mask_params {
    int32_t largest_component_hull;
    int32_t dilate;
} btba_mask_params;
BTBA_API void btba_mask_params_default(btba_mask_params *p);
BTBA_API int btba_apply_masks(btba_workspace *ws, const btba_mask_params *params, int n_frames, int H, int W,
                              const uint8_t *const *mask_dev, float *const *depth_dev, float *const *normal_dev,
                              uint8_t *const *color_dev, uint8_t *const *mask_out_dev, float *roi_out);

typedef struct btba_detector_params {
    int32_t out_size;
} btba_detector_params;
BTBA_API void btba_detector_params_default(btba_detector_params *p);
BTBA_API int btba_detector_transform(const btba_detector_params *params, const float *roi, float *fwd, float *bwd);
BTBA_API int btba_detector_inputs(btba_workspace *ws, const btba_detector_params *params, int n_frames, int H, int W,
                                  const uint8_t *const *color_dev, const float *roi_host, uint8_t *bgr_out_dev, float *gray_out_dev);
BTBA_API int btba_detector_keypoints_to_image(btba_workspace *ws, const btba_detector_params *params, int n_frames, const float *roi_host,
                                              const float *const *kpts_in_dev, const int32_t *n_kpts, float *const *kpts_out_dev);

#define BTBA_EVAL_MAX_POINTS (1 << 22)
BTBA_API int btba_pose_errors(btba_workspace *ws, int device_resident,
                              int n_models, const float *const *model_pts_dev, const int32_t *n_pts,
                              int n_evals, const int32_t *model_index,
                              const float *poses_pred, const float *poses_gt,
                              float *add_out, float *adds_out);

typedef struct btba_mappoints btba_mappoints;
typedef struct btba_corres_params {
    int32_t n_trials;
    float dist_thres;
    int32_t hypothesis;
    int32_t pad;
    uint64_t seed;
} btba_corres_params;
BTBA_API int btba_mappoints_create(btba_workspace *ws, btba_mappoints **out);
// ... 28 lines not shown
```

Measured before the change: 209,800.

## Cache pose-invariant correspondence moments and transform them algebraically per iteration

The sparse residual kernel used to recompute 28 world-frame first and second moments of each correspondence chunk on every Gauss-Newton iteration. Now the first iteration stores centered camera-frame moments per chunk in a new workspace buffer. Later iterations rebuild the world-frame moments from the current poses in double precision, so each thread accumulates only the 16 pose-dependent robust terms. This cuts per-correspondence FMAs and register pressure, at the cost of an extra moments buffer, an extra block sync and a per-block transform step. It also adds a debug export of the sparse records.

```diff
diff --git a/bundletrack_amd/_lib.py b/bundletrack_amd/_lib.py
--- a/bundletrack_amd/_lib.py
+++ b/bundletrack_amd/_lib.py
@@ -21,6 +21,7 @@
 FLAG_OVERLAP, FLAG_NO_FUSE, FLAG_KEYED_CORR, FLAG_FLOAT4_CACHE, FLAG_NO_COMPACTION, FLAG_COMPACTION, FLAG_TIME_SAMPLED = 32, 64, 4096, 256, 512, 1024, 2048
 OPT_DENSE_ORDER, OPT_TILE_MAJOR, OPT_BLOCK_WALK, OPT_BLOCK_SKIP, OPT_BIG_ASSEMBLY, OPT_OVERLAP_GROUPS, OPT_OVERLAP_EQUAL_PRIO, OPT_KEYED_CORR_MIN_BYTES, OPT_SPARSE_TAIL = 1, 2, 3, 4, 5, 6, 7, 8, 9
 OPT_CHAIN, OPT_CHAIN_SPARSE_PERIOD, OPT_CHAIN_TIMEOUT_MS, OPT_COUNT_LIVE, OPT_RELAYOUT, OPT_CORR_NONTEMPORAL, OPT_SOLVE_SMALL = 10, 11, 12, 13, 14, 15, 16
+OPT_SPARSE_MOMENTS = 17
 
 ENTRYJ_DTYPE = np.dtype(
     [("imgIdx_i", "<u4"), ("imgIdx_j", "<u4"), ("pos_i", "<f4", (3,)), ("pos_j", "<f4", (3,))]
@@ -29,7 +30,7 @@
 EXPORTED_SYMBOLS = [
     "btba_params_default", "btba_strerror", "btba_last_hip_error", "btba_version",
     "btba_workspace_create", "btba_workspace_create_on_stream", "btba_workspace_destroy", "btba_workspace_sync",
-    "btba_workspace_wait_stream", "btba_workspace_signal_stream", "btba_workspace_set_option", "btba_workspace_live_blocks",
+    "btba_workspace_wait_stream", "btba_workspace_signal_stream", "btba_workspace_set_option", "btba_workspace_live_blocks", "btba_workspace_sparse_records",
     "btba_optimize_frames", "btba_optimize_frames_keyed", "btba_frame_cache_clear", "btba_frame_cache_evict", "btba_ransac_pairs", "btba_ransac_pairs_ex", "btba_ransac_reference_uniforms", "btba_build_cache", "btba_solve_batch", "btba_solve_cached", "btba_collect_stats",
     "btba_trace_layout_get", "btba_bucket_correspondences",
     "btba_matrices_to_poses", "btba_poses_to_matrices",
@@ -169,7 +170,7 @@
         L.btba_strerror.restype = C.c_char_p
         L.btba_strerror.argtypes = [C.c_int]
         for name in EXPORTED_SYMBOLS:
-            if "BTBA_LIB_PATH" in os.environ and name in ("btba_workspace_set_option", "btba_pack_correspondences24", "btba_workspace_live_blocks") and not hasattr(L, name):
+            if "BTBA_LIB_PATH" in os.environ and name in ("btba_workspace_set_option", "btba_pack_correspondences24", "btba_workspace_live_blocks", "btba_workspace_sparse_records") and not hasattr(L, name):
                 continue
             getattr(L, name)
         L.btba_workspace_create.argtypes = [C.POINTER(C.c_void_p), C.c_void_p]
@@ -181,6 +182,8 @@
             L.btba_workspace_set_option.argtypes = [C.c_void_p, C.c_int, C.c_int64]
         if hasattr(L, "btba_workspace_live_blocks"):
             L.btba_workspace_live_blocks.argtypes = [C.c_void_p, C.POINTER(C.c_uint64)]
+        if hasattr(L, "btba_workspace_sparse_records"):
+            L.btba_workspace_sparse_records.argtypes = [C.c_void_p, C.c_void_p, C.c_int64]
         L.btba_workspace_wait_stream.argtypes = [C.c_void_p, C.c_void_p]
         L.btba_workspace_signal_stream.argtypes = [C.c_void_p, C.c_void_p]
         L.btba_collect_stats.argtypes = [C.c_void_p, C.POINTER(Stats)]
diff --git a/bundletrack_amd/csrc/btba_api.hip b/bundletrack_amd/csrc/btba_api.hip
--- a/bundletrack_amd/csrc/btba_api.hip
+++ b/bundletrack_amd/csrc/btba_api.hip
@@ -71,6 +71,7 @@
     DevBuf chain_sync;
     DevBuf chain_trace;
     DevBuf corr24_tmp;
+    DevBuf sparse_mom;
     DevBuf live_blocks;
     bool count_live = false;
     int *chain_error = nullptr;
@@ -97,6 +98,7 @@
         int chain_timeout_ms = 500;
         int chain_solve_prio = 0;
         int chain_debug_skip = 0;
+        bool sparse_moments = true;
         bool solve_small = true;
         int prepare_keep_T = 0;
         int debug_lds_pad = 0;
@@ -261,6 +263,7 @@
         if (const char *e = std::getenv("BTBA_CHAIN_PERIOD")) t.chain_sparse_period = std::max(0, std::atoi(e));
         t.relayout = on("BTBA_RELAYOUT");
         t.solve_small = !on("BTBA_SOLVE_LEGACY");
+        if (const char *e = std::getenv("BTBA_SPARSE_MOMENTS")) t.sparse_moments = e[0] != '0';
         if (const char *e = std::getenv("BTBA_CORR_NT")) t.corr_nt = std::atoi(e);
         if (const char *e = std::getenv("BTBA_LLC_MB")) t.last_level_cache = (long long)std::atoll(e) << 20;
         if (const char *e = std::getenv("BTBA_CORR_NT_PARTIAL")) t.corr_nt_partial = std::atoi(e);
@@ -296,7 +299,7 @@
     for (auto e : ws->event_pool) (void)hipEventDestroy(e);
     DevBuf *bufs[] = { &ws->x, &ws->T, &ws->Tinv, &ws->sparse_part, &ws->dense_part, &ws->pairsum, &ws->dense_pairs, &ws->ptrs, &ws->big_A, &ws->solve_tab,
                        &ws->corr, &ws->offsets, &ws->poses, &ws->campos, &ws->normals, &ws->nvalid, &ws->valid_lists, &ws->valid_counts, &ws->block_ranges,
-                       &ws->chain_sync, &ws->chain_trace, &ws->live_blocks, &ws->corr24_tmp, &ws->pool_zn, &ws->pool_lists, &ws->pool_counts, &ws->pool_nvalid, &ws->pool_map, &ws->pool_ranges, &ws->ransac, &ws->ransac_u, &ws->match, &ws->mask, &ws->eval, &ws->corr_pool, &ws->corr_desc, &ws->corr_stage_dev, &ws->corr_lens, &ws->window };
+                       &ws->chain_sync, &ws->chain_trace, &ws->live_blocks, &ws->sparse_mom, &ws->corr24_tmp, &ws->pool_zn, &ws->pool_lists, &ws->pool_counts, &ws->pool_nvalid, &ws->pool_map, &ws->pool_ranges, &ws->ransac, &ws->ransac_u, &ws->match, &ws->mask, &ws->eval, &ws->corr_pool, &ws->corr_desc, &ws->corr_stage_dev, &ws->corr_lens, &ws->window };
     for (auto b : bufs) b->release();
     if (ws->corr_stage) (void)hipHostFree(ws->corr_stage);
     if (ws->chain_error) (void)hipHostFree(ws->chain_error);
@@ -338,6 +341,7 @@
     case BTBA_OPT_CHAIN_TIMEOUT_MS: if (value < 1 || value > 60000) return BTBA_EINVAL; t.chain_timeout_ms = (int)value; break;
     case BTBA_OPT_RELAYOUT: t.relayout = value != 0; break;
     case BTBA_OPT_SOLVE_SMALL: t.solve_small = value != 0; break;
+    case BTBA_OPT_SPARSE_MOMENTS: t.sparse_moments = value != 0; break;
     case BTBA_OPT_CORR_NONTEMPORAL: if (value < -1 || value > 1) return BTBA_EINVAL; t.corr_nt = (int)value; break;
     case BTBA_OPT_COUNT_LIVE:
         ws->count_live = value != 0;
@@ -379,6 +383,15 @@
     unsigned long long v = 0;
     HIP_TRY(hipMemcpy(&v, ws->live_blocks.p, sizeof v, hipMemcpyDeviceToHost));
     *blocks = v;
+    return BTBA_OK;
+}
+
+int btba_workspace_sparse_records(btba_workspace *ws, float *records_host, int64_t n_floats)
+{
+    DeviceGuard device_guard(ws);
+    if (!ws || !records_host || n_floats < 0 || (size_t)n_floats * sizeof(float) > ws->sparse_part.cap) return BTBA_EINVAL;
+    HIP_TRY(hipStreamSynchronize(ws->stream));
+    if (n_floats) HIP_TRY(hipMemcpy(records_host, ws->sparse_part.p, sizeof(float) * (size_t)n_floats, hipMemcpyDeviceToHost));
     return BTBA_OK;
 }
 
@@ -602,6 +615,9 @@
     if ((rc = ws->Tinv.ensure(sizeof(float) * 16 * (size_t)B * N))) return rc;
     if ((rc = ws->sparse_part.ensure(sizeof(float) * (size_t)B * P * chunks * kSparseVals))) return rc;
     if ((rc = ws->dense_part.ensure(sizeof(float) * (size_t)B * (Pd > 0 ? Pd : 1) * tiles * kDenseVals))) return rc;
+    const bool sparse_moments = use_sparse && ws->tune.sparse_moments;
+    const size_t mo_stride = (((size_t)P * chunks * kMomentVals) + 31) & ~(size_t)31;
+    if (sparse_moments) { if ((rc = ws->sparse_mom.ensure(sizeof(float) * (size_t)B * mo_stride))) return rc; }
     if (Pd > 0 && (pairs != ws->dense_pairs_host || ws->dense_pairs_frames != N)) {
         std::vector<int32_t> tab(pairs);
         std::vector<int32_t> off(N + 1, 0);
@@ -673,6 +689,7 @@
     D.dp_stride = (unsigned)((size_t)(Pd > 0 ? Pd : 1) * (atomic_sums ? 1 : tiles) * kDenseVals);
     if ((size_t)B * std::max(D.sp_stride, D.dp_stride) >= ((size_t)1 << 32) || (size_t)B * 16 * N >= ((size_t)1 << 31)) return BTBA_EINVAL;
     D.atomic_sums = atomic_sums ? 1 : 0;
+    D.moments = sparse_moments ? ws->sparse_mom.as<float>() : nullptr; D.mo_stride = (unsigned)mo_stride; D.moments_first = 1;
     D.corr24 = corr24 ? 1 : 0;
     D.pair_lens = pair_lens;
     if (Pd > 0) { D.dense_work = reinterpret_cast<const int4 *>(ws->dense_pairs.as<int32_t>() + ws->dense_work_offset); D.work_formula = ws->work_formula; }
@@ -969,6 +986,7 @@
             Dh.corr24 = c24_it ? 1 : 0;
             Dh.corr_entry0 = (c24_it || relayout) ? (int64_t)b0 * corr_stride : 0;
             Dh.corr24_out = (relayout && it == 0) ? ws->corr24_tmp.as<float2>() : nullptr;
+            if (Dh.moments) { Dh.moments += b0 * mo_stride; Dh.moments_first = it == 0 ? 1 : 0; }
             if (Dh.block_ranges) Dh.block_ranges += b0 * N * (size_t)((Wd / 8) * (Hd / 8));
             const unsigned n_d = (unsigned)tiles * D.n_dense_pairs * H.nb, n_s = (unsigned)chunks * P * H.nb;
             const bool fuse = use_sparse && use_dense_it && n_s >= 64 && n_d >= 64 && !(prm->flags & BTBA_FLAG_NO_FUSE);
diff --git a/bundletrack_amd/csrc/btba_kernels.hpp b/bundletrack_amd/csrc/btba_kernels.hpp
--- a/bundletrack_amd/csrc/btba_kernels.hpp
+++ b/bundletrack_amd/csrc/btba_kernels.hpp
@@ -62,6 +62,9 @@
     unsigned long long *live_blocks;
     int publish;
     int corr_nt_from;
+    float *moments;
+    unsigned mo_stride;
+    int moments_first;
 };
 
 __device__ __forceinline__ size_t frame_slot_of(const SolveDims &D, size_t f) { return D.frame_slot ? (size_t)D.frame_slot[f] : f; }
@@ -224,7 +227,42 @@
 }
 
 __device__ __forceinline__ size_t corr24_index(size_t E) { return (E >> 6) * 192 + (E & 63); }
-template <bool C24, bool NT>
+constexpr int kMomentVals = 28;
+constexpr int kPoseVals = kSparseVals - kMomentVals;
+
+__device__ __forceinline__ float world_moment(const float *M, int k, const float *Tb, int fi, int fj, const float (&ci)[3], const float (&cj)[3])
+{
+    const bool second = k >= 7, cross = k >= 19;
+    const int q = cross ? k - 19 : second ? (k - 7) % 6 : (k + 2) % 3;
+    const int ea = cross ? 0 : second ? (k - 7) / 6 : (k >= 4 ? 1 : 0), eb = cross ? 1 : ea;
+    const int r = cross ? q / 3 : second ? (q < 3 ? 0 : q < 5 ? 1 : 2) : q;
+    const int c = cross ? q % 3 : (q < 3 ? q : q < 5 ? q - 2 : 2);
+    const float4 Ra = *reinterpret_cast<const float4 *>(Tb + 16 * (ea ? fj : fi) + 4 * r);
+    const float4 Rb = *reinterpret_cast<const float4 *>(Tb + 16 * (eb ? fj : fi) + 4 * c);
+    const double n = (double)M[0];
+    if (k == 0) return M[0];
+    const double A[3] = { (double)Ra.x, (double)Ra.y, (double)Ra.z };
+    const double ta = (double)Ra.w + (A[0] * (double)(ea ? cj[0] : ci[0]) + A[1] * (double)(ea ? cj[1] : ci[1]) + A[2] * (double)(ea ? cj[2] : ci[2]));
+    const float *ma = M + 1 + 3 * ea, *mb = M + 1 + 3 * eb;
+    const double am = A[0] * (double)ma[0] + A[1] * (double)ma[1] + A[2] * (double)ma[2];
+    if (!second) return (float)(am + n * ta);
+    const double B[3] = { (double)Rb.x, (double)Rb.y, (double)Rb.z };
+    const double tb = (double)Rb.w + (B[0] * (double)(eb ? cj[0] : ci[0]) + B[1] * (double)(eb ? cj[1] : ci[1]) + B[2] * (double)(eb ? cj[2] : ci[2]));
+    const double bm = B[0] * (double)mb[0] + B[1] * (double)mb[1] + B[2] * (double)mb[2];
+    constexpr int sym[3][3] = { { 0, 1, 2 }, { 1, 3, 4 }, { 2, 4, 5 } };
+    const int s0 = 7 + 6 * ea;
+    double quad = 0.0;
+#pragma unroll
+    for (int y = 0; y < 3; y++) {
+        double u = 0.0;
+#pragma unroll
+        for (int x = 0; x < 3; x++) u += A[x] * (double)M[cross ? 19 + 3 * x + y : s0 + sym[x][y]];
+        quad += u * B[y];
+    }
+    return (float)(quad + am * tb + ta * (bm + n * tb));
+}
+
+template <bool C24, bool NT, int MOM>
 __device__ __forceinline__ void sparse_block_impl(const SolveDims &D, const float4 *__restrict__ corr, const uint32_t *__restrict__ pair_offsets,
                                                   const float *__restrict__ T, float *__restrict__ partials, int chunk, int p, int b, float *red)
 {
@@ -239,18 +277,64 @@
     const float *Tb = T + (unsigned)b * (unsigned)D.pose_stride;
     const Mat4 Ti = load_mat4_uniform(Tb + 16 * fi);
     const Mat4 Tj = load_mat4_uniform(Tb + 16 * fj);
-    float acc[kSparseVals];
-#pragma unroll
-    for (int k = 0; k < kSparseVals; k++) acc[k] = 0.0f;
-
+    constexpr int NA = MOM == 2 ? kPoseVals : kSparseVals;
+    constexpr int PB = NA - kPoseVals;
+    float acc[NA];
+#pragma unroll
+    for (int k = 0; k < NA; k++) acc[k] = 0.0f;
+    float *const mom = MOM ? D.moments + ((unsigned)b * D.mo_stride + (unsigned)(p * D.sparse_chunks + chunk) * (unsigned)kMomentVals) : nullptr;
+    float cached = 0.0f;
+    if (MOM == 2 && tid >= (unsigned)kPoseVals && tid < (unsigned)kSparseVals)
+        cached = D.publish ? __hip_atomic_load(mom + (tid - kPoseVals), __ATOMIC_RELAXED, __HIP_MEMORY_SCOPE_AGENT) : mom[tid - kPoseVals];
+
+    float ci[3] = { 0.0f, 0.0f, 0.0f }, cj[3] = { 0.0f, 0.0f, 0.0f };
+    if (MOM && hi > lo) {
+        float v[6];
+        bool ok;
+        if (C24) {
+            const float2 *q = reinterpret_cast<const float2 *>(corr) + corr24_index((size_t)D.corr_entry0 + (size_t)b * (size_t)D.corr_stride + lo);
+            const float2 a0 = q[0], a1 = q[64], a2 = q[128];
+            ok = __float_as_uint(a0.x) != 0xFFFFFFFFu;
+            v[0] = a0.x; v[1] = a0.y; v[2] = a1.x; v[3] = a1.y; v[4] = a2.x; v[5] = a2.y;
+        } else {
+            const float4 *q = corr + 2 * ((size_t)b * D.corr_stride + lo);
+            const float4 q0 = q[0], q1 = q[1];
+            ok = __float_as_uint(q0.x) != 0xFFFFFFFFu;
+            v[0] = q0.z; v[1] = q0.w; v[2] = q1.x; v[3] = q1.y; v[4] = q1.z; v[5] = q1.w;
+        }
+#pragma unroll
+        for (int k = 0; k < 6; k++) ok = ok && fabsf(v[k]) < __builtin_inff();
+#pragma unroll
+        for (int k = 0; k < 3; k++) {
+            ci[k] = __uint_as_float(__builtin_amdgcn_readfirstlane(__float_as_uint(ok ? v[k] : 0.0f)));
+            cj[k] = __uint_as_float(__builtin_amdgcn_readfirstlane(__float_as_uint(ok ? v[3 + k] : 0.0f)));
+        }
+    }
     const float delta2 = D.robust_delta * D.robust_delta;
     auto accumulate = [&](bool valid, float pix, float piy, float piz, float pjx, float pjy, float pjz) {
         const float m = valid ? 1.0f : 0.0f;
+        if (MOM) {
+            pix = valid ? pix : ci[0]; piy = valid ? piy : ci[1]; piz = valid ? piz : ci[2];
+            pjx = valid ? pjx : cj[0]; pjy = valid ? pjy : cj[1]; pjz = valid ? pjz : cj[2];
+        }
+        auto moments = [&](auto aix, auto aiy, auto aiz, auto ajx, auto ajy, auto ajz) {
+            acc[0] += m;
+            acc[1] += aix; acc[2] += aiy; acc[3] += aiz;
+            acc[4] += ajx; acc[5] += ajy; acc[6] += ajz;
+            acc[7] += aix * aix; acc[8] += aix * aiy; acc[9] += aix * aiz; acc[10] += aiy * aiy; acc[11] += aiy * aiz; acc[12] += aiz * aiz;
+            acc[13] += ajx * ajx; acc[14] += ajx * ajy; acc[15] += ajx * ajz; acc[16] += ajy * ajy; acc[17] += ajy * ajz; acc[18] += ajz * ajz;
+            acc[19] += aix * ajx; acc[20] += aix * ajy; acc[21] += aix * ajz;
+            acc[22] += aiy * ajx; acc[23] += aiy * ajy; acc[24] += aiy * ajz;
+            acc[25] += aiz * ajx; acc[26] += aiz * ajy; acc[27] += aiz * ajz;
+        };
+        if constexpr (MOM == 1) moments(pix - ci[0], piy - ci[1], piz - ci[2], pjx - cj[0], pjy - cj[1], pjz - cj[2]);
         float wix, wiy, wiz, wjx, wjy, wjz;
         xform_point(Ti, pix, piy, piz, wix, wiy, wiz);
         xform_point(Tj, pjx, pjy, pjz, wjx, wjy, wjz);
-        wix = m != 0.0f ? wix : 0.0f; wiy = m != 0.0f ? wiy : 0.0f; wiz = m != 0.0f ? wiz : 0.0f;
-        wjx = m != 0.0f ? wjx : 0.0f; wjy = m != 0.0f ? wjy : 0.0f; wjz = m != 0.0f ? wjz : 0.0f;
+        if (!MOM) {
+            wix = m != 0.0f ? wix : 0.0f; wiy = m != 0.0f ? wiy : 0.0f; wiz = m != 0.0f ? wiz : 0.0f;
+            wjx = m != 0.0f ? wjx : 0.0f; wjy = m != 0.0f ? wjy : 0.0f; wjz = m != 0.0f ? wjz : 0.0f;
+        }
         const float rx = wix - wjx, ry = wiy - wjy, rz = wiz - wjz;
         const float e2 = rx * rx + ry * ry + rz * rz;
 #ifdef BTBA_EXACT_DIV
@@ -258,20 +342,13 @@
 #else
         const float rho = m * ((e2 <= delta2) ? 1.0f : D.robust_delta * __builtin_amdgcn_rsqf(e2));
 #endif
-        acc[0] += m;
-        acc[1] += wix; acc[2] += wiy; acc[3] += wiz;
-        acc[4] += wjx; acc[5] += wjy; acc[6] += wjz;
-        acc[7] += wix * wix; acc[8] += wix * wiy; acc[9] += wix * wiz; acc[10] += wiy * wiy; acc[11] += wiy * wiz; acc[12] += wiz * wiz;
-        acc[13] += wjx * wjx; acc[14] += wjx * wjy; acc[15] += wjx * wjz; acc[16] += wjy * wjy; acc[17] += wjy * wjz; acc[18] += wjz * wjz;
-        acc[19] += wix * wjx; acc[20] += wix * wjy; acc[21] += wix * wjz;
-        acc[22] += wiy * wjx; acc[23] += wiy * wjy; acc[24] += wiy * wjz;
-        acc[25] += wiz * wjx; acc[26] += wiz * wjy; acc[27] += wiz * wjz;
-        acc[28] += rho * rx; acc[29] += rho * ry; acc[30] += rho * rz;
-        acc[31] += rho * (wiy * rz - wiz * ry); acc[32] += rho * (wiz * rx - wix * rz); acc[33] += rho * (wix * ry - wiy * rx);
-        acc[34] += rho * (wjy * rz - wjz * ry); acc[35] += rho * (wjz * rx - wjx * rz); acc[36] += rho * (wjx * ry - wjy * rx);
-        acc[37] += rho;
-        acc[38] += rho * (wiy * wiy + wiz * wiz); acc[39] += rho * (wix * wix + wiz * wiz); acc[40] += rho * (wix * wix + wiy * wiy);
-        acc[41] += rho * (wjy * wjy + wjz * wjz); acc[42] += rho * (wjx * wjx + wjz * wjz); acc[43] += rho * (wjx * wjx + wjy * wjy);
+        if constexpr (MOM == 0) moments(wix, wiy, wiz, wjx, wjy, wjz);
+        acc[PB + 0] += rho * rx; acc[PB + 1] += rho * ry; acc[PB + 2] += rho * rz;
+        acc[PB + 3] += rho * (wiy * rz - wiz * ry); acc[PB + 4] += rho * (wiz * rx - wix * rz); acc[PB + 5] += rho * (wix * ry - wiy * rx);
+        acc[PB + 6] += rho * (wjy * rz - wjz * ry); acc[PB + 7] += rho * (wjz * rx - wjx * rz); acc[PB + 8] += rho * (wjx * ry - wjy * rx);
+        acc[PB + 9] += rho;
+        acc[PB + 10] += rho * (wiy * wiy + wiz * wiz); acc[PB + 11] += rho * (wix * wix + wiz * wiz); acc[PB + 12] += rho * (wix * wix + wiy * wiy);
+        acc[PB + 13] += rho * (wjy * wjy + wjz * wjz); acc[PB + 14] += rho * (wjx * wjx + wjz * wjz); acc[PB + 15] += rho * (wjx * wjx + wjy * wjy);
     };
     if (C24) {
         const float2 *cb = reinterpret_cast<const float2 *>(corr);
@@ -311,13 +388,40 @@
         if (D.order_flag && misplaced) atomicOr(D.order_flag, 1);
     }
     float *out = partials + ((unsigned)b * D.sp_stride + (unsigned)(D.atomic_sums ? p : p * D.sparse_chunks + chunk) * (unsigned)kSparseVals);
-    block_reduce_store<kSparseVals, 4>(acc, red, out, D.atomic_sums ? 1 : D.publish ? 2 : 0);
+    const int mode = D.atomic_sums ? 1 : D.publish ? 2 : 0;
+    if constexpr (MOM == 0) { block_reduce_store<kSparseVals, 4>(acc, red, out, mode); return; } else {
+    const int wave = (int)(tid >> 6);
+    wave_fold_store<NA>(acc, red + wave * NA);
+    __syncthreads();
+    float *M = MOM == 1 ? red : red + 4 * NA;
+    if (tid < (unsigned)NA) {
+        float s = red[tid];
+#pragma unroll
+        for (int w = 1; w < 4; w++) s += red[w * NA + tid];
+        M[PB ? tid : kMomentVals + tid] = s;
+        if (MOM == 1 && tid < (unsigned)kMomentVals) {
+            if (D.publish) __hip_atomic_store(mom + tid, s, __ATOMIC_RELAXED, __HIP_MEMORY_SCOPE_AGENT); else mom[tid] = s;
+        }
+    } else if (MOM == 2 && tid < (unsigned)kSparseVals) M[tid - kPoseVals] = cached;
+    __syncthreads();
+    if (tid < (unsigned)kSparseVals) {
+        const float s = tid < (unsigned)kMomentVals ? world_moment(M, (int)tid, Tb, fi, fj, ci, cj) : M[tid];
+        if (mode == 1) unsafeAtomicAdd(out + tid, s);
+        else if (mode == 2) __hip_atomic_store(out + tid, s, __ATOMIC_RELAXED, __HIP_MEMORY_SCOPE_AGENT);
+        else out[tid] = s;
+    }
+    }
 }
 __device__ __forceinline__ void sparse_block(const SolveDims &D, const float4 *__restrict__ corr, const uint32_t *__restrict__ pair_offsets,
-                                             const float *__restrict__ T, float *__restrict__ partials, int chunk, int p, int b, float *red)
-{
-    if (D.corr24) { if (b >= D.corr_nt_from) sparse_block_impl<true, true>(D, corr, pair_offsets, T, partials, chunk, p, b, red); else sparse_block_impl<true, false>(D, corr, pair_offsets, T, partials, chunk, p, b, red); }
-    else { if (b >= D.corr_nt_from) sparse_block_impl<false, true>(D, corr, pair_offsets, T, partials, chunk, p, b, red); else sparse_block_impl<false, false>(D, corr, pair_offsets, T, partials, chunk, p, b, red); }
+                                             const float *__restrict__ T, float *__restrict__ partials, int chunk, int p, int b, float *red, bool first)
+{
+#define BTBA_SPARSE_IMPL(C24, NT) do { \
+        if (!D.moments) sparse_block_impl<C24, NT, 0>(D, corr, pair_offsets, T, partials, chunk, p, b, red); \
+        else if (first) sparse_block_impl<C24, NT, 1>(D, corr, pair_offsets, T, partials, chunk, p, b, red); \
+        else sparse_block_impl<C24, NT, 2>(D, corr, pair_offsets, T, partials, chunk, p, b, red); } while (0)
+    if (D.corr24) { if (b >= D.corr_nt_from) BTBA_SPARSE_IMPL(true, true); else BTBA_SPARSE_IMPL(true, false); }
+    else { if (b >= D.corr_nt_from) BTBA_SPARSE_IMPL(false, true); else BTBA_SPARSE_IMPL(false, false); }
+#undef BTBA_SPARSE_IMPL
 }
 
 __global__ void __launch_bounds__(256) k_pack_corr24(const uint4 *__restrict__ seg, const uint4 *__restrict__ src, float2 *__restrict__ dst, int *__restrict__ order_flag)
@@ -356,7 +460,7 @@
                                                         const float *__restrict__ T, float *__restrict__ partials)
 {
     __shared__ float red[kRedFloats];
-    sparse_block(D, corr, pair_offsets, T, partials, blockIdx.x, blockIdx.y, blockIdx.z, red);
+    sparse_block(D, corr, pair_offsets, T, partials, blockIdx.x, blockIdx.y, blockIdx.z, red, D.moments_first != 0);
 }
 
 #ifdef BTBA_EXACT_DIV
@@ -1162,7 +1266,7 @@
         const int chunk = (int)(i % (unsigned)D.sparse_chunks);
         const int p = (int)((i / (unsigned)D.sparse_chunks) % (unsigned)D.n_pairs);
         const int b = (int)(i / ((unsigned)D.sparse_chunks * (unsigned)D.n_pairs));
-        sparse_block(D, corr, pair_offsets, T, sparse_partials, chunk, p, b, red);
+        sparse_block(D, corr, pair_offsets, T, sparse_partials, chunk, p, b, red, D.moments_first != 0);
     } else {
         const unsigned before = nsi ? min(nsi, (slot + Rx - 1u) / Rx) : 0u;
         const unsigned dl = slot - before;
@@ -2067,7 +2171,7 @@
         kind = is_sparse ? 1 : 0;
         if (is_sparse) {
             const int chunk = (int)(idx % (unsigned)D.sparse_chunks), p = (int)(idx / (unsigned)D.sparse_chunks);
-            sparse_block(D, corr, pair_offsets, T_it, sparse_partials + (size_t)it * Cn.sp_ring, chunk, p, b, red);
+            sparse_block(D, corr, pair_offsets, T_it, sparse_partials + (size_t)it * Cn.sp_ring, chunk, p, b, red, it == 0u);
         } else {
             const int tile = D.tile_major ? (int)(idx / (unsigned)D.n_dense_pairs) : (int)(idx % (unsigned)D.dense_tiles);
             const int p = D.tile_major ? (int)(idx % (unsigned)D.n_dense_pairs) : (int)(idx / (unsigned)D.dense_tiles);
diff --git a/bundletrack_amd/optimizer.py b/bundletrack_amd/optimizer.py
--- a/bundletrack_amd/optimizer.py
+++ b/bundletrack_amd/optimizer.py
@@ -47,6 +47,11 @@
         v = C.c_uint64(0)
         check(lib().btba_workspace_live_blocks(self._h, C.byref(v)), "btba_workspace_live_blocks")
         return int(v.value)
+
+    def sparse_records(self, n_instances: int, n_pairs: int, sparse_chunks: int) -> np.ndarray:
+        out = np.empty((n_instances, n_pairs, sparse_chunks, 44), np.float32)
+        check(lib().btba_workspace_sparse_records(self._h, out.ctypes.data, out.size), "btba_workspace_sparse_records")
+        return out
 
     def collect_stats(self) -> dict:
         s = Stats()
diff --git a/include/btba.h b/include/btba.h
--- a/include/btba.h
+++ b/include/btba.h
@@ -134,8 +134,10 @@
     BTBA_OPT_COUNT_LIVE           = 13,
     BTBA_OPT_SOLVE_SMALL          = 16
 };
+#define BTBA_OPT_SPARSE_MOMENTS 17
 BTBA_API int btba_workspace_set_option(btba_workspace *ws, int option, int64_t value);
 BTBA_API int btba_workspace_live_blocks(btba_workspace *ws, uint64_t *blocks);
+BTBA_API int btba_workspace_sparse_records(btba_workspace *ws, float *records_host, int64_t n_floats);
 BTBA_API int btba_workspace_wait_stream(btba_workspace *ws, void *stream);
 BTBA_API int btba_workspace_signal_stream(btba_workspace *ws, void *stream);
 
```

New measurement: 209,700. No clear change (-0.1%).
